# VinAIResearch/DiMSUM

Hardware: AMD Instinct MI355X
Metric: denoiser-fwd latents/sec (higher is better)
Workload: dtype f32; 1 GPU; DiM-L/2 denoiser forward, 256px (4x32x32 latents, 256 tokens), 256 latents per GPU, random-init weights (reference init, zero tensors re-drawn N(0, 0.02^2)); global_batch=256, parallelism=dp1 (replicas, independent latents), launch=eager, matmul_policy=f16s (see notes.matmul_policy)

## Files before the change

dimsum_amd/_lib.py:

```python
import ctypes as C
import os

_HERE = os.path.dirname(os.path.abspath(__file__))
LIB_PATH = os.environ.get("DIMSUM_HIP_LIB") or os.path.join(_HERE, "lib", "libdimsum_hip.so")

F32, F16, BF16 = 0, 1, 2
i32, i64, vp, f32 = C.c_int32, C.c_int64, C.c_void_p, C.c_float


u32 = C.c_uint32


class _Sized(C.Structure):

    def __init__(self, *args, **kw):
        super().__init__(*args, **kw)
        self.struct_size = C.sizeof(type(self))


class SsmExt(_Sized):
    _fields_ = [("struct_size", u32), ("kernel_variant", i32), ("ckpt_ptr", vp), ("timing_start_event", vp), ("timing_stop_event", vp),
                ("out_z_lo_offset", i64), ("dt_w_ptr", vp), ("dt_x_ptr", vp), ("dt_w_row_stride", i64), ("dt_x_row_stride", i64),
                ("dt_rank", i32), ("out_z_f16", i32), ("out_z_scale_ptr", vp), ("out_z_scale_ld", i64)]

# ... 235 lines not shown


class StateUpdateSlotsParams(_Sized):
    _fields_ = [("struct_size", u32), ("num_slots", i32), ("update", StateUpdateParams), ("slots_ptr", vp), ("slots_stride", i64)]


class DecodeLinearSlotsParams(_Sized):
    _fields_ = [("struct_size", u32), ("num_slots", i32), ("linear", DecodeLinearParams), ("slots_ptr", vp), ("slots_stride", i64)]


DECODE_NORM_NONE, DECODE_NORM_LAYER, DECODE_NORM_RMS = 0, 1, 2
DECODE_MAX_BATCH = 16


class CrossEntropyParams(_Sized):
    _fields_ = ([("struct_size", u32), ("dtype", i32)]
                + [(n, i64) for n in ("rows", "vocab", "logits_row_stride", "dlogits_row_stride", "dloss_stride", "ignore_index")]
                + [(n, f32) for n in ("label_smoothing", "logit_scale", "lse_square_scale")] + [("reserved", i32)]
                + [(n, vp) for n in ("logits_ptr", "labels_ptr", "dloss_ptr", "loss_ptr", "lse_ptr", "z_loss_ptr", "dlogits_ptr")])


CROSS_ENTROPY_WAVE_ROW_MAX = 4096


class SampleLogitsParams(_Sized):
    _fields_ = ([("struct_size", u32), ("dtype", i32)] + [(n, i64) for n in ("rows", "vocab", "logits_row_stride")]
                + [("top_k", i32), ("top_p", f32), ("temperature", f32), ("reserved", i32)]
                + [(n, vp) for n in ("logits_ptr", "u_ptr", "out_ptr", "row_index_ptr", "out_table_ptr")] + [("table_steps", i64)])


class NormParams(_Sized):
    _fields_ = ([("struct_size", u32)] + [(n, i32) for n in ("rows", "cols", "is_rms_norm", "x_dtype", "residual_dtype", "out_dtype")]
                + [("eps", f32)]
                + [(n, i64) for n in ("x_row_stride", "residual_row_stride", "y_row_stride", "residual_out_row_stride")]
                + [(n, vp) for n in ("x_ptr", "residual_ptr", "weight_ptr", "bias_ptr", "y_ptr", "residual_out_ptr",
                                     "mean_ptr", "rstd_ptr", "xbias_ptr", "mod_scale_ptr", "mod_shift_ptr")]
                + [("mod_row_stride", i64), ("rows_per_batch", i32), ("y_split3", i32), ("y_inv_scale_ptr", vp)])


class NormBwdParams(_Sized):
    _fields_ = ([("struct_size", u32)] + [(n, i32) for n in ("rows", "cols", "is_rms_norm")] + [("eps", f32), ("reserved", i32)]
                + [(n, i64) for n in ("r_row_stride", "dy_row_stride", "dres_row_stride", "dx_row_stride")]
                + [(n, vp) for n in ("r_ptr", "weight_ptr", "mean_ptr", "rstd_ptr", "dy_ptr", "dres_ptr", "dx_ptr",
                                     "dweight_ptr", "dbias_ptr")])


class TtParams(_Sized):
    _fields_ = ([("struct_size", u32)] + [(n, i32) for n in ("batch", "tokens", "channels", "grid", "kind", "y_split3")]
                + [(n, i64) for n in ("x_batch_stride", "x_token_stride", "res_batch_stride", "res_token_stride",
                                      "y_batch_stride", "y_token_stride", "mod_batch_stride", "w_batch_stride",
                                      "w_token_stride", "red_batch_stride")]
                + [(n, vp) for n in ("x_ptr", "in_index_ptr", "out_index_ptr", "gate_ptr", "scale_ptr", "shift_ptr",
                                     "residual_ptr", "y_ptr", "w_ptr", "wdot_ptr", "wsum_ptr", "tsum_ptr", "y_inv_scale_ptr")]
                + [("y_f16s_lds_offset", i32), ("reserved", i32)])


class XattnParams(_Sized):
    _fields_ = ([("struct_size", u32)] + [(n, i32) for n in ("batch", "seqlen", "heads", "head_dim")] + [("scale", f32), ("n_dirs", i32)]
                + [(n, i64) for n in ("qkv_batch_stride", "qkv_token_stride", "out_batch_stride", "out_token_stride")]
                + [(n, vp) for n in ("qkv1_ptr", "qkv2_ptr", "out_ptr", "lse_ptr", "bias1_ptr", "bias2_ptr")]
                + [("precision", i32), ("out_split3", i32)]
                + [(n, vp) for n in ("x1_inv_ptr", "x2_inv_ptr", "kv_bound_ptr", "out_inv_ptr")] + [("qkv_f16", i32), ("reserved2", i32)])


class XattnBwdParams(_Sized):
    _fields_ = ([("struct_size", u32), ("reserved", u32), ("fwd", XattnParams)] + [(n, i64) for n in ("dqkv_batch_stride", "dqkv_token_stride")]
                + [(n, vp) for n in ("dout_ptr", "dqkv1_ptr", "dqkv2_ptr", "delta_ptr")])


class GemmExt(_Sized):
    _fields_ = ([("struct_size", u32), ("rows_per_batch", i32), ("timing_start_event", vp), ("timing_stop_event", vp)]
                + [(n, i32) for n in ("tune_variant", "tune_group_m", "tune_reserved", "c_image_pieces")]
                + [(n, vp) for n in ("gate_bound_ptr", "h_inv_scale_ptr", "residual_ptr", "gate_ptr")]
                + [("residual_ld", i64), ("gate_ld", i64), ("x12_ptr", vp), ("x12_ld", i64), ("a_alias_rows", i64), ("b_alias_rows", i64),
                   ("a_alias_weight_order", i32), ("qkv_q_cols", i32), ("conv_weight_ptr", vp), ("conv_bias_ptr", vp),
                   ("conv_rows", i32), ("conv_width", i32), ("conv_seq", i32), ("conv_weight_ld", i32),
                   ("a_block_inv_ptr", vp), ("a_block_inv_ld", i64), ("tn_pair_a_cols", i64), ("tn_pair_b_cols", i64),
                   ("k_scale_ptr", vp), ("c_scale_ptr", vp), ("k_inv_a_ptr", vp), ("k_inv_b_ptr", vp)])


class GemmParams(_Sized):
    _fields_ = ([("struct_size", u32)] + [(n, i32) for n in ("m", "n", "k", "operand_dtype", "epilogue")] + [("out_scale", f32), ("reserved", i32)]
                + [(n, i64) for n in ("lda", "ldb", "ldc")]
                + [(n, vp) for n in ("a_ptr", "b_ptr", "bias_ptr", "c_ptr", "a_inv_scale_ptr", "b_inv_scale_ptr")]
                + [("ext", C.POINTER(GemmExt))])


class GeluExt(_Sized):
    _fields_ = [("struct_size", u32), ("reserved", i32), ("row_inv_ptr", vp), ("bound_ptr", vp)]


class GeluParams(_Sized):
    _fields_ = ([("struct_size", u32), ("out_image", i32), ("rows", i64), ("hidden", i64)]
                + [(n, vp) for n in ("x_ptr", "bias_ptr", "dh_ptr", "out_ptr", "inv_scale_ptr", "dbias_ptr")] + [("ext", C.POINTER(GeluExt))])


GELU_OUT_F32, GELU_OUT_SPLIT3, GELU_OUT_PAIR, GELU_OUT_F16S = 0, 1, 2, 3


class MoeExt(_Sized):
    _fields_ = [("struct_size", u32), ("reserved", i32)]


class MoeRouteParams(_Sized):
    _fields_ = ([("struct_size", u32), ("mode", i32), ("num_experts", i32), ("reserved", i32), ("tokens", i64), ("hidden", i64)]
                + [(n, vp) for n in ("x_ptr", "w_ptr", "b_ptr", "prob_ptr", "expert_ptr", "logits_ptr", "offsets_ptr", "perm_ptr", "inv_ptr",
                                     "row_expert_ptr", "work_ptr")]
                + [("work_bytes", i64)] + [(n, vp) for n in ("dprob_ptr", "dxp_ptr", "dx_ptr", "dw_ptr", "db_ptr")] + [("ext", C.POINTER(MoeExt))])


class MoeRowsParams(_Sized):
    _fields_ = ([("struct_size", u32), ("reserved", i32), ("rows", i64), ("hidden", i64)]
                + [(n, vp) for n in ("src_ptr", "perm_ptr", "prob_ptr", "y_ptr", "dst_ptr", "dprob_ptr")] + [("ext", C.POINTER(MoeExt))])


class MoeActParams(_Sized):
    _fields_ = ([("struct_size", u32), ("gated", i32), ("num_experts", i32), ("reserved", i32), ("rows", i64), ("width", i64)]
                + [(n, vp) for n in ("x_ptr", "bias_ptr", "row_expert_ptr", "dh_ptr", "out_ptr", "dbias_ptr")] + [("ext", C.POINTER(MoeExt))])


class MoeGemmParams(_Sized):
    _fields_ = ([("struct_size", u32), ("num_experts", i32), ("tokens", i64), ("k", i64), ("n", i64), ("ldc", i64), ("x_ptr", vp), ("offsets_ptr", vp),
                 ("w_ptrs", C.POINTER(vp)), ("bias_ptr", vp), ("out_ptr", vp), ("ext", C.POINTER(MoeExt))])


class MoeGemmDgradParams(_Sized):
    _fields_ = ([("struct_size", u32), ("num_experts", i32), ("tokens", i64), ("k", i64), ("n", i64), ("ldc", i64), ("dy_ptr", vp), ("offsets_ptr", vp),
                 ("w_ptrs", C.POINTER(vp)), ("dx_ptr", vp), ("ext", C.POINTER(MoeExt))])


class MoeGemmWgradParams(_Sized):
# ... 137 lines not shown
```

dimsum_amd/attention_fusion.py:

```python
import torch
import torch.nn as nn
import torch.nn.functional as F

from . import gemm, native
from .utils import note_torch_path


class _XattnCoreFn(torch.autograd.Function):

    @staticmethod
    def forward(ctx, qkv1, qkv2, bias1, bias2, heads):
        b1 = None if bias1 is None else bias1.float().contiguous()
        b2 = None if bias2 is None else bias2.float().contiguous()
        if not any(ctx.needs_input_grad[:4]):
            return native.xattn_fusion_fwd(qkv1, qkv2, heads, bias1=b1, bias2=b2)
        out, lse = native.xattn_fusion_fwd(qkv1, qkv2, heads, need_lse=True, bias1=b1, bias2=b2)
        ctx.heads = heads
        ctx.f16 = gemm.attn_bwd_f16_enabled(qkv1)
        ctx.save_for_backward(qkv1, qkv2, b1, b2, out, lse)
        return out

    @staticmethod
    def backward(ctx, dout):
        qkv1, qkv2, b1, b2, out, lse = ctx.saved_tensors
        dqkv1, dqkv2 = native.xattn_fusion_bwd(qkv1, qkv2, out, lse, dout, ctx.heads, bias1=b1, bias2=b2, f16=ctx.f16)
        W = dqkv1.shape[-1]
        db1 = dqkv1.reshape(-1, W).sum(0) if (b1 is not None and ctx.needs_input_grad[2]) else None
        db2 = dqkv2.reshape(-1, W).sum(0) if (b2 is not None and dqkv2 is not None and ctx.needs_input_grad[3]) else None
        return dqkv1, dqkv2, db1, db2, None


class CrossAttentionFusion(nn.Module):
    def __init__(self, dim, num_heads=8, qkv_bias=False, qk_norm=False, attn_drop=0.0, proj_drop=0.0,
                 norm_layer=nn.LayerNorm, swap_k=False):
        super().__init__()
        assert dim % num_heads == 0, "dim should be divisible by num_heads"
        self.num_heads = num_heads
        self.head_dim = dim // 2 // num_heads
        self.scale = self.head_dim ** -0.5
        self.swap_k = swap_k
        self.qkv1 = nn.Linear(dim // 2, dim // 2 * 3, bias=qkv_bias)
        self.q_norm1 = norm_layer(self.head_dim) if qk_norm else nn.Identity()
        self.k_norm1 = norm_layer(self.head_dim) if qk_norm else nn.Identity()
        self.qkv2 = nn.Linear(dim // 2, dim // 2 * 3, bias=qkv_bias)
        self.q_norm2 = norm_layer(self.head_dim) if qk_norm else nn.Identity()
        self.k_norm2 = norm_layer(self.head_dim) if qk_norm else nn.Identity()
        self.attn_drop = nn.Dropout(attn_drop)
        self.proj = nn.Linear(dim, dim)
        self.proj_drop = nn.Dropout(proj_drop)
        self._plain = not qk_norm and not swap_k

    def _split(self, qkv, B, N):
        return qkv.reshape(B, N, 3, self.num_heads, self.head_dim).permute(2, 0, 3, 1, 4).unbind(0)

    def forward(self, x1, x2):
        y, b = self.forward_deferred(x1, x2)
        return y if b is None else y + b

    def takes_images(self, ref):
        return self._plain and not (self.training and (self.attn_drop.p > 0.0 or self.proj_drop.p > 0.0)) and native.xattn_supported(ref, self.head_dim)

    def forward_deferred(self, x1, x2, images=False, residual=None):
        if images:
            B, N, C3 = x1.shape
            b1, b2 = self.qkv1.bias, self.qkv2.bias
            if (b1 is None) != (b2 is None):
                raise RuntimeError("CrossAttentionFusion: qkv1 / qkv2 must both have a bias or none")
            bk1 = {} if b1 is None else {"bias": b1.float().contiguous()}
            bk2 = {} if b2 is None else {"bias": b2.float().contiguous()}
            f16 = isinstance(x1, native.F16Image) and (self.num_heads * self.head_dim) % 8 == 0
            qkv1 = qkv2 = None
            if f16:
                kvb = gemm.attn_kv_bound(self.qkv1.weight, b1, self.qkv2.weight, b2)
                qkv1 = gemm.qkv_f16s(x1.reshape(B * N, C3), self.qkv1.weight, b1, N, kvb[0:2])
                qkv2 = gemm.qkv_f16s(x2.reshape(B * N, C3), self.qkv2.weight, b2, N, kvb[2:4]) if qkv1 is not None else None
            if qkv2 is None:
                qkv1 = gemm.linear_split3(x1.reshape(B * N, C3), self.qkv1.weight, **bk1)
                qkv2 = gemm.linear_split3(x2.reshape(B * N, C3), self.qkv2.weight, **bk2)
            qkv1, qkv2 = qkv1.view(B, N, -1), qkv2.view(B, N, -1)
            if f16:
                f3 = native.xattn_fusion_fwd(qkv1, qkv2, self.num_heads, split3="f16s", f16s=(x1.inv.reshape(B, N), x2.inv.reshape(B, N), kvb))
            else:
                f3 = native.xattn_fusion_fwd(qkv1, qkv2, self.num_heads, split_bf16=True, split3="pair" if isinstance(x1, native.PairImage) else True)
            if residual is not None:
                pb = None if self.proj.bias is None else self.proj.bias.float()
                y = gemm.linear_split3(f3.reshape(B * N, -1), self.proj.weight, bias=pb, residual=residual.reshape(B * N, -1))
                return y.view(residual.shape), None
            return gemm.linear_split3(f3.reshape(B * N, -1), self.proj.weight).view(B, N, -1), self.proj.bias
        B, N, C = x1.shape
        drop = self.attn_drop.p if self.training else 0.0
        if self._plain and drop == 0.0 and native.xattn_supported(x1, self.head_dim):
            b1, b2 = self.qkv1.bias, self.qkv2.bias
            if (b1 is None) != (b2 is None):
                raise RuntimeError("CrossAttentionFusion: qkv1 / qkv2 must both have a bias or none")
            fused = _XattnCoreFn.apply(gemm.linear(x1, self.qkv1.weight), gemm.linear(x2, self.qkv2.weight), b1, b2, self.num_heads)
        else:
            if self._plain and drop == 0.0:
                note_torch_path(f"CrossAttentionFusion core for head_dim {self.head_dim} / {x1.dtype}", required_opt_in=True)
            else:
                note_torch_path("CrossAttentionFusion variant (qk_norm / swap_k / attention dropout: unused by the published configs)")
            qkv1, qkv2 = self.qkv1(x1), self.qkv2(x2)
            q1, k1, v1 = self._split(qkv1, B, N)
            q2, k2, v2 = self._split(qkv2, B, N)
            q1, k1, q2, k2 = self.q_norm1(q1), self.k_norm1(k1), self.q_norm2(q2), self.k_norm2(k2)
            if not self.swap_k:
                x12 = F.scaled_dot_product_attention(q1, k2, v2, dropout_p=drop)
                x21 = F.scaled_dot_product_attention(q2, k1, v1, dropout_p=drop)
            else:
                x12 = F.scaled_dot_product_attention(q2, k1, v2, dropout_p=drop)
                x21 = F.scaled_dot_product_attention(q1, k2, v1, dropout_p=drop)
            fused = torch.cat((x12.transpose(1, 2).reshape(B, N, C), x21.transpose(1, 2).reshape(B, N, C)), dim=-1)
        if isinstance(self.proj_drop, nn.Dropout) and self.proj_drop.p > 0.0 and self.training:
            return self.proj_drop(self.proj(fused)), None
        return gemm.linear(fused, self.proj.weight), self.proj.bias
```

dimsum_amd/csrc/gemm_nt.hip:

```cpp
#include "gemm_nt_kernel.hpp"

namespace dimsum {
namespace gemm_nt {

struct gemm_flat_t : dimsum_gemm_ext_t {
    int32_t m, n, k, operand_dtype, epilogue;
    float out_scale;
    int64_t lda, ldb, ldc;
    const void *a_ptr, *b_ptr, *bias_ptr;
    void *c_ptr;
    const void *a_inv_scale_ptr, *b_inv_scale_ptr;
};
static int gemm_flat_from(const dimsum_gemm_params_t *p, gemm_flat_t &f) {
    if (!p) return DIMSUM_ERR_NULL;
    if (p->struct_size != sizeof(dimsum_gemm_params_t)) return DIMSUM_ERR_ABI;
    const int rc = ext_from<dimsum_gemm_ext_t>(p->ext, f);
    if (rc != DIMSUM_OK) return rc;
    f.m = p->m; f.n = p->n; f.k = p->k; f.operand_dtype = p->operand_dtype; f.epilogue = p->epilogue; f.out_scale = p->out_scale;
    f.lda = p->lda; f.ldb = p->ldb; f.ldc = p->ldc;
    f.a_ptr = p->a_ptr; f.b_ptr = p->b_ptr; f.bias_ptr = p->bias_ptr; f.c_ptr = p->c_ptr;
    f.a_inv_scale_ptr = p->a_inv_scale_ptr; f.b_inv_scale_ptr = p->b_inv_scale_ptr;
    return DIMSUM_OK;
}

// ... 100 lines not shown
    return a.N % (gated ? 128 : kBN) == 0 && nk >= 4 && nk % 2 == 0 && a.tiles_m * a.tiles_n > persist_grid() && a.a_alias_tiles == 0 && a.b_alias_tiles == 0;
}

}
}

#ifdef DIMSUM_GEMM_TUNE
#define DIMSUM_GEMM_TUNE_VARIANTS(X) X(1) X(2) X(4) X(8) X(12) X(16) X(3) X(40) X(44) X(72) X(104)
#define DIMSUM_GEMM_TUNE_CASE(V) case V: return launch<kOpBf16, kEpiF32, V>(a, w);
#endif

static int gemm_nt_run(const dimsum_gemm_params_t *pub, void *stream, int *probe) {
    using namespace dimsum;
    using namespace dimsum::gemm_nt;
    gemm_flat_t p;
    Args a;
    if (const int rc = gemm_prologue(pub, p, a)) return rc;
    if (p.m <= 0 || p.n <= 0 || p.k < 2 * kBK || p.m % kBM != 0 || p.k % kBK != 0 || p.n % 4 != 0) return DIMSUM_ERR_SHAPE;
    if (p.a_alias_rows != 0 && (p.a_alias_rows < 0 || p.a_alias_rows % kBK != 0 || p.k != 3 * p.a_alias_rows)) return DIMSUM_ERR_SHAPE;
    if (p.b_alias_rows != 0 && (p.b_alias_rows < 0 || p.b_alias_rows % kBK != 0 || p.k != 3 * p.b_alias_rows || (p.epilogue != DIMSUM_GEMM_EPI_F32 && p.epilogue != DIMSUM_GEMM_EPI_F32_CONV))) return DIMSUM_ERR_SHAPE;
    if (!rows_16bit_ok(p.a_ptr, p.lda, p.a_alias_rows ? 2 * p.a_alias_rows : p.k) || !rows_16bit_ok(p.b_ptr, p.ldb, p.b_alias_rows ? 2 * p.b_alias_rows : p.k)) return DIMSUM_ERR_STRIDE;
    if (!offsets_fit(p, false, false)) return DIMSUM_ERR_STRIDE;
    a.K = p.k;
    a.a_alias_tiles = (int)(p.a_alias_rows / kBK);
    a.a_alias_from = a.a_alias_tiles;
    if (p.a_alias_weight_order) {
        if (!p.a_alias_rows) return DIMSUM_ERR_SHAPE;
        a.a_alias_tiles *= 2;
        a.a_alias_from = a.a_alias_tiles;
    }
    a.b_alias_tiles = (int)(p.b_alias_rows / kBK);
    a.stagger = p.tune_reserved > 0 ? p.tune_reserved : 0;
    if ((p.a_inv_scale_ptr == nullptr) != (p.b_inv_scale_ptr == nullptr)) return DIMSUM_ERR_NULL;
    if (a.sb && !aligned_to<char>(a.sb, 16)) return DIMSUM_ERR_STRIDE;
#ifndef DIMSUM_GEMM_TUNE
    if (p.tune_variant != 0 && p.tune_variant != 512 && p.tune_variant != 513 && p.tune_variant != 514) return DIMSUM_ERR_UNSUPPORTED;
#endif
    const bool bf = p.operand_dtype == DIMSUM_BF16;
    if (p.tune_variant == 512 && bf) return DIMSUM_ERR_UNSUPPORTED;
    const bool m128 = m128_tiles(p.epilogue, bf, p.k, p.tune_variant);
    const Where w = where(p, stream, probe);
    constexpr int kShip = kVarFullLineStores | kVarNtStores;
    if (p.epilogue == DIMSUM_GEMM_EPI_F32_GATE_RESIDUAL) {
        if (!p.residual_ptr) return DIMSUM_ERR_NULL;
        if (!rows_f32_out_ok(p) || p.residual_ld % 4 != 0 || p.residual_ld < p.n || !aligned_to<char>(p.residual_ptr, 16) ||
            (p.bias_ptr && !aligned_to<char>(p.bias_ptr, 16)) || (p.gate_ptr && (p.gate_ld % 4 != 0 || !aligned_to<char>(p.gate_ptr, 16))))
            return DIMSUM_ERR_STRIDE;
        if (p.gate_ptr && (p.rows_per_batch <= 0 || p.rows_per_batch % kBM != 0 || p.m % p.rows_per_batch != 0)) return DIMSUM_ERR_SHAPE;
        fill_right(a, p, p.n, kBN);
        a.res = reinterpret_cast<const float *>(p.residual_ptr);
        a.gate = reinterpret_cast<const float *>(p.gate_ptr);
        a.ldr = p.residual_ld; a.ldg = p.gate_ld;
        a.rows_per_batch = p.gate_ptr ? p.rows_per_batch : p.m;
        if (persist_ok(a, p.epilogue, bf, p.tune_variant)) return launch_persist<kOpF16, kEpiF32GateRes, kShip>(a, w);
        return bf ? launch<kOpBf16, kEpiF32GateRes, kShip>(a, w) : launch_f16<kEpiF32GateRes, kShip>(a, w, m128);
    }
    if (p.epilogue == DIMSUM_GEMM_EPI_F16_QKV) {
        if (bf || !a.sa || !p.gate_bound_ptr) return DIMSUM_ERR_NULL;
        if (p.rows_per_batch <= 0 || p.rows_per_batch % kBM != 0 || p.m % p.rows_per_batch != 0 || p.qkv_q_cols <= 0 || p.qkv_q_cols % 16 != 0 ||
            p.qkv_q_cols > p.n || p.n % 8 != 0)
            return DIMSUM_ERR_SHAPE;
        if (p.ldc % 8 != 0 || p.ldc < p.n || !aligned_to<char>(p.c_ptr, 16) || (p.bias_ptr && !aligned_to<char>(p.bias_ptr, 16)) ||
            (int64_t)257 * p.ldc * 2 >= ((int64_t)1 << 31))
            return DIMSUM_ERR_STRIDE;
        fill_right(a, p, p.n, kBN);
        a.gate_bound = reinterpret_cast<const float *>(p.gate_bound_ptr);
        a.rows_per_batch = p.rows_per_batch;
        a.q_cols = p.qkv_q_cols;
        return launch_f16<kEpiF16Qkv>(a, w, m128);
    }
    if (p.epilogue == DIMSUM_GEMM_EPI_GELU_F16) {
        if (bf || !a.sa || !p.gate_bound_ptr || p.a_alias_rows != 0 || p.x12_ptr || p.c_image_pieces != 0) return DIMSUM_ERR_UNSUPPORTED;
        if (!p.h_inv_scale_ptr) return DIMSUM_ERR_NULL;
        if (p.n % 8 != 0) return DIMSUM_ERR_SHAPE;
        if (p.ldc % 8 != 0 || p.ldc < p.n || !aligned_to<char>(p.c_ptr, 16) || (p.bias_ptr && !aligned_to<char>(p.bias_ptr, 16)) ||
            !aligned_to<char>(p.h_inv_scale_ptr, 4) || (int64_t)257 * p.ldc * 2 >= ((int64_t)1 << 31))
            return DIMSUM_ERR_STRIDE;
        fill_right(a, p, p.n, kBN);
        a.gate_bound = reinterpret_cast<const float *>(p.gate_bound_ptr);
        a.inv_out = reinterpret_cast<float *>(p.h_inv_scale_ptr);
        return launch_f16<kEpiGeluF16>(a, w, m128);
    }
    if (p.epilogue == DIMSUM_GEMM_EPI_F32_CONV) {
        if (!p.conv_weight_ptr) return DIMSUM_ERR_NULL;
        if (p.conv_rows <= 0 || p.conv_rows % kBM != 0 || p.conv_rows > p.m || p.conv_width < 2 || p.conv_width > 4 || p.conv_seq <= 0 || 256 % p.conv_seq != 0 ||
            p.conv_seq % 4 != 0 || p.n % p.conv_seq != 0 || p.conv_weight_ld < p.conv_width)
            return DIMSUM_ERR_SHAPE;
        if (!rows_f32_out_ok(p)) return DIMSUM_ERR_STRIDE;
        fill_right(a, p, p.n, kBN);
        a.bias0 = nullptr;
        a.conv_w = reinterpret_cast<const float *>(p.conv_weight_ptr);
        a.conv_b = reinterpret_cast<const float *>(p.conv_bias_ptr);
        a.conv_rows = p.conv_rows; a.conv_width = p.conv_width; a.conv_seq = p.conv_seq; a.conv_w_ld = p.conv_weight_ld;
        return bf ? launch<kOpBf16, kEpiF32Conv, kShip>(a, w) : launch_f16<kEpiF32Conv, kShip>(a, w, m128);
    }
    if (p.epilogue == DIMSUM_GEMM_EPI_F32 || p.epilogue == DIMSUM_GEMM_EPI_F32_BIAS) {
        if (!rows_f32_out_ok(p)) return DIMSUM_ERR_STRIDE;
        const bool bias = p.epilogue == DIMSUM_GEMM_EPI_F32_BIAS;
        if (bias && (!p.bias_ptr || !aligned_to<char>(p.bias_ptr, 16))) return DIMSUM_ERR_NULL;
        fill_right(a, p, p.n, kBN);
        if (bias) return bf ? launch<kOpBf16, kEpiF32Bias, kShip>(a, w) : launch_f16<kEpiF32Bias, kShip>(a, w, m128);
#ifdef DIMSUM_GEMM_TUNE
        if (bf) switch (p.tune_variant) {
            case 0: case 512: case 513: break;
            case 100: return launch<kOpBf16, kEpiF32, 0>(a, w);
            DIMSUM_GEMM_TUNE_VARIANTS(DIMSUM_GEMM_TUNE_CASE)
// ... 123 lines not shown
```

dimsum_amd/csrc/gemm_nt_kernel.hpp:

```cpp
#pragma once
#include "common.hpp"

namespace dimsum {
namespace gemm_nt {

typedef float f4 __attribute__((ext_vector_type(4)));
typedef __bf16 bf16x8_t __attribute__((ext_vector_type(8)));
typedef _Float16 f16x8_t __attribute__((ext_vector_type(8)));
typedef unsigned u32x4 __attribute__((ext_vector_type(4)));
typedef unsigned u32x2 __attribute__((ext_vector_type(2)));
typedef __attribute__((address_space(3))) void lds_void_t;
typedef __attribute__((address_space(1))) const void glb_void_t;

constexpr int kBM = 256, kBN = 256, kBK = 64;
constexpr int kHalf = 16384;
constexpr int kParity = 4 * kHalf;
constexpr int kSlotA0 = 0, kSlotA1 = kHalf, kSlotB0 = 2 * kHalf, kSlotB1 = 3 * kHalf;

enum { kOpBf16 = 0, kOpF16 = 1 };
enum { kEpiF32 = 0, kEpiGatedSplit3 = 1, kEpiGatedF16 = 2, kEpiF32Bias = 3, kEpiF32GateRes = 4, kEpiF16Qkv = 5, kEpiF32Conv = 6, kEpiGeluF16 = 7 };

struct Args {
    const char *A, *B0, *B1;
    void *C;
    const float *bias0, *bias1;
    const float *sa, *sb;
    const float *gate_bound;
    float *inv_out;
    const float *res, *gate;
    int64_t ldr, ldg;
    int rows_per_batch;
    int64_t lda, ldb, ldc;
    int M, N, K;
    int tiles_m, tiles_n;
    float out_scale;
    int group_m;
    int stagger;
    float *x12;
    int64_t ldx;
    int splits;
    int64_t c_split_stride;
    int a_alias_tiles;
    int a_alias_from;
    int tn_pieces;
    int64_t a_pair_cols, b_pair_cols;
    int b_alias_tiles;
    const float *conv_w, *conv_b;
    int conv_rows, conv_width, conv_seq, conv_w_ld;
    const float *a_block_inv;
    int a_block_inv_ld;
    const _Float16 *k_fac;
    const float *c_scale;
    const float *k_inv_a, *k_inv_b;
    int q_cols;
    int c_pieces2;
};
enum { kVarLgkmAfterBarrier = 1, kVarNoEpilogue = 2, kVarNtStores = 4, kVarFullLineStores = 8, kVarNoSetprio = 16, kVarSc1Stores = 32, kVarSc0Stores = 64, kVarKeepX12 = 128, kVarTN = 256, kVarM128 = 512, kVarRebase = 1024, kVarPersist = 2048, kVarRowFac = 4096, kVarNN = 8192 };

__device__ __forceinline__ float dpp_row_ror8(float x) {
    const int v = __builtin_bit_cast(int, x);
    return __builtin_bit_cast(float, __builtin_amdgcn_update_dpp(v, v, 0x128, 0xf, 0xf, false));
}
template <int kAux> __device__ __forceinline__ void store_f4(__amdgpu_buffer_rsrc_t rsrc, unsigned voff, const f4 &v) {
    __builtin_amdgcn_raw_buffer_store_b128(__builtin_bit_cast(u32x4, v), rsrc, voff, 0, kAux);
}

template <int kOp> __device__ __forceinline__ f4 mma(const u32x4 &a, const u32x4 &b, f4 c) {
    if constexpr (kOp == kOpBf16) return __builtin_amdgcn_mfma_f32_16x16x32_bf16(__builtin_bit_cast(bf16x8_t, a), __builtin_bit_cast(bf16x8_t, b), c, 0, 0, 0);
    else return __builtin_amdgcn_mfma_f32_16x16x32_f16(__builtin_bit_cast(f16x8_t, a), __builtin_bit_cast(f16x8_t, b), c, 0, 0, 0);
}

__device__ __forceinline__ const char *uniform_ptr(const char *q) {
    const uint64_t v = reinterpret_cast<uint64_t>(q);
    const unsigned lo = __builtin_amdgcn_readfirstlane((unsigned)v), hi = __builtin_amdgcn_readfirstlane((unsigned)(v >> 32));
    return reinterpret_cast<const char *>(((uint64_t)hi << 32) | lo);
}

__device__ __forceinline__ unsigned pick_mask(bool c) {
    unsigned m = c ? 0xffffffffu : 0u;
    asm volatile("" : "+v"(m));
    return m;
}
// ... 501 lines not shown
        DIMSUM_WAIT_VM(8);
        DIMSUM_PHASE_SYNC();
        DIMSUM_QUADRANT(0, 1, a0, b1);
        DIMSUM_PHASE_END();
        DIMSUM_READ_A(a1, kSlotA1, par);
        read_fac(kt);
        DIMSUM_WAIT_VM(6);
        DIMSUM_PHASE_SYNC();
        rebase(a1, 1, kt);
        DIMSUM_QUADRANT(1, 1, a1, b1);
        DIMSUM_PHASE_END();
        DIMSUM_READ_A(a0, kSlotA0, par_next);
        read_fac(kt + 1);
        DIMSUM_WAIT_VM(4);
        DIMSUM_PHASE_SYNC();
        DIMSUM_QUADRANT(1, 0, a1, b0);
        rebase(a0, 0, kt + 1);
        DIMSUM_PHASE_END();
        DIMSUM_READ_B(b0, kSlotB0, par_next);
        DIMSUM_WAIT_VM(2);
        DIMSUM_PHASE_SYNC();
        DIMSUM_QUADRANT(0, 0, a0, b0);
        DIMSUM_PHASE_END();
        DIMSUM_READ_B(b1, kSlotB1, par_next);
        DIMSUM_WAIT_VM(0);
        DIMSUM_PHASE_SYNC();
        DIMSUM_QUADRANT(0, 1, a0, b1);
        DIMSUM_PHASE_END();
        DIMSUM_READ_A(a1, kSlotA1, par_next);
        read_fac(kt + 1);
        DIMSUM_PHASE_SYNC();
        rebase(a1, 1, kt + 1);
        DIMSUM_QUADRANT(1, 1, a1, b1);
        DIMSUM_PHASE_END();
        DIMSUM_QUADRANT(1, 0, a1, b0);
    }
    if (wr == 0) __builtin_amdgcn_s_barrier();
    }

    int lane_e = lane;
    if constexpr (kPersist) asm volatile("" : "+v"(lane_e));
    {
    const int lane = lane_e;
    const int ecol = wc * 32 + (lane >> 4) * 4;
    if constexpr (kVar & kVarNoEpilogue) {
#pragma unroll
        for (int mi = 0; mi < 2; ++mi)
#pragma unroll
            for (int ni = 0; ni < 2; ++ni)
#pragma unroll
                for (int i = 0; i < 4; ++i)
#pragma unroll
                    for (int j = 0; j < 2; ++j) asm volatile("" ::"v"(acc[mi][ni][i][j]));
    } else if constexpr (kEpi == kEpiF32 || kEpi == kEpiF32Bias || kEpi == kEpiF32GateRes || kEpi == kEpiF32Conv) {
        if constexpr (kEpi == kEpiF32Conv) {
            if (m0 < p.conv_rows) {
                constexpr int kNW = kM1 ? 4 : 8;
                constexpr int kHalfRows = kM1 ? 64 : 128;
                float *Ct = reinterpret_cast<float *>(p.C) + (int64_t)m0 * p.ldc + n0;
                const __amdgpu_buffer_rsrc_t crsrc = __builtin_amdgcn_make_buffer_rsrc(Ct, 0, 0x7fffffff, 0x00020000);
                const int W = p.conv_width;
                const bool has_s = p.sa != nullptr;
                const unsigned ms = pick_mask(has_s);
                const float *sap = has_s ? p.sa + m0 : reinterpret_cast<const float *>(p.A), *sbp = has_s ? p.sb : reinterpret_cast<const float *>(p.B0);
                float csa[2][4];
                f4 csb[2][2];
#pragma unroll
                for (int mi = 0; mi < 2; ++mi)
#pragma unroll
                    for (int i = 0; i < 4; ++i) {
                        csa[mi][i] = pick(ms, sap[mi * kMiRows + wr * 64 + i * 16 + (lane & 15)], 1.0f);
                    }
#pragma unroll
                for (int ni = 0; ni < 2; ++ni)
#pragma unroll
                    for (int j = 0; j < 2; ++j) {
                        const int col = n0 + ni * 128 + ecol + j * 16;
                        csb[ni][j] = pick(ms, *reinterpret_cast<const f4 *>(sbp + (col < p.N ? col : 0)), f4{1.f, 1.f, 1.f, 1.f});
                    }
                float ctap[2], cbia[2];
#pragma unroll
                for (int mi = 0; mi < 2; ++mi) {
                    const int row = m0 + mi * kMiRows + w * (kHalfRows / kNW) + (lane & 15);
                    ctap[mi] = pick(pick_mask_lanes((lane >> 4) < W), p.conv_w[(int64_t)row * p.conv_w_ld + ((lane >> 4) < W ? (lane >> 4) : 0)], 0.f);
                    cbia[mi] = pick(pick_mask(p.conv_b != nullptr), (p.conv_b ? p.conv_b : reinterpret_cast<const float *>(p.B0))[row], 0.f);
                }
#pragma unroll
                for (int mi = 0; mi < 2; ++mi) {
                    if (mi) __syncthreads();
#pragma unroll
                    for (int ni = 0; ni < 2; ++ni)
#pragma unroll
                        for (int j = 0; j < 2; ++j) {
                            const int tcol = ni * 128 + ecol + j * 16;
#pragma unroll
                            for (int i = 0; i < 4; ++i) {
                                const int rl = wr * 64 + i * 16 + (lane & 15);
                                const f4 x = acc[mi][ni][i][j] * (csb[ni][j] * csa[mi][i]);
                                *reinterpret_cast<f4 *>(lds + rl * 1024 + (((tcol >> 2) ^ (rl & 7)) << 4)) = x;
                            }
                        }
                    __syncthreads();
#pragma unroll 4
                    for (int it = 0; it < kHalfRows / kNW; ++it) {
                        const int rl = w * (kHalfRows / kNW) + it, row = m0 + mi * kMiRows + rl;
                        const f4 v = *reinterpret_cast<const f4 *>(lds + rl * 1024 + ((lane ^ (rl & 7)) << 4));
                        float w4[4];
#pragma unroll
                        for (int k = 0; k < 4; ++k)
                            w4[k] = (k >= 4 - W) ? __builtin_bit_cast(float, __builtin_amdgcn_readlane(__builtin_bit_cast(int, ctap[mi]), it + 16 * (k - (4 - W)))) : 0.f;
                        const float cbias = __builtin_bit_cast(float, __builtin_amdgcn_readlane(__builtin_bit_cast(int, cbia[mi]), it));
                        const bool start = ((4 * lane) % p.conv_seq) == 0;
                        float p1 = __shfl_up(v[3], 1, 64), p2 = __shfl_up(v[2], 1, 64), p3 = __shfl_up(v[1], 1, 64);
                        p1 = start ? 0.f : p1; p2 = start ? 0.f : p2; p3 = start ? 0.f : p3;
                        f4 y;
                        y[0] = fmaf(w4[0], p3, fmaf(w4[1], p2, fmaf(w4[2], p1, fmaf(w4[3], v[0], cbias))));
                        y[1] = fmaf(w4[0], p2, fmaf(w4[1], p1, fmaf(w4[2], v[0], fmaf(w4[3], v[1], cbias))));
                        y[2] = fmaf(w4[0], p1, fmaf(w4[1], v[0], fmaf(w4[2], v[1], fmaf(w4[3], v[2], cbias))));
                        y[3] = fmaf(w4[0], v[0], fmaf(w4[1], v[1], fmaf(w4[2], v[2], fmaf(w4[3], v[3], cbias))));
#pragma unroll
                        for (int e = 0; e < 4; ++e) y[e] = y[e] * fast_rcp(1.0f + fast_exp(-y[e]));
                        if (n0 + 4 * lane < p.N) store_f4<2>(crsrc, (unsigned)(((mi * kMiRows + rl) * p.ldc + 4 * lane) * 4), y);
                        DIMSUM_PACE_STORES();
                    }
                }
                return;
            }
        }
        constexpr int kAux = ((kVar & kVarNtStores) ? 2 : 0) | ((kVar & kVarSc1Stores) ? 16 : 0) | ((kVar & kVarSc0Stores) ? 1 : 0);
        float *Ct = reinterpret_cast<float *>(p.C) + (int64_t)m0 * p.ldc + n0 + (kBT ? (int64_t)split * p.c_split_stride : (int64_t)0);
        const __amdgpu_buffer_rsrc_t rsrc = __builtin_amdgcn_make_buffer_rsrc(Ct, 0, 0x7fffffff, 0x00020000);
        if constexpr (kVar & kVarFullLineStores) {
            const bool up = (lane & 8) != 0;
            const int frow = wr * 64 + (lane & 7);
            const int fcol = wc * 32 + (lane >> 4) * 4 + (up ? 16 : 0);
            const bool has_s = kRebase || p.sa != nullptr;
            const unsigned ms = pick_mask(has_s);
            const bool has_sb = has_s && !kRowFac;
            const unsigned msb = pick_mask(has_sb);
            const float *sap = p.sa ? p.sa + m0 : reinterpret_cast<const float *>(p.A), *sbp = has_sb ? p.sb : reinterpret_cast<const float *>(p.B0);
            float c_scale = 1.0f;
            if constexpr (kRowFac) c_scale = p.k_inv_a ? c_scale_own : *p.c_scale;
            bool live[2];
            f4 bv[2], sbv[2], gv[2];
            auto load_cols = [&](int ni) {
                const int col = ni * 128 + fcol;
                live[ni] = n0 + col < p.N;
                const int lc = live[ni] ? n0 + col : 0;
                bv[ni] = f4{0.f, 0.f, 0.f, 0.f}; sbv[ni] = gv[ni] = f4{1.f, 1.f, 1.f, 1.f};
                if constexpr (kEpi == kEpiF32Bias) bv[ni] = *reinterpret_cast<const f4 *>(p.bias0 + lc);
                if constexpr (kEpi == kEpiF32GateRes) {
                    bv[ni] = pick(pick_mask(p.bias0 != nullptr), *reinterpret_cast<const f4 *>((p.bias0 ? p.bias0 : reinterpret_cast<const float *>(p.B0)) + lc), bv[ni]);
                    gv[ni] = pick(pick_mask(p.gate != nullptr),
                                  *reinterpret_cast<const f4 *>((p.gate ? p.gate + (int64_t)(m0 / p.rows_per_batch) * p.ldg : reinterpret_cast<const float *>(p.B0)) + lc), gv[ni]);
                }
                sbv[ni] = pick(msb, *reinterpret_cast<const f4 *>(sbp + lc), sbv[ni]);
            };
            load_cols(0);
            live[1] = n0 + 128 + fcol < p.N;
            float rs[2][4][2];
            if constexpr (!kPersist || kRebase || kEpi != kEpiF32GateRes)
#pragma unroll
            for (int mi = 0; mi < 2; ++mi)
#pragma unroll
                for (int i = 0; i < 4; ++i) {
                    const int lrow = frow + mi * kMiRows + i * 16;
                    if constexpr (kRebase) rs[mi][i][0] = rs[mi][i][1] = top[mi * 2 + (i >> 1)];
                    else if constexpr (kRowFac) {
                        rs[mi][i][0] = c_scale * pick(ms, sap[lrow], 1.0f); rs[mi][i][1] = c_scale * pick(ms, sap[lrow + 8], 1.0f);
                    }
                    else {
                        rs[mi][i][0] = pick(ms, sap[lrow], 1.0f); rs[mi][i][1] = pick(ms, sap[lrow + 8], 1.0f);
                    }
                }
            constexpr int kGS = kPersist ? DIMSUM_PERSIST_GS : 4, kNG = 16 / kGS;
            f4 rr[2][kGS][2];
            float rg[2][kGS][2];
            auto load_res = [&](int g) {
                if constexpr (kEpi == kEpiF32GateRes) {
                    const int t0 = g * kGS, ni = t0 >> 3, mi = (t0 >> 2) & 1;
                    if constexpr (kPersist) {
#pragma unroll
                        for (int k = 0; k < kGS; ++k) {
                            const int lrow = frow + mi * kMiRows + ((t0 + k) & 3) * 16;
                            rg[g & 1][k][0] = pick(ms, sap[lrow], 1.0f); rg[g & 1][k][1] = pick(ms, sap[lrow + 8], 1.0f);
                        }
                    }
                    const float *rp = p.res + (int64_t)(m0 + frow + mi * kMiRows) * p.ldr + (live[ni] ? n0 + ni * 128 + fcol : 0);
#pragma unroll
                    for (int k = 0; k < kGS; ++k) {
                        const int i = (t0 + k) & 3;
                        rr[g & 1][k][0] = *reinterpret_cast<const f4 *>(rp + (int64_t)(i * 16) * p.ldr);
                        rr[g & 1][k][1] = *reinterpret_cast<const f4 *>(rp + (int64_t)(i * 16 + 8) * p.ldr);
                    }
                }
            };
            load_res(0);
#pragma unroll
            for (int g = 0; g < kNG; ++g) {
                if (g + 1 < kNG) load_res(g + 1);
                if (g * kGS == 4) load_cols(1);
#pragma unroll
                for (int k = 0; k < kGS; ++k) {
                    const int t = g * kGS + k, ni = t >> 3, mi = (t >> 2) & 1, i = t & 3;
                    const int col = ni * 128 + fcol;
                    const f4 x0 = acc[mi][ni][i][0], x1 = acc[mi][ni][i][1];
                    f4 s0, s1;
#pragma unroll
                    for (int e = 0; e < 4; ++e) {
                        const float r0 = dpp_row_ror8(x0[e]), r1 = dpp_row_ror8(x1[e]);
                        s0[e] = up ? r1 : x0[e];
                        s1[e] = up ? x1[e] : r0;
                    }
                    const int lrow = frow + mi * kMiRows + i * 16;
                    const unsigned voff = (unsigned)((lrow * p.ldc + col) * 4);
                    constexpr bool kRowsInGroup = kPersist && kEpi == kEpiF32GateRes;
                    s0 = s0 * (sbv[ni] * (kRowsInGroup ? rg[g & 1][k][0] : rs[mi][i][0]));
                    s1 = s1 * (sbv[ni] * (kRowsInGroup ? rg[g & 1][k][1] : rs[mi][i][1]));
                    if constexpr (kEpi == kEpiF32GateRes) {
                        s0 = rr[g & 1][k][0] + gv[ni] * (s0 + bv[ni]);
                        s1 = rr[g & 1][k][1] + gv[ni] * (s1 + bv[ni]);
                    } else {
                        s0 = s0 + bv[ni];
                        s1 = s1 + bv[ni];
                    }
                    if (live[ni]) {
                        store_f4<kAux>(rsrc, voff, s0);
                        store_f4<kAux>(rsrc, voff + (unsigned)(8 * p.ldc * 4), s1);
                    }
                    if constexpr (kEpi != kEpiF32GateRes) DIMSUM_PACE_STORES();
                }
            }
        } else {
            const int frow = wr * 64 + (lane & 15);
#pragma unroll
            for (int ni = 0; ni < 2; ++ni)
#pragma unroll
                for (int j = 0; j < 2; ++j) {
                    const int col = ni * 128 + ecol + j * 16;
                    if (n0 + col < p.N) {
                        f4 bv = f4{0.f, 0.f, 0.f, 0.f};
                        if constexpr (kEpi == kEpiF32Bias) bv = *reinterpret_cast<const f4 *>(p.bias0 + n0 + col);
#pragma unroll
                        for (int mi = 0; mi < 2; ++mi)
#pragma unroll
                            for (int i = 0; i < 4; ++i)
                                store_f4<kAux>(rsrc, (unsigned)(((frow + mi * kMiRows + i * 16) * p.ldc + col) * 4), acc[mi][ni][i][j] + bv);
                    }
                }
        }
    } else if constexpr (kEpi == kEpiF16Qkv || kEpi == kEpiGeluF16) {
        constexpr bool kGelu = kEpi == kEpiGeluF16;
        constexpr int kNW = kM1 ? 4 : 8;
        float *red = reinterpret_cast<float *>(lds);
        (void)red;
        const float wl1 = p.gate_bound[0], bmax = p.gate_bound[1];
        float row_sa[2][4], row_qs[2][4];
        f4 cbv[2][2], csb[2][2];
#pragma unroll
        for (int mi = 0; mi < 2; ++mi)
#pragma unroll
            for (int i = 0; i < 4; ++i) row_sa[mi][i] = p.sa[m0 + mi * kMiRows + wr * 64 + i * 16 + (lane & 15)];
        {
            const unsigned mbias = pick_mask(p.bias0 != nullptr);
            const float *b0p = p.bias0 ? p.bias0 : p.sb;
#pragma unroll
            for (int ni = 0; ni < 2; ++ni)
#pragma unroll
                for (int j = 0; j < 2; ++j) {
                    const int col = n0 + ni * 128 + ecol + j * 16, lc = col < p.N ? col : 0;
                    cbv[ni][j] = pick(mbias, *reinterpret_cast<const f4 *>(b0p + lc), f4{0.f, 0.f, 0.f, 0.f});
                    csb[ni][j] = *reinterpret_cast<const f4 *>(p.sb + lc);
                }
        }
        float kv_scale = 0.f, kv_inv;
        if constexpr (!kGelu) {
            {
                const float *sab = p.sa + (int64_t)(m0 / p.rows_per_batch) * p.rows_per_batch;
                float mloc = 0.f;
                for (int t = threadIdx.x; t < p.rows_per_batch; t += kNW * 64) mloc = fmaxf(mloc, sab[t]);
                mloc = wave_allmax(mloc);
                if (lane == 0) red[w] = mloc;
            }
// ... 278 lines not shown
```

dimsum_amd/csrc/norm.hip:

```cpp
#include "common.hpp"

namespace dimsum {

constexpr int kMaxPieces = 8;

__device__ __forceinline__ float wave_allsum(float v) {
#pragma unroll
    for (int o = 32; o > 0; o >>= 1) v += __shfl_xor(v, o, kWave);
    return v;
}

template <typename T> __device__ __forceinline__ f32x4 ld_cols(const T *row, int c, int N, bool vec) {
    if (vec) return c < N ? widen(ld4<T>(row + c)) : f32x4{{0.f, 0.f, 0.f, 0.f}};
    f32x4 r;
#pragma unroll
    for (int e = 0; e < 4; ++e) r.v[e] = (c + e < N) ? to_f32<T>(row[c + e]) : 0.f;
    return r;
}
template <typename T> __device__ __forceinline__ void st_cols(T *row, int c, int N, bool vec, const f32x4 &v) {
    if (vec) { if (c < N) st4<T>(row + c, v); return; }
#pragma unroll
    for (int e = 0; e < 4; ++e)
        if (c + e < N) row[c + e] = from_f32<T>(v.v[e]);
}
// ... 18 lines not shown
        const TR *res = p.residual_ptr ? reinterpret_cast<const TR *>(p.residual_ptr) + row * p.residual_row_stride : nullptr;
        TR *ro = p.residual_out_ptr ? reinterpret_cast<TR *>(p.residual_out_ptr) + row * p.residual_out_row_stride : nullptr;
        TY *y = reinterpret_cast<TY *>(p.y_ptr) + row * p.y_row_stride;
        f32x4 r[kPieces];
        float s = 0.f;
#pragma unroll
        for (int i = 0; i < kPieces; ++i) r[i] = ld_cols<TX>(x, (i * kWave + lane) * 4, N, vec);
        if (xb) {
            f32x4 q[kPieces];
#pragma unroll
            for (int i = 0; i < kPieces; ++i) q[i] = ld_cols<float>(xb, (i * kWave + lane) * 4, N, vec);
#pragma unroll
            for (int i = 0; i < kPieces; ++i)
#pragma unroll
                for (int e = 0; e < 4; ++e) r[i].v[e] += q[i].v[e];
        }
        if (res) {
            f32x4 q[kPieces];
#pragma unroll
            for (int i = 0; i < kPieces; ++i) q[i] = ld_cols<TR>(res, (i * kWave + lane) * 4, N, vec);
#pragma unroll
            for (int i = 0; i < kPieces; ++i)
#pragma unroll
                for (int e = 0; e < 4; ++e) r[i].v[e] += q[i].v[e];
        }
        if (ro) {
#pragma unroll
            for (int i = 0; i < kPieces; ++i) st_cols<TR>(ro, (i * kWave + lane) * 4, N, vec, r[i]);
        }
#pragma unroll
        for (int i = 0; i < kPieces; ++i)
#pragma unroll
            for (int e = 0; e < 4; ++e) s += p.is_rms_norm ? r[i].v[e] * r[i].v[e] : r[i].v[e];
        s = wave_allsum(s);
        float mean = 0.f, var;
        if (p.is_rms_norm) {
            var = s * inv_n;
        } else {
            mean = s * inv_n;
            float v2 = 0.f;
#pragma unroll
            for (int i = 0; i < kPieces; ++i) {
                const int c = (i * kWave + lane) * 4;
#pragma unroll
                for (int e = 0; e < 4; ++e) { const float dlt = (c + e < N) ? r[i].v[e] - mean : 0.f; v2 += dlt * dlt; }
            }
            var = wave_allsum(v2) * inv_n;
        }
        const float rstd = 1.0f / sqrtf(var + p.eps);
        if (lane == 0) {
            if (p.rstd_ptr) reinterpret_cast<float *>(p.rstd_ptr)[row] = rstd;
            if (p.mean_ptr && !p.is_rms_norm) reinterpret_cast<float *>(p.mean_ptr)[row] = mean;
        }
        float ymax = 0.f;
#pragma unroll
        for (int i = 0; i < kPieces; ++i) {
            const int c = (i * kWave + lane) * 4;
            if (c < N) {
                const f32x4 wv = ld_cols<float>(w, c, N, vec);
                const f32x4 bv = bb ? ld_cols<float>(bb, c, N, vec) : f32x4{{0.f, 0.f, 0.f, 0.f}};
                f32x4 o;
#pragma unroll
                for (int e = 0; e < 4; ++e) o.v[e] = (r[i].v[e] - mean) * rstd * wv.v[e] + bv.v[e];
                if (msc) {
                    const f32x4 sc = ld_cols<float>(msc, c, N, vec), sh = ld_cols<float>(msh, c, N, vec);
#pragma unroll
                    for (int e = 0; e < 4; ++e) o.v[e] = fmaf(o.v[e], 1.0f + sc.v[e], sh.v[e]);
                }
                if (p.y_split3 == 2) {
                    r[i] = o;
#pragma unroll
                    for (int e = 0; e < 4; ++e) ymax = fmaxf(ymax, fabsf(o.v[e]));
                } else if (p.y_split3) st_split_left(reinterpret_cast<unsigned short *>(p.y_ptr) + row * p.y_row_stride, c, N, o, p.y_split3 == 3);
                else st_cols<TY>(y, c, N, vec, o);
            }
        }
        if (p.y_split3 == 2) {
            float sc, inv;
            f16s_scales(wave_allmax(ymax), sc, inv);
            __half *yh = reinterpret_cast<__half *>(p.y_ptr) + row * p.y_row_stride;
#pragma unroll
            for (int i = 0; i < kPieces; ++i) {
                const int c = (i * kWave + lane) * 4;
                if (c < N) *reinterpret_cast<uint2 *>(yh + c) = f16s_pack4(r[i], sc);
            }
            if (lane == 0) reinterpret_cast<float *>(p.y_inv_scale_ptr)[row] = inv;
        }
    }
}

template <int kPieces>
__global__ __launch_bounds__(256) void norm_bwd_kernel(const dimsum_norm_bwd_params_t p, const bool vec) {
    const int lane = threadIdx.x & (kWave - 1);
    const int wave = __builtin_amdgcn_readfirstlane(threadIdx.x >> 6);
    const int N = p.cols;
    const float inv_n = 1.0f / (float)N;
    const float *w = reinterpret_cast<const float *>(p.weight_ptr);
    f32x4 wreg[kPieces], dw[kPieces], db[kPieces];
#pragma unroll
    for (int i = 0; i < kPieces; ++i) {
        const int c = (i * kWave + lane) * 4;
        wreg[i] = ld_cols<float>(w, c, N, vec);
        dw[i] = {{0.f, 0.f, 0.f, 0.f}};
        db[i] = {{0.f, 0.f, 0.f, 0.f}};
    }
    const int64_t stride = (int64_t)gridDim.x * 4;
// ... 79 lines not shown
        }
    }
}

template <typename TX, typename TR, typename TY>
static int launch_norm_fwd(const dimsum_norm_params_t &p, hipStream_t s) {
    const int N = p.cols;
    bool vec = N % 4 == 0 && aligned_to<TX>(p.x_ptr, 4 * sizeof(TX)) && aligned_to<TY>(p.y_ptr, 4 * sizeof(TY)) &&
               p.x_row_stride % 4 == 0 && p.y_row_stride % 4 == 0 && aligned_to<float>(p.weight_ptr, 16) &&
               (!p.bias_ptr || aligned_to<float>(p.bias_ptr, 16));
    if (p.residual_ptr) vec = vec && aligned_to<TR>(p.residual_ptr, 4 * sizeof(TR)) && p.residual_row_stride % 4 == 0;
    if (p.residual_out_ptr) vec = vec && aligned_to<TR>(p.residual_out_ptr, 4 * sizeof(TR)) && p.residual_out_row_stride % 4 == 0;
    if (p.xbias_ptr) vec = vec && aligned_to<float>(p.xbias_ptr, 16);
    if (p.mod_scale_ptr) vec = vec && aligned_to<float>(p.mod_scale_ptr, 16) && aligned_to<float>(p.mod_shift_ptr, 16) && p.mod_row_stride % 4 == 0;
    const int pieces = (N + 255) / 256;
    const int64_t blocks = (p.rows + 3) / 4;
    const dim3 grid((unsigned)(blocks < 256 * 16 ? blocks : 256 * 16)), block(256);
#define DIMSUM_NF(K) hipLaunchKernelGGL((norm_fwd_kernel<TX, TR, TY, K>), grid, block, 0, s, p, vec)
    if (pieces <= 1) DIMSUM_NF(1);
    else if (pieces <= 2) DIMSUM_NF(2);
    else if (pieces <= 4) DIMSUM_NF(4);
    else if (pieces <= 5) DIMSUM_NF(5);
    else if (pieces <= kMaxPieces) DIMSUM_NF(8);
    else return DIMSUM_ERR_SHAPE;
#undef DIMSUM_NF
    return launch_status();
}

template <typename TX, typename TR>
static int dispatch_out(const dimsum_norm_params_t &p, hipStream_t s) {
    switch (p.out_dtype) {
        case DIMSUM_F32: return launch_norm_fwd<TX, TR, float>(p, s);
        case DIMSUM_F16: return launch_norm_fwd<TX, TR, __half>(p, s);
        case DIMSUM_BF16: return launch_norm_fwd<TX, TR, __hip_bfloat16>(p, s);
        default: return DIMSUM_ERR_DTYPE;
    }
}
template <typename TX>
static int dispatch_res(const dimsum_norm_params_t &p, hipStream_t s) {
    switch (p.residual_dtype) {
        case DIMSUM_F32: return dispatch_out<TX, float>(p, s);
        case DIMSUM_F16: return dispatch_out<TX, __half>(p, s);
        case DIMSUM_BF16: return dispatch_out<TX, __hip_bfloat16>(p, s);
        default: return DIMSUM_ERR_DTYPE;
    }
}

}

extern "C" int dimsum_norm_fwd(const dimsum_norm_params_t *p, void *stream) {
    using namespace dimsum;
    if (!p) return DIMSUM_ERR_NULL;
    if (p->struct_size != sizeof(dimsum_norm_params_t)) return DIMSUM_ERR_ABI;
    if (!p->x_ptr || !p->weight_ptr || !p->y_ptr) return DIMSUM_ERR_NULL;
    if (p->rows < 0 || p->cols <= 0) return DIMSUM_ERR_SHAPE;
    if ((p->mod_scale_ptr == nullptr) != (p->mod_shift_ptr == nullptr)) return DIMSUM_ERR_NULL;
    if (p->mod_scale_ptr && p->rows_per_batch <= 0) return DIMSUM_ERR_SHAPE;
    if (p->y_split3 == 2) {
        if (!p->y_inv_scale_ptr) return DIMSUM_ERR_NULL;
        if (p->out_dtype != DIMSUM_F16 || p->cols % 4 != 0 || p->y_row_stride % 4 != 0 || p->y_row_stride < p->cols || !dimsum::aligned_to<char>(p->y_ptr, 8))
            return DIMSUM_ERR_STRIDE;
    } else
    if (p->y_split3 && (p->out_dtype != DIMSUM_BF16 || p->cols % 4 != 0 || p->y_row_stride % 4 != 0 || p->y_row_stride < (p->y_split3 == 3 ? 2 : 3) * (int64_t)p->cols ||
                        !dimsum::aligned_to<char>(p->y_ptr, 8)))
        return DIMSUM_ERR_STRIDE;
    if (p->rows == 0) return DIMSUM_OK;
    hipStream_t s = reinterpret_cast<hipStream_t>(stream);
    switch (p->x_dtype) {
        case DIMSUM_F32: return dispatch_res<float>(*p, s);
        case DIMSUM_F16: return dispatch_res<__half>(*p, s);
        case DIMSUM_BF16: return dispatch_res<__hip_bfloat16>(*p, s);
        default: return DIMSUM_ERR_DTYPE;
    }
}

extern "C" int dimsum_norm_bwd(const dimsum_norm_bwd_params_t *p, void *stream) {
    using namespace dimsum;
    if (!p) return DIMSUM_ERR_NULL;
    if (p->struct_size != sizeof(dimsum_norm_bwd_params_t)) return DIMSUM_ERR_ABI;
    if (!p->r_ptr || !p->weight_ptr || !p->rstd_ptr || !p->dy_ptr || !p->dx_ptr || !p->dweight_ptr) return DIMSUM_ERR_NULL;
    if (p->rows < 0 || p->cols <= 0) return DIMSUM_ERR_SHAPE;
    if (p->rows == 0) return DIMSUM_OK;
    hipStream_t s = reinterpret_cast<hipStream_t>(stream);
    const int N = p->cols;
    bool vec = N % 4 == 0 && aligned_to<float>(p->r_ptr, 16) && aligned_to<float>(p->dy_ptr, 16) && aligned_to<float>(p->dx_ptr, 16) &&
               aligned_to<float>(p->weight_ptr, 16) && p->r_row_stride % 4 == 0 && p->dy_row_stride % 4 == 0 && p->dx_row_stride % 4 == 0;
    if (p->dres_ptr) vec = vec && aligned_to<float>(p->dres_ptr, 16) && p->dres_row_stride % 4 == 0;
    const int pieces = (N + 255) / 256;
    const int64_t blocks = (p->rows + 3) / 4;
    const int64_t cap = p->rows >= 32768 ? 512 : 384;
    const dim3 grid((unsigned)(blocks < cap ? blocks : cap)), block(256);
#define DIMSUM_NB(K) hipLaunchKernelGGL((norm_bwd_kernel<K>), grid, block, 0, s, *p, vec)
    if (pieces <= 1) DIMSUM_NB(1);
    else if (pieces <= 2) DIMSUM_NB(2);
    else if (pieces <= 4) DIMSUM_NB(4);
    else if (pieces <= 5) DIMSUM_NB(5);
    else if (pieces <= kMaxPieces) DIMSUM_NB(8);
    else return DIMSUM_ERR_SHAPE;
#undef DIMSUM_NB
    return launch_status();
}
```

dimsum_amd/csrc/token_transform.hip:

```cpp
#include <stdlib.h>
#include <type_traits>

#include "common.hpp"

namespace dimsum {

constexpr int kTTThreads = 256;
__device__ __forceinline__ int haar_lds(int j) {
    const int cp = j >> 4, p = j & 15;
    return (cp >> 2) * 68 + p * 4 + (cp & 3);
}

__device__ __forceinline__ void haar2(float a, float b, float c, float d, float &ll, float &lh, float &hl, float &hh) {
    const float p = a + b, q = a - b, r = c + d, s = c - d;
    ll = (p + r) * 0.5f; lh = (p - r) * 0.5f; hl = (q + s) * 0.5f; hh = (q - s) * 0.5f;
}
__device__ __forceinline__ void ihaar2(float ll, float lh, float hl, float hh, float &a, float &b, float &c, float &d) {
    const float p = ll + lh, q = ll - lh, r = hl + hh, s = hl - hh;
    a = (p + r) * 0.5f; b = (p - r) * 0.5f; c = (q + s) * 0.5f; d = (q - s) * 0.5f;
}

__device__ __forceinline__ void haar_fwd16(const float *X, float *Y) {
    float b1[4][4];
#pragma unroll
// ... 1 lines not shown
#pragma unroll
        for (int j = 0; j < 2; ++j)
            haar2(X[(2 * i) * 4 + 2 * j], X[(2 * i) * 4 + 2 * j + 1], X[(2 * i + 1) * 4 + 2 * j], X[(2 * i + 1) * 4 + 2 * j + 1],
                  b1[0][i * 2 + j], b1[1][i * 2 + j], b1[2][i * 2 + j], b1[3][i * 2 + j]);
#pragma unroll
    for (int k1 = 0; k1 < 4; ++k1) {
        float o[4];
        haar2(b1[k1][0], b1[k1][1], b1[k1][2], b1[k1][3], o[0], o[1], o[2], o[3]);
#pragma unroll
        for (int k2 = 0; k2 < 4; ++k2) Y[k1 * 4 + k2] = o[k2] * 0.25f;
    }
}
__device__ __forceinline__ void haar_inv16(const float *Y, float *X) {
    float b1[4][4];
#pragma unroll
    for (int k1 = 0; k1 < 4; ++k1)
        ihaar2(Y[k1 * 4 + 0], Y[k1 * 4 + 1], Y[k1 * 4 + 2], Y[k1 * 4 + 3], b1[k1][0], b1[k1][1], b1[k1][2], b1[k1][3]);
#pragma unroll
    for (int i = 0; i < 2; ++i)
#pragma unroll
        for (int j = 0; j < 2; ++j)
            ihaar2(b1[0][i * 2 + j], b1[1][i * 2 + j], b1[2][i * 2 + j], b1[3][i * 2 + j], X[(2 * i) * 4 + 2 * j],
                   X[(2 * i) * 4 + 2 * j + 1], X[(2 * i + 1) * 4 + 2 * j], X[(2 * i + 1) * 4 + 2 * j + 1]);
}

__device__ __forceinline__ void dct4(const float *in, int stride, float *out, int ostride, bool inverse) {
    constexpr float kA = 0.5f;
    constexpr float kC1 = 0.6532814824381883f;
    constexpr float kC2 = 0.5f;
    constexpr float kC3 = 0.2705980500730985f;
    const float x0 = in[0], x1 = in[stride], x2 = in[2 * stride], x3 = in[3 * stride];
    if (!inverse) {
        const float s03 = x0 + x3, d03 = x0 - x3, s12 = x1 + x2, d12 = x1 - x2;
        out[0] = kA * (s03 + s12);
        out[ostride] = kC1 * d03 + kC3 * d12;
        out[2 * ostride] = kC2 * (s03 - s12);
        out[3 * ostride] = kC3 * d03 - kC1 * d12;
    } else {
        const float e = kA * x0 + kC2 * x2, f = kA * x0 - kC2 * x2, g = kC1 * x1 + kC3 * x3, h = kC3 * x1 - kC1 * x3;
        out[0] = e + g;
        out[ostride] = f + h;
        out[2 * ostride] = f - h;
        out[3 * ostride] = e - g;
    }
}
__device__ __forceinline__ void dct16(const float *X, float *Y, bool inverse) {
    float t[16];
#pragma unroll
    for (int r = 0; r < 4; ++r) dct4(X + r * 4, 1, t + r * 4, 1, inverse);
#pragma unroll
    for (int c = 0; c < 4; ++c) dct4(t + c, 4, Y + c, 4, inverse);
}

template <int KIND, int VEC, bool F16S = false, int kFix = 0>
__global__ __launch_bounds__(kTTThreads) void token_transform_kernel(const dimsum_tt_params_t p) {
    extern __shared__ __attribute__((aligned(16))) float lds[];
    const int tid = threadIdx.x;
    const int nthreads = (F16S || KIND != DIMSUM_TT_NONE) ? (int)blockDim.x : kTTThreads;
    const int b = blockIdx.y;
    const int C = p.channels, G = p.grid;
    int s_of[16];
    if (KIND == DIMSUM_TT_NONE) {
#pragma unroll
        for (int k = 0; k < 16; ++k) s_of[k] = blockIdx.x * 16 + k;
    } else {
        const int gb = G / 4, bh = blockIdx.x / gb, bw = blockIdx.x - bh * gb;
#pragma unroll
        for (int k = 0; k < 16; ++k) s_of[k] = (bh * 4 + (k >> 2)) * G + bw * 4 + (k & 3);
    }
    int grp = blockIdx.x;
    const int ngrp = KIND == DIMSUM_TT_NONE ? (p.tokens + 15) / 16 : 1;
    auto pos_of = [&](int k) { return KIND == DIMSUM_TT_NONE ? grp * 16 + k : s_of[k]; };
    int tin[KIND == DIMSUM_TT_NONE ? 1 : 16], tout[KIND == DIMSUM_TT_NONE ? 1 : 16];
    if constexpr (KIND != DIMSUM_TT_NONE) {
        if (p.in_index_ptr) {
#pragma unroll
            for (int k = 0; k < 16; ++k) tin[k] = p.in_index_ptr[s_of[k]];
        } else {
#pragma unroll
            for (int k = 0; k < 16; ++k) tin[k] = s_of[k];
        }
        if (p.out_index_ptr) {
#pragma unroll
            for (int k = 0; k < 16; ++k) tout[k] = p.out_index_ptr[s_of[k]];
        } else {
#pragma unroll
            for (int k = 0; k < 16; ++k) tout[k] = s_of[k];
        }
    }
    float stash[F16S ? 16 : 1][VEC], tmax[F16S ? 16 : 1];
    if constexpr (F16S) {
#pragma unroll
        for (int k = 0; k < 16; ++k) tmax[k] = 0.f;
    }
    const float *xb = reinterpret_cast<const float *>(p.x_ptr) + (int64_t)b * p.x_batch_stride;
    float *yb = p.y_ptr ? reinterpret_cast<float *>(p.y_ptr) + (int64_t)b * p.y_batch_stride : nullptr;
    const float *rb = p.residual_ptr ? reinterpret_cast<const float *>(p.residual_ptr) + (int64_t)b * p.res_batch_stride : nullptr;
    const float *gate = p.gate_ptr ? reinterpret_cast<const float *>(p.gate_ptr) + (int64_t)b * p.mod_batch_stride : nullptr;
    const float *scale = p.scale_ptr ? reinterpret_cast<const float *>(p.scale_ptr) + (int64_t)b * p.mod_batch_stride : nullptr;
    const float *shift = p.shift_ptr ? reinterpret_cast<const float *>(p.shift_ptr) + (int64_t)b * p.mod_batch_stride : nullptr;

    const float *wb = p.w_ptr ? reinterpret_cast<const float *>(p.w_ptr) + (int64_t)b * p.w_batch_stride : nullptr;
    const bool has_gate = kFix == 0 ? gate != nullptr : kFix == 2;
    const bool has_mod = kFix == 0 ? scale != nullptr : (kFix == 1 || kFix == 3 || kFix == 5);
    const bool has_shift = kFix == 0 ? shift != nullptr : kFix == 1;
    const bool has_res = kFix == 0 ? rb != nullptr : kFix == 2;
    const bool has_w = kFix == 0 ? wb != nullptr : kFix >= 3;
    const bool has_tsum = kFix == 0 ? p.tsum_ptr != nullptr : kFix == 5;
    const bool has_y = kFix == 0 ? yb != nullptr : kFix != 4;
    float wdot[VEC], wsum[VEC], tsum[VEC];
#pragma unroll
    for (int e = 0; e < VEC; ++e) { wdot[e] = 0.f; wsum[e] = 0.f; tsum[e] = 0.f; }
    auto flush_red = [&](int c) {
        if (wb || p.tsum_ptr) {
#pragma unroll
            for (int e = 0; e < VEC; ++e) {
                if (p.wdot_ptr) atomicAdd(reinterpret_cast<float *>(p.wdot_ptr) + (int64_t)b * p.red_batch_stride + c + e, wdot[e]);
                if (p.wsum_ptr) atomicAdd(reinterpret_cast<float *>(p.wsum_ptr) + (int64_t)b * p.red_batch_stride + c + e, wsum[e]);
                if (p.tsum_ptr) atomicAdd(reinterpret_cast<float *>(p.tsum_ptr) + (int64_t)b * p.red_batch_stride + c + e, tsum[e]);
                wdot[e] = 0.f; wsum[e] = 0.f; tsum[e] = 0.f;
            }
        }
    };

    auto load_vec = [&](const float *ptr, float *dst) {
        if constexpr (VEC == 4) { const float4 t = *reinterpret_cast<const float4 *>(ptr); dst[0] = t.x; dst[1] = t.y; dst[2] = t.z; dst[3] = t.w; }
        else dst[0] = *ptr;
    };
    auto store_out = [&](int k, int c, const float *val) {
#pragma clang fp contract(off)
        int tok;
        if constexpr (KIND == DIMSUM_TT_NONE) {
            if (pos_of(k) >= p.tokens) return;
            tok = p.out_index_ptr ? p.out_index_ptr[pos_of(k)] : pos_of(k);
        } else {
            tok = tout[k];
        }
        float o[VEC], t[VEC];
#pragma unroll
        for (int e = 0; e < VEC; ++e) o[e] = val[e];
        if (has_w) { load_vec(wb + (int64_t)tok * p.w_token_stride + c, t);
#pragma unroll
            for (int e = 0; e < VEC; ++e) { wdot[e] = fmaf(o[e], t[e], wdot[e]); wsum[e] += t[e]; } }
        if (has_tsum) {
#pragma unroll
            for (int e = 0; e < VEC; ++e) tsum[e] += o[e]; }
        if (!has_y) return;
        if (has_mod) { load_vec(scale + c, t);
#pragma unroll
            for (int e = 0; e < VEC; ++e) o[e] *= 1.0f + t[e]; }
        if (has_shift) { load_vec(shift + c, t);
#pragma unroll
            for (int e = 0; e < VEC; ++e) o[e] += t[e]; }
        if (has_res) { load_vec(rb + (int64_t)tok * p.res_token_stride + c, t);
#pragma unroll
            for (int e = 0; e < VEC; ++e) o[e] += t[e]; }
        if constexpr (F16S) {
#pragma unroll
            for (int e = 0; e < VEC; ++e) { stash[k][e] = o[e]; tmax[k] = fmaxf(tmax[k], fabsf(o[e])); }
            return;
        }
        if constexpr (VEC == 4) {
            if (p.y_split3) {
                st_split_left(reinterpret_cast<unsigned short *>(p.y_ptr) + (int64_t)b * p.y_batch_stride + (int64_t)tok * p.y_token_stride, c, C,
                              f32x4{{o[0], o[1], o[2], o[3]}}, p.y_split3 == 3);
                return;
            }
        }
        float *dst = yb + (int64_t)tok * p.y_token_stride + c;
        if constexpr (VEC == 4) *reinterpret_cast<float4 *>(dst) = make_float4(o[0], o[1], o[2], o[3]);
        else dst[0] = o[0];
    };
    auto load_in = [&](int k, int c, float *dst) {
#pragma clang fp contract(off)
        int tok;
        if constexpr (KIND == DIMSUM_TT_NONE) {
            if (pos_of(k) >= p.tokens) {
#pragma unroll
                for (int e = 0; e < VEC; ++e) dst[e] = 0.f;
                return;
            }
            tok = p.in_index_ptr ? p.in_index_ptr[pos_of(k)] : pos_of(k);
        } else {
            tok = tin[k];
        }
        load_vec(xb + (int64_t)tok * p.x_token_stride + c, dst);
        if (has_gate) { float t[VEC]; load_vec(gate + c, t);
#pragma unroll
            for (int e = 0; e < VEC; ++e) dst[e] *= t[e]; }
    };

    if constexpr (KIND == DIMSUM_TT_NONE) {
        const int cg = (C + VEC - 1) / VEC;
        const int nsub = cg <= kTTThreads / 4 ? 4 : (cg <= kTTThreads / 2 ? 2 : 1);
        if (!F16S && nsub > 1 && C % VEC == 0) {
            const int sub = tid / cg, c = (tid - sub * cg) * VEC;
            if (sub < nsub) {
                auto pass = [&](auto perc) {
                    constexpr int PER = decltype(perc)::value;
                    for (grp = blockIdx.x; grp < ngrp; grp += gridDim.x) {
                        float v[PER][VEC];
#pragma unroll
                        for (int k = 0; k < PER; ++k) load_in(sub * PER + k, c, v[k]);
#pragma unroll
                        for (int k = 0; k < PER; ++k) store_out(sub * PER + k, c, v[k]);
                    }
                    flush_red(c);
                };
                if (nsub == 2) pass(std::integral_constant<int, 8>{});
                else pass(std::integral_constant<int, 4>{});
            }
            return;
        }
    }

    if constexpr (KIND == DIMSUM_TT_HAAR_INV) {
        for (int c = tid * VEC; c < C; c += nthreads * VEC) {
#pragma unroll
            for (int k = 0; k < 16; ++k) {
                float v[VEC];
                load_in(k, c, v);
#pragma unroll
                for (int e = 0; e < VEC; ++e) lds[haar_lds((c + e) * 16 + k)] = v[e] * 4.0f;
            }
        }
        __syncthreads();
    }

    for (int c = tid * VEC; c < C; c += nthreads * VEC) {
        float X[VEC][16], Y[VEC][16];
        if constexpr (KIND == DIMSUM_TT_HAAR_INV) {
#pragma unroll
            for (int q = 0; q < 16; ++q)
#pragma unroll
                for (int e = 0; e < VEC; ++e) Y[e][q] = lds[haar_lds(q * C + c + e)];
#pragma unroll
            for (int e = 0; e < VEC; ++e) haar_inv16(Y[e], X[e]);
#pragma unroll
            for (int k = 0; k < 16; ++k) { float o[VEC];
// ... 41 lines not shown
            }
        }
    }

    if constexpr (KIND == DIMSUM_TT_HAAR_FWD) {
        __syncthreads();
        for (int c = tid * VEC; c < C; c += nthreads * VEC) {
#pragma unroll
            for (int k = 0; k < 16; ++k) {
                float o[VEC];
                if constexpr (VEC == 4) {
                    const float4 t = *reinterpret_cast<const float4 *>(&lds[(c >> 2) * 68 + k * 4]);
                    o[0] = t.x; o[1] = t.y; o[2] = t.z; o[3] = t.w;
                } else {
                    o[0] = lds[haar_lds(c * 16 + k)];
                }
                store_out(k, c, o);
            }
            flush_red(c);
        }
    }

    if constexpr (F16S && VEC == 4) {
        float *red = lds + p.y_f16s_lds_offset;
        const int wave = tid >> 6, lane = tid & 63;
#pragma unroll
        for (int k = 0; k < 16; ++k) tmax[k] = wave_allmax(tmax[k]);
        if (lane < 16) {
            float m = tmax[0];
#pragma unroll
            for (int k = 1; k < 16; ++k) m = lane == k ? tmax[k] : m;
            red[wave * 16 + lane] = m;
        }
        __syncthreads();
        const int c = tid * VEC;
        __half *yh = reinterpret_cast<__half *>(p.y_ptr) + (int64_t)b * p.y_batch_stride;
        float *inv_out = reinterpret_cast<float *>(p.y_inv_scale_ptr) + (int64_t)b * p.tokens;
#pragma unroll
        for (int k = 0; k < 16; ++k) {
            if (KIND == DIMSUM_TT_NONE && pos_of(k) >= p.tokens) continue;
            float m = red[k];
            for (int w = 1; w < (nthreads >> 6); ++w) m = fmaxf(m, red[w * 16 + k]);
            float sc, inv;
            f16s_scales(m, sc, inv);
            int tok;
            if constexpr (KIND == DIMSUM_TT_NONE) tok = p.out_index_ptr ? p.out_index_ptr[pos_of(k)] : pos_of(k);
            else tok = tout[k];
            if (c < C) *reinterpret_cast<uint2 *>(yh + (int64_t)tok * p.y_token_stride + c) = f16s_pack4(f32x4{{stash[k][0], stash[k][1], stash[k][2], stash[k][3]}}, sc);
            if (tid == k) inv_out[tok] = inv;
        }
    }
}

template <int kPieces, int kOut>
__global__ __launch_bounds__(256) void token_rows_kernel(const dimsum_tt_params_t p) {
    const int lane = threadIdx.x & 63, wave = threadIdx.x >> 6;
    const int C = p.channels, T = p.tokens;
    const int64_t rows = (int64_t)p.batch * T;
    for (int64_t row = (int64_t)blockIdx.x * 4 + wave; row < rows; row += (int64_t)gridDim.x * 4) {
        const int b = (int)(row / T), s = (int)(row - (int64_t)b * T);
        const int src = p.in_index_ptr ? p.in_index_ptr[s] : s, dst = p.out_index_ptr ? p.out_index_ptr[s] : s;
        const float *x = reinterpret_cast<const float *>(p.x_ptr) + (int64_t)b * p.x_batch_stride + (int64_t)src * p.x_token_stride;
        const float *res = p.residual_ptr ? reinterpret_cast<const float *>(p.residual_ptr) + (int64_t)b * p.res_batch_stride + (int64_t)dst * p.res_token_stride : nullptr;
        const float *gate = p.gate_ptr ? reinterpret_cast<const float *>(p.gate_ptr) + (int64_t)b * p.mod_batch_stride : nullptr;
        const float *scale = p.scale_ptr ? reinterpret_cast<const float *>(p.scale_ptr) + (int64_t)b * p.mod_batch_stride : nullptr;
        const float *shift = p.shift_ptr ? reinterpret_cast<const float *>(p.shift_ptr) + (int64_t)b * p.mod_batch_stride : nullptr;
        f32x4 v[kPieces];
        float m = 0.f;
        auto ld = [&](const float *ptr, f32x4 (&q)[kPieces]) {
#pragma unroll
            for (int i = 0; i < kPieces; ++i) {
                const int c = (i * 64 + lane) * 4;
                const float4 t = c < C ? *reinterpret_cast<const float4 *>(ptr + c) : make_float4(0.f, 0.f, 0.f, 0.f);
                q[i] = f32x4{{t.x, t.y, t.z, t.w}};
            }
        };
        f32x4 q[kPieces];
        ld(x, v);
        if (gate) { ld(gate, q);
#pragma unroll
            for (int i = 0; i < kPieces; ++i)
#pragma unroll
                for (int e = 0; e < 4; ++e) v[i].v[e] *= q[i].v[e]; }
        if (scale) { ld(scale, q);
#pragma unroll
            for (int i = 0; i < kPieces; ++i)
#pragma unroll
                for (int e = 0; e < 4; ++e) v[i].v[e] *= 1.0f + q[i].v[e]; }
        if (shift) { ld(shift, q);
#pragma unroll
            for (int i = 0; i < kPieces; ++i)
#pragma unroll
                for (int e = 0; e < 4; ++e) v[i].v[e] += q[i].v[e]; }
        if (res) { ld(res, q);
#pragma unroll
            for (int i = 0; i < kPieces; ++i)
#pragma unroll
                for (int e = 0; e < 4; ++e) v[i].v[e] += q[i].v[e]; }
#pragma unroll
        for (int i = 0; i < kPieces; ++i)
#pragma unroll
            for (int e = 0; e < 4; ++e) m = fmaxf(m, fabsf(v[i].v[e]));
        if constexpr (kOut == 2) {
            float sc, inv;
            f16s_scales(wave_allmax(m), sc, inv);
            __half *y = reinterpret_cast<__half *>(p.y_ptr) + (int64_t)b * p.y_batch_stride + (int64_t)dst * p.y_token_stride;
#pragma unroll
            for (int i = 0; i < kPieces; ++i) {
                const int c = (i * 64 + lane) * 4;
                if (c < C) *reinterpret_cast<uint2 *>(y + c) = f16s_pack4(v[i], sc);
            }
            if (lane == 0) reinterpret_cast<float *>(p.y_inv_scale_ptr)[(int64_t)b * T + dst] = inv;
        } else if constexpr (kOut == 1) {
            unsigned short *y = reinterpret_cast<unsigned short *>(p.y_ptr) + (int64_t)b * p.y_batch_stride + (int64_t)dst * p.y_token_stride;
#pragma unroll
            for (int i = 0; i < kPieces; ++i) {
                const int c = (i * 64 + lane) * 4;
                if (c < C) st_split_left(y, c, C, v[i], p.y_split3 == 3);
            }
        } else {
            float *y = reinterpret_cast<float *>(p.y_ptr) + (int64_t)b * p.y_batch_stride + (int64_t)dst * p.y_token_stride;
#pragma unroll
            for (int i = 0; i < kPieces; ++i) {
                const int c = (i * 64 + lane) * 4;
                if (c < C) *reinterpret_cast<float4 *>(y + c) = make_float4(v[i].v[0], v[i].v[1], v[i].v[2], v[i].v[3]);
            }
        }
    }
}

template <int VEC>
static int launch_tt(const dimsum_tt_params_t &p, hipStream_t s) {
    const bool blocked = p.kind != DIMSUM_TT_NONE;
    const int nblk = blocked ? (p.grid / 4) * (p.grid / 4) : (p.tokens + 15) / 16;
    const int cgs = (p.channels + VEC - 1) / VEC;
    int gx = nblk;
    if (!blocked && (p.w_ptr || p.tsum_ptr) && p.y_split3 != 2) {
        const int min_wgs = p.y_ptr ? 1024 : 512;
        while (gx % 2 == 0 && (int64_t)(gx / 2) * p.batch >= min_wgs) gx /= 2;
    }
    const dim3 grid(gx, p.batch), block(blocked ? (cgs <= 64 ? 64 : (cgs <= 128 ? 128 : kTTThreads)) : kTTThreads);
    size_t lds = (p.kind == DIMSUM_TT_HAAR_FWD || p.kind == DIMSUM_TT_HAAR_INV) ? (size_t)((p.channels + 3) / 4) * 68 * 4 : 0;
    if (lds > 160 * 1024) return DIMSUM_ERR_SHAPE;
    if (p.kind == DIMSUM_TT_NONE && p.y_ptr && !p.w_ptr && !p.tsum_ptr && p.channels <= 2048) {
        if constexpr (VEC == 4) {
            const int64_t rows = (int64_t)p.batch * p.tokens;
            int64_t blocks = (rows + 3) / 4;
            if (blocks > 256 * 16) blocks = 256 * 16;
            const dim3 g1((unsigned)blocks), b1(256);
#define DIMSUM_TTR(O)                                                                                    \
            if (p.channels <= 512) hipLaunchKernelGGL((token_rows_kernel<2, O>), g1, b1, 0, s, p);          \
            else if (p.channels <= 1024) hipLaunchKernelGGL((token_rows_kernel<4, O>), g1, b1, 0, s, p);    \
            else hipLaunchKernelGGL((token_rows_kernel<8, O>), g1, b1, 0, s, p)
            if (p.y_split3 == 2) { DIMSUM_TTR(2); }
            else if (p.y_split3) { DIMSUM_TTR(1); }
            else { DIMSUM_TTR(0); }
#undef DIMSUM_TTR
            return launch_status();
        }
        if (p.y_split3 == 2) return DIMSUM_ERR_STRIDE;
    }
    if (p.y_split3 == 2) {
        if constexpr (VEC == 4) {
            dimsum_tt_params_t q = p;
            q.y_f16s_lds_offset = (int32_t)(lds / 4);
            lds += 64 * 4;
            const int cg = (p.channels + 3) / 4;
            const dim3 blockh(cg <= 64 ? 64 : (cg <= 128 ? 128 : kTTThreads));
            static const bool fix = !(getenv("DIMSUM_TT_FIX") && atoi(getenv("DIMSUM_TT_FIX")) == 0);
            const bool pre = fix && p.scale_ptr && p.shift_ptr && !p.gate_ptr && !p.residual_ptr, post = fix && p.gate_ptr && p.residual_ptr && !p.scale_ptr && !p.shift_ptr;
#define DIMSUM_TTH(K) do { if (blocked && pre) hipLaunchKernelGGL((token_transform_kernel<K, 4, true, (K) == DIMSUM_TT_NONE ? 0 : 1>), grid, blockh, lds, s, q);          \
                           else if (blocked && post) hipLaunchKernelGGL((token_transform_kernel<K, 4, true, (K) == DIMSUM_TT_NONE ? 0 : 2>), grid, blockh, lds, s, q);    \
                           else hipLaunchKernelGGL((token_transform_kernel<K, 4, true, 0>), grid, blockh, lds, s, q); } while (0)
            switch (p.kind) {
                case DIMSUM_TT_NONE: DIMSUM_TTH(DIMSUM_TT_NONE); break;
                case DIMSUM_TT_HAAR_FWD: DIMSUM_TTH(DIMSUM_TT_HAAR_FWD); break;
                case DIMSUM_TT_HAAR_INV: DIMSUM_TTH(DIMSUM_TT_HAAR_INV); break;
                case DIMSUM_TT_DCT_FWD: DIMSUM_TTH(DIMSUM_TT_DCT_FWD); break;
                case DIMSUM_TT_DCT_INV: DIMSUM_TTH(DIMSUM_TT_DCT_INV); break;
                default: return DIMSUM_ERR_SHAPE;
            }
#undef DIMSUM_TTH
            return launch_status();
        }
        return DIMSUM_ERR_STRIDE;
    }
    if constexpr (VEC == 4) {
        static const bool fix = !(getenv("DIMSUM_TT_FIX") && atoi(getenv("DIMSUM_TT_FIX")) == 0);
        const bool sc = p.scale_ptr != nullptr, sh = p.shift_ptr != nullptr, ga = p.gate_ptr != nullptr, re = p.residual_ptr != nullptr;
        const bool w = p.w_ptr != nullptr, ts = p.tsum_ptr != nullptr, y = p.y_ptr != nullptr;
        int kf = 0;
        if (fix && !w && !ts && y) kf = (blocked && sc && sh && !ga && !re) ? 1 : (blocked && ga && re && !sc && !sh) ? 2 : 0;
        else if (fix && w && !sh && !ga && !re) kf = (sc && !ts && y) ? 3 : (!sc && !ts && !y) ? 4 : (sc && ts && y) ? 5 : 0;
        if (kf) {
#define DIMSUM_TTF(K) do { if (kf == 1) hipLaunchKernelGGL((token_transform_kernel<K, 4, false, 1>), grid, block, lds, s, p);      \
                           else if (kf == 2) hipLaunchKernelGGL((token_transform_kernel<K, 4, false, 2>), grid, block, lds, s, p); \
                           else if (kf == 3) hipLaunchKernelGGL((token_transform_kernel<K, 4, false, 3>), grid, block, lds, s, p); \
                           else if (kf == 4) hipLaunchKernelGGL((token_transform_kernel<K, 4, false, 4>), grid, block, lds, s, p); \
                           else hipLaunchKernelGGL((token_transform_kernel<K, 4, false, 5>), grid, block, lds, s, p); } while (0)
            switch (p.kind) {
                case DIMSUM_TT_NONE: DIMSUM_TTF(DIMSUM_TT_NONE); break;
                case DIMSUM_TT_HAAR_FWD: DIMSUM_TTF(DIMSUM_TT_HAAR_FWD); break;
                case DIMSUM_TT_HAAR_INV: DIMSUM_TTF(DIMSUM_TT_HAAR_INV); break;
                case DIMSUM_TT_DCT_FWD: DIMSUM_TTF(DIMSUM_TT_DCT_FWD); break;
                case DIMSUM_TT_DCT_INV: DIMSUM_TTF(DIMSUM_TT_DCT_INV); break;
                default: return DIMSUM_ERR_SHAPE;
            }
#undef DIMSUM_TTF
            return launch_status();
        }
    }
#define DIMSUM_TT(K) hipLaunchKernelGGL((token_transform_kernel<K, VEC>), grid, block, lds, s, p)
    switch (p.kind) {
        case DIMSUM_TT_NONE: DIMSUM_TT(DIMSUM_TT_NONE); break;
        case DIMSUM_TT_HAAR_FWD: DIMSUM_TT(DIMSUM_TT_HAAR_FWD); break;
        case DIMSUM_TT_HAAR_INV: DIMSUM_TT(DIMSUM_TT_HAAR_INV); break;
        case DIMSUM_TT_DCT_FWD: DIMSUM_TT(DIMSUM_TT_DCT_FWD); break;
        case DIMSUM_TT_DCT_INV: DIMSUM_TT(DIMSUM_TT_DCT_INV); break;
        default: return DIMSUM_ERR_SHAPE;
    }
#undef DIMSUM_TT
    return launch_status();
}

}

extern "C" int dimsum_token_transform(const dimsum_tt_params_t *p, void *stream) {
    using namespace dimsum;
    if (!p) return DIMSUM_ERR_NULL;
    if (p->struct_size != sizeof(dimsum_tt_params_t)) return DIMSUM_ERR_ABI;
    if (!p->x_ptr) return DIMSUM_ERR_NULL;
    if (!p->y_ptr && !p->tsum_ptr && !(p->w_ptr && (p->wdot_ptr || p->wsum_ptr))) return DIMSUM_ERR_NULL;
    if ((p->wdot_ptr || p->wsum_ptr) && !p->w_ptr) return DIMSUM_ERR_NULL;
    if (p->batch < 0 || p->tokens <= 0 || p->channels <= 0) return DIMSUM_ERR_SHAPE;
    if (p->kind != DIMSUM_TT_NONE && (p->grid % 4 != 0 || p->grid * p->grid != p->tokens)) return DIMSUM_ERR_SHAPE;
    if (p->batch == 0) return DIMSUM_OK;
    hipStream_t s = reinterpret_cast<hipStream_t>(stream);
    bool vec = p->channels % 4 == 0 && aligned_to<float>(p->x_ptr, 16) && (!p->y_ptr || aligned_to<float>(p->y_ptr, 16)) &&
               p->x_batch_stride % 4 == 0 && p->x_token_stride % 4 == 0 && p->y_batch_stride % 4 == 0 && p->y_token_stride % 4 == 0 &&
               p->mod_batch_stride % 4 == 0 && (!p->gate_ptr || aligned_to<float>(p->gate_ptr, 16)) &&
               (!p->scale_ptr || aligned_to<float>(p->scale_ptr, 16)) && (!p->shift_ptr || aligned_to<float>(p->shift_ptr, 16));
    if (p->residual_ptr) vec = vec && aligned_to<float>(p->residual_ptr, 16) && p->res_batch_stride % 4 == 0 && p->res_token_stride % 4 == 0;
    if (p->w_ptr) vec = vec && aligned_to<float>(p->w_ptr, 16) && p->w_batch_stride % 4 == 0 && p->w_token_stride % 4 == 0;
    if (p->y_split3 == 2) {
        if (!p->y_ptr || !p->y_inv_scale_ptr) return DIMSUM_ERR_NULL;
        if (!vec || p->y_token_stride < p->channels || p->channels > (p->kind == DIMSUM_TT_NONE ? 2048 : 4 * kTTThreads) || p->w_ptr || p->tsum_ptr)
            return DIMSUM_ERR_STRIDE;
    } else
    if (p->y_split3 && (!vec || !p->y_ptr || p->y_token_stride < (p->y_split3 == 3 ? 2 : 3) * (int64_t)p->channels)) return DIMSUM_ERR_STRIDE;
    return vec ? launch_tt<4>(*p, s) : launch_tt<1>(*p, s);
}
```

dimsum_amd/gemm.py:

```python
import contextlib
import os
import threading

import torch
import torch.nn.functional as F

_policy = "default"


class _Local(threading.local):
    frozen = None


_tls = _Local()


@contextlib.contextmanager
def frozen_weights():
    outer = _tls.frozen
    if outer is None:
        _tls.frozen = {}
    try:
        yield
    finally:
# ... 428 lines not shown
            cache[key("w16s_bound", w)] = (scal[sl:sl + 2], w)
        else:
            cache[key("w16s", w)] = ((images[j], lambda i=sl: scal[i:i + 1] / _K10), w)
            if partner is not None:
                j2 = j + (2 if bias is not None else 1)
                cache[key("w16s", partner.weight)] = ((images[j2], lambda i=sl + 2: scal[i:i + 1] / _K10), partner.weight)
                cache[key("kvbound", w)] = (scal[sl:sl + 4], w)
            else:
                cache[key("kvbound", w)] = (torch.cat([scal[sl:sl + 2], scal[sl:sl + 2]]), w)
    if not training and os.environ.get("DIMSUM_FORWARD_MEMO", "1") != "0":
        alogs = [a for m in model.modules() for a in (getattr(m, "A_log", None), getattr(m, "A_b_log", None)) if isinstance(a, torch.nn.Parameter) and a.is_cuda]
        if alogs:
            vals = torch._foreach_neg(torch._foreach_exp([a.detach().float() for a in alogs]))
            for a, v in zip(alogs, vals):
                cache[key("negexpA", a)] = (v, a)
    _tls.frozen = cache
    try:
        yield
    finally:
        _tls.frozen = None


def neg_exp(a_log):
    frozen = _tls.frozen
    if frozen is not None and not torch.is_grad_enabled() and not torch.cuda.is_current_stream_capturing():
        hit = frozen.get(("negexpA", a_log.data_ptr(), tuple(a_log.shape), tuple(a_log.stride()), a_log.dtype))
        if hit is not None:
            return hit[0]
    return -torch.exp(a_log.float())


def own_gemm_enabled():
    return os.environ.get("DIMSUM_GEMM_NT", "1") != "0"


def _nt(a, b, **kw):
    from . import native
    if own_gemm_enabled() and native.gemm_nt_supported(a, b):
        return native.gemm_nt(a, b, **kw)
    y = torch.mm(a, b.t(), out_dtype=torch.float32)
    return y if kw.get("bias") is None else y + kw["bias"]


def _tail(y, bias, residual, gate, rows_per_batch):
    if bias is not None:
        y = y + bias
    if residual is None:
        return y
    if gate is not None:
        y = (y.view(-1, rows_per_batch, y.shape[-1]) * gate.unsqueeze(1)).view(y.shape)
    return residual + y


def _nt_f16s(a, b, bias=None, residual=None, gate=None, rows_per_batch=None):
    from . import native
    if own_gemm_enabled() and native.gemm_nt_supported(a.data, b.data) and (gate is None or rows_per_batch % 256 == 0):
        return native.gemm_nt(a.data, b.data, bias=bias, scales=(a.inv, b.inv), residual=residual, gate=gate, rows_per_batch=rows_per_batch)
    return _tail(torch.mm(a.data, b.data.t(), out_dtype=torch.float32) * a.inv[:, None] * b.inv[None, :], bias, residual, gate, rows_per_batch)


def linear_split3(x3, weight, bias=None, residual=None, gate=None, rows_per_batch=None):
    from . import native
    if isinstance(x3, native.F16Image):
        return _nt_f16s(x3, weight_f16s(weight), bias, residual, gate, rows_per_batch)
    w3i = weight_image(weight)
    if isinstance(x3, native.PairImage) and not (own_gemm_enabled() and native.gemm_nt_supported(x3, w3i) and (gate is None or rows_per_batch % 256 == 0)):
        x3 = x3.image3()
    if residual is None and bias is None:
        return _nt(x3, w3i)
    if own_gemm_enabled() and native.gemm_nt_supported(x3, w3i) and (gate is None or rows_per_batch % 256 == 0):
        return native.gemm_nt(x3, w3i, bias=bias, residual=residual, gate=gate, rows_per_batch=rows_per_batch)
    return _tail(torch.mm(x3, w3i.t(), out_dtype=torch.float32), bias, residual, gate, rows_per_batch)


def matmul_wx_split3(weight, x3, conv=None):
    from . import native
    if conv is not None:
        cw, cb, seq = conv
        a = weight_f16s(weight) if isinstance(x3, native.F16Image) else weight_image(weight)
        ad, bd = (a.data, x3.data) if isinstance(x3, native.F16Image) else (a, x3)
        ok = (os.environ.get("DIMSUM_INPROJ_CONV", "1") != "0" and own_gemm_enabled() and native.gemm_nt_supported(ad, bd)
              and cw.dtype == torch.float32 and cw.dim() == 2 and cw.stride(1) == 1 and cw.shape[0] % 256 == 0 and 2 <= cw.shape[1] <= 4
              and seq % 4 == 0 and 256 % seq == 0 and x3.shape[0] % seq == 0)
        if ok:
            cbf = None if cb is None else cb.detach().float().contiguous()
            if isinstance(x3, native.F16Image):
                return native.gemm_nt(ad, bd, scales=(a.inv, x3.inv), conv=(cw.detach(), cbf, seq)), True
            return native.gemm_nt(a, x3, conv=(cw.detach(), cbf, seq)), True
        return matmul_wx_split3(weight, x3), False
    if isinstance(x3, native.F16Image):
        return _nt_f16s(weight_f16s(weight), x3)
    w3i = weight_image(weight)
    if isinstance(x3, native.PairImage) and not (own_gemm_enabled() and native.gemm_nt_supported(w3i, x3)):
        x3 = x3.image3()
    return _nt(w3i, x3)


def gated_mlp_hidden_split3(x3, w12, b12):
    from . import native
    if isinstance(x3, native.F16Image):
        w16 = weight_f16s(w12)
        if own_gemm_enabled() and native.gemm_nt_supported(x3.data, w16.data, gated=True):
            return native.gemm_nt(x3.data, w16.data, bias=b12, epilogue="gated_f16", scales=(x3.inv, w16.inv), gate_bound=gated_bound(w12, b12))
        x12 = _nt_f16s(x3, w16)
        return native.rows_f16s(native.gated_gelu_fwd(x12, b12))
    w3i = weight_image(w12)
    if own_gemm_enabled() and native.gemm_nt_supported(x3, w3i, gated=True):
        pair = (w12.shape[0] // 2) % 64 == 0 and os.environ.get("DIMSUM_PAIR_IMAGES", "1") != "0"
        return native.gemm_nt(x3, w3i, bias=b12, epilogue="gated_split3", pair_out=pair)
    if isinstance(x3, native.PairImage):
        x3 = x3.image3()
    return native.gated_gelu_fwd(torch.mm(x3, w3i.t(), out_dtype=torch.float32), b12, split3=True)


def mlp_hidden_split3(x3, w1, b1):
    from . import native
    F_ = w1.shape[0]
# ... 117 lines not shown
```

dimsum_amd/models_dim.py:

```python
import math
import os
from functools import partial

import numpy as np
import torch
import torch.nn as nn
import torch.nn.functional as F

from . import scanning_orders as so
from . import gemm
from .attention_fusion import CrossAttentionFusion
from .dct_layer import init_dct_kernel, init_idct_kernel
from .mlp import GatedMLP, Mlp
from .switch_mlp import SwitchMLP
from .modules.mamba_simple import CondMamba, Mamba
from .ops import token_ops
from .ops.layernorm import RMSNorm, layer_norm_fn, rms_norm_fn
from .pe.cpe import AdaInPosCNN
from .pe.my_rotary import apply_rotary, get_2d_sincos_rotary_embed
from .wavelet_layer import DWT_2D, IDWT_2D


def modulate(x, shift, scale):
    return x * (1 + scale.unsqueeze(1)) + shift.unsqueeze(1)
# ... 225 lines not shown
    if inference_params is not None:
        raise NotImplementedError("inference_params: " + _NOT_CAUSAL)


def _modulation(seq, c):
    hit = getattr(gemm._tls, "cond", None)
    if hit is not None and hit[0] is c and len(seq) == 2 and isinstance(seq[0], nn.SiLU):
        return seq[1](hit[1])
    return seq(c)


def _mlp_in_weight(mlp):
    return (mlp.w12 if isinstance(mlp, GatedMLP) else mlp.fc1).weight


def _mlp_tail(mlp, x, normed, shift, scale, gate):
    if isinstance(mlp, GatedMLP) and mlp._fused and gemm.split3_train_enabled(normed, mlp.w12.weight):
        from .mlp import mod_gated_mlp_images
        m, mb = mod_gated_mlp_images(mlp, normed, shift, scale)
        return token_ops.gate_residual(x, m, gate, mb)
    h = token_ops.pre_mixer(normed, "none", None, shift, scale)
    if hasattr(mlp, "forward_deferred"):
        m, mb = mlp.forward_deferred(h)
        return token_ops.gate_residual(x, m, gate, mb)
    return token_ops.gate_residual(x, mlp(h), gate, None)


def _fast_tail(norm_2, mlp, hidden_states):
    return (not torch.is_grad_enabled() and isinstance(norm_2, RMSNorm) and hasattr(mlp, "forward_deferred")
            and hidden_states.dtype == torch.float32)


def _norm_mlp_tail(norm_2, mlp, hidden_states, shift, scale, gate, fused=None, pb=None, in_epilogue=False):
    if _fast_tail(norm_2, mlp, hidden_states):
        from . import native
        B, L, H = hidden_states.shape
        x, res = (hidden_states, None) if fused is None else (fused, None if in_epilogue else hidden_states)
        s3 = getattr(mlp, "_fused", False) and gemm.split3_enabled(hidden_states, _mlp_in_weight(mlp), producer="norm")
        y, _, _, hnew = native.layer_norm_fwd(x.reshape(B * L, H), norm_2.weight, norm_2.bias, norm_2.eps,
                                              residual=None if res is None else res.reshape(B * L, H), is_rms_norm=True, x_bias=pb,
                                              mod_scale=scale, mod_shift=shift, rows_per_batch=L, **({"split3": s3} if s3 else {}))
        if s3 and hnew.is_contiguous():
            return mlp.forward_deferred(hidden_states, x3=y, residual=hnew.view(B, L, H), gate=gate)[0]
        m, mb = mlp.forward_deferred(hidden_states, x3=y) if s3 else mlp.forward_deferred(y.view(B, L, H))
        return token_ops.gate_residual(hnew.view(B, L, H), m, gate, mb)
    if fused is not None:
        hidden_states = token_ops.gate_residual(hidden_states, fused, None, pb)
    if isinstance(norm_2, RMSNorm) and hidden_states.is_cuda and torch.is_grad_enabled():
        normed, hidden_states = norm_2(hidden_states, prenorm=True)
        return _mlp_tail(mlp, hidden_states, normed, shift, scale, gate)
    return _mlp_tail(mlp, hidden_states, norm_2(hidden_states), shift, scale, gate)


def _mix_through_images(mixer, hidden_states, kind, table, shift, scale, c, fork=False):
    if getattr(mixer, "takes_image", lambda: False)() and gemm.split3_enabled(hidden_states, mixer.in_proj.weight, left=False):
        m = mixer(None, c, x3=token_ops.pre_mixer(hidden_states, kind, table, shift, scale,
                                                  split3=gemm.split3_enabled(hidden_states, mixer.in_proj.weight, left=False)))
        return (m, hidden_states) if fork else m
    if fork and hidden_states.is_cuda and torch.is_grad_enabled() and hidden_states.requires_grad:
        t, hidden_states = token_ops.pre_mixer_fork(hidden_states, kind, table, shift, scale)
        return mixer(t, c), hidden_states
    m = mixer(token_ops.pre_mixer(hidden_states, kind, table, shift, scale), c)
    return (m, hidden_states) if fork else m


class _BlockBase(nn.Module):

    def _prenorm(self, hidden_states, residual):
        if not self.fused_add_norm:
            residual = hidden_states if residual is None else residual + self.drop_path(hidden_states)
            hidden_states = (self.norm(residual) if isinstance(self.norm, nn.Identity)
                             else self.norm(residual.to(dtype=self.norm.weight.dtype)))
            if self.residual_in_fp32:
                residual = residual.to(torch.float32)
            return hidden_states, residual
        fn = rms_norm_fn if isinstance(self.norm, RMSNorm) else layer_norm_fn
        x = hidden_states if residual is None else self.drop_path(hidden_states)
        return fn(x, self.norm.weight, self.norm.bias, residual=residual, prenorm=True,
                  residual_in_fp32=self.residual_in_fp32, eps=self.norm.eps)

    def _table(self, L, device, build):
        cache = self.__dict__.setdefault("_tables", {})
        key = (L, str(device))
        if key not in cache:
            fwd = build(math.isqrt(L))
            mixer = getattr(self, "mixer", None)
            if mixer is not None and getattr(mixer, "_is_zigzag", lambda: False)() and getattr(mixer, "zigzag_paths", None) is not None \
                    and os.environ.get("DIMSUM_FOLD_ZIGZAG", "1") != "0":
                perm = mixer.zigzag_paths[mixer.layer_idx].detach().cpu().numpy().astype(np.int64)
                assert perm.shape[0] == L, "zigzag path length != sequence length"
                fwd = perm if fwd is None else so.compose(fwd, perm)
                mixer._zigzag_folded = True
            if fwd is None:
                cache[key] = None
            else:
                inv = so.reverse_permut_np(fwd)
                cache[key] = {"fwd": so.as_index(fwd, device), "inv": so.as_index(inv, device),
                              "inv32": torch.as_tensor(inv.astype(np.int32), device=device)}
        return cache[key]

    def allocate_inference_cache(self, *a, **k):
        raise NotImplementedError("allocate_inference_cache: " + _NOT_CAUSAL)


class DiMBlockRaw(_BlockBase):

    def __init__(self, dim, mixer_cls, norm_cls=nn.LayerNorm, fused_add_norm=False, residual_in_fp32=False, drop_path=0.0,
                 reverse=False, transpose=False, scanning_continuity=False, c_dim=None):
        super().__init__()
        self.residual_in_fp32, self.fused_add_norm = residual_in_fp32, fused_add_norm
        self.reverse, self.transpose, self.scanning_continuity = reverse, transpose, scanning_continuity
        c_dim = dim if c_dim is None else c_dim
        self.mixer = mixer_cls(dim)
        self.norm = norm_cls(dim)
        self.drop_path = DropPath(drop_path) if drop_path > 0.0 else nn.Identity()
        self.adaLN_modulation = nn.Sequential(nn.SiLU(), nn.Linear(c_dim, 3 * dim, bias=True))

    def _order(self, H):
        if not (self.reverse or self.transpose or self.scanning_continuity):
            return None
        return so.block_order_table(H, self.reverse, self.transpose, self.scanning_continuity)

    def forward(self, hidden_states, residual=None, c=None, inference_params=None, out_split3=False):
        _refuse_cache(inference_params)
        hidden_states, residual = self._prenorm(hidden_states, residual)
        table = self._table(hidden_states.shape[1], hidden_states.device, self._order)
        shift, scale, gate = _modulation(self.adaLN_modulation, c).chunk(3, dim=1)
        m, hidden_states = _mix_through_images(self.mixer, hidden_states, "none", table, shift, scale, c, fork=True)
        return token_ops.post_mixer(hidden_states, m, gate, "none", table, **({"split3": out_split3} if out_split3 else {})), residual


class DiMBlock(_BlockBase):

    def __init__(self, dim, mixer_cls, norm_cls=nn.LayerNorm, fused_add_norm=False, residual_in_fp32=False, drop_path=0.0,
                 reverse=False, transpose=False, scanning_continuity=False, skip=False, use_gated_mlp=True):
        super().__init__()
        self.residual_in_fp32, self.fused_add_norm = residual_in_fp32, fused_add_norm
        self.reverse, self.transpose, self.scanning_continuity = reverse, transpose, scanning_continuity
        self.mixer = mixer_cls(dim)
        self.norm = norm_cls(dim)
        self.norm_2 = norm_cls(dim)
        self.drop_path = DropPath(drop_path) if drop_path > 0.0 else nn.Identity()
        self.adaLN_modulation = nn.Sequential(nn.SiLU(), nn.Linear(dim, 6 * dim, bias=True))
        self.mlp = _make_mlp(dim)

    def _order(self, H):
        if not (self.reverse or self.transpose or self.scanning_continuity):
            return None
        return so.block_order_table(H, self.reverse, self.transpose, self.scanning_continuity)

    def forward(self, hidden_states, residual=None, c=None, inference_params=None):
        _refuse_cache(inference_params)
        hidden_states, residual = self._prenorm(hidden_states, residual)
        table = self._table(hidden_states.shape[1], hidden_states.device, self._order)
        shift, scale, gate, shift_mlp, scale_mlp, gate_mlp = _modulation(self.adaLN_modulation, c).chunk(6, dim=1)
        m, hidden_states = _mix_through_images(self.mixer, hidden_states, "none", table, shift, scale, c, fork=True)
        hidden_states = token_ops.post_mixer(hidden_states, m, gate, "none", table)
        return _norm_mlp_tail(self.norm_2, self.mlp, hidden_states, shift_mlp, scale_mlp, gate_mlp), residual


class DiMBlockWindow(DiMBlock):

    def __init__(self, dim, mixer_cls, norm_cls=nn.LayerNorm, fused_add_norm=False, residual_in_fp32=False, drop_path=0.0,
                 reverse=False, transpose=False, scanning_continuity=False, skip=False, shift_window=False):
        super().__init__(dim, mixer_cls, norm_cls=norm_cls, fused_add_norm=fused_add_norm, residual_in_fp32=residual_in_fp32,
                         drop_path=drop_path, reverse=reverse, transpose=transpose, scanning_continuity=scanning_continuity, skip=skip)
        self.shift_window = shift_window

    def _order(self, H):
        if H % 4:
            raise NotImplementedError("DiMBlockWindow: the reference zero-pads a token grid that 4x4 windows do not tile "
                                      "(scanning_orders.py:358-360), which lengthens the sequence -- not a token permutation")
        tab = so.local_scan_table(H, 4, column_first=bool(self.transpose))
        if self.shift_window:
            tab = so.compose(tab, np.roll(np.arange(H * H).reshape(H, H), (-1, -1), axis=(0, 1)).reshape(-1))
        return tab[::-1].copy() if self.reverse else tab


class _FreqBlock(_BlockBase):
    kind = "none"

    def _init_common(self, dim, mixer_cls, norm_cls, fused_add_norm, residual_in_fp32, drop_path, reverse, transpose,
                     scanning_continuity, no_ffn, c_dim):
        self.residual_in_fp32, self.fused_add_norm = residual_in_fp32, fused_add_norm
        self.reverse, self.transpose, self.scanning_continuity, self.no_ffn = reverse, transpose, scanning_continuity, no_ffn
        self._c_dim = dim if c_dim is None else c_dim

    def _finish_common(self, dim, norm_cls, drop_path):
        self.drop_path = DropPath(drop_path) if drop_path > 0.0 else nn.Identity()
        self.adaLN_modulation = nn.Sequential(nn.SiLU(), nn.Linear(self._c_dim, 6 * dim if not self.no_ffn else 3 * dim, bias=True))
        if not self.no_ffn:
            self.norm_2 = norm_cls(dim)
            self.mlp = _make_mlp(dim)

    def forward(self, hidden_states, residual=None, c=None, inference_params=None, out_split3=False):
        _refuse_cache(inference_params)
        hidden_states, residual = self._prenorm(hidden_states, residual)
        table = self._table(hidden_states.shape[1], hidden_states.device, self._order)
        mods = _modulation(self.adaLN_modulation, c).chunk(3 if self.no_ffn else 6, dim=1)
        shift, scale, gate = mods[:3]
        if self.no_ffn:
            m, hidden_states = _mix_through_images(self.mixer, hidden_states, self.kind, table, shift, scale, c, fork=True)
            return token_ops.post_mixer(hidden_states, m, gate, self.kind, table, **({"split3": out_split3} if out_split3 else {})), residual
        assert not out_split3
        t = token_ops.pre_mixer(hidden_states, self.kind, table, torch.zeros_like(shift), torch.zeros_like(scale))
        t = t + gate.unsqueeze(1) * self.mixer(modulate(t, shift, scale), c)
        t = t + mods[5].unsqueeze(1) * self.mlp(modulate(self.norm_2(t), mods[3], mods[4]))
        zero = torch.zeros_like(hidden_states)
        return token_ops.post_mixer(zero, t, torch.ones_like(gate), self.kind, table), residual


class WaveDiMBlock(_FreqBlock):
    kind = "haar"

    def __init__(self, dim, mixer_cls, norm_cls=nn.LayerNorm, fused_add_norm=False, residual_in_fp32=False, drop_path=0.0,
                 reverse=False, transpose=False, scanning_continuity=False, skip=False, no_ffn=False, c_dim=None,
                 window_scan=True, num_wavelet_lv=2):
        super().__init__()
        assert num_wavelet_lv == 2, "only the two-level transform of the published configs is implemented"
        self._init_common(dim, mixer_cls, norm_cls, fused_add_norm, residual_in_fp32, drop_path, reverse, transpose,
                          scanning_continuity, no_ffn, c_dim)
        self.window_scan, self.num_wavelet_lv = window_scan, num_wavelet_lv
        self.mixer = mixer_cls(dim)
        self.norm = norm_cls(dim)
        self.dwt, self.idwt = DWT_2D(wave="haar"), IDWT_2D(wave="haar")
        self._finish_common(dim, norm_cls, drop_path)

    def _order(self, H):
        if self.window_scan:
            tab = so.local_scan_table(H, H // 4, column_first=bool(self.transpose))
        else:
            tab = so.block_order_table(H, False, self.transpose, False)
        return so.compose(tab, so.block_order_table(H, self.reverse, False, self.scanning_continuity))


class DCTBlock(_FreqBlock):
    kind = "dct"

    def __init__(self, dim, mixer_cls, fused_add_norm=False, residual_in_fp32=False, drop_path=0.0, norm_cls=nn.LayerNorm,
                 dct_size=2, reverse=False, transpose=False, scanning_continuity=False, no_ffn=False, c_dim=None):
        super().__init__()
        assert dct_size == 4, "only the 4x4 DCT of DiMBlockCombinedFourier is implemented"
        self._init_common(dim, mixer_cls, norm_cls, fused_add_norm, residual_in_fp32, drop_path, reverse, transpose,
                          scanning_continuity, no_ffn, c_dim)
        self.dim, self.dct_size, self.reserve_kernel = dim, dct_size, dct_size
        self.norm = norm_cls(dim)
        self.mixer = mixer_cls(dim)
        self._finish_common(dim, norm_cls, drop_path)
        self.dct_conv = init_dct_kernel(dim, dct_size, dct_size)
        self.idct_conv = nn.Sequential(init_idct_kernel(dim, dct_size, dct_size), nn.PixelShuffle(dct_size))

    def _order(self, H):
        if not (self.reverse or self.transpose or self.scanning_continuity):
            return None
        return so.block_order_table(H, self.reverse, self.transpose, self.scanning_continuity)


class _ForkHalves(torch.autograd.Function):

    @staticmethod
    def forward(ctx, h):
        C = h.shape[-1] // 2
        return h[..., :C], h[..., C:], h.view_as(h)

    @staticmethod
    def backward(ctx, d1, d2, dres):
        if dres is None:
            return torch.cat((d1, d2), dim=-1)
        C = dres.shape[-1] // 2
        out = torch.empty(dres.shape, device=dres.device, dtype=dres.dtype)
        for d, sl in ((d1, slice(0, C)), (d2, slice(C, 2 * C))):
            if d is None:
                out[..., sl] = dres[..., sl]
            else:
                torch.add(d, dres[..., sl], out=out[..., sl])
        return out


class _CombinedBase(_BlockBase):
    _branch_images = True

    def _freq(self, x2, c, inference_params, kw):
        return self.freq_mamba(x2, None, c, inference_params, **kw)[0]

    def _init_tail(self, dim, norm_cls, drop_path, use_gated_mlp, swap_k_kw):
        self.proj = CrossAttentionFusion(dim, num_heads=8, qkv_bias=True, **swap_k_kw)
        self.drop_path = DropPath(drop_path) if drop_path > 0.0 else nn.Identity()
        self.norm_2 = norm_cls(dim)
        self.adaLN_modulation = nn.Sequential(nn.SiLU(), nn.Linear(dim, 3 * dim, bias=True))
        self.mlp = _make_mlp(dim, use_gated_mlp)

    def forward(self, hidden_states, residual=None, c=None, inference_params=None):
        _refuse_cache(inference_params)
        hidden_states, residual = self._prenorm(hidden_states, residual)
        if hidden_states.is_cuda and torch.is_grad_enabled() and hidden_states.requires_grad:
            x1, x2, hidden_states = _ForkHalves.apply(hidden_states)
        else:
            x1, x2 = hidden_states.chunk(2, dim=2)
        img = self._branch_images and self.proj.takes_images(hidden_states) and gemm.split3_enabled(x1, self.proj.qkv1.weight)
        kw = {"out_split3": img} if img else {}
        if ((not torch.is_grad_enabled()) and hidden_states.is_cuda and branch_streams_enabled()
                and not torch.cuda.is_current_stream_capturing()):
            cur = torch.cuda.current_stream(hidden_states.device)
            side = self.__dict__.get("_side_stream")
            if side is None or side.device != hidden_states.device:
                side = self.__dict__["_side_stream"] = torch.cuda.Stream(device=hidden_states.device)
            side.wait_stream(cur)
            with torch.cuda.stream(side):
                x2 = self._freq(x2, c, inference_params, kw)
            x1, _ = self.spatial_mamba(x1, None, c, inference_params, **kw)
            cur.wait_stream(side)
            x2.record_stream(cur)
        else:
            x1, _ = self.spatial_mamba(x1, None, c, inference_params, **kw)
            x2 = self._freq(x2, c, inference_params, kw)
        fast_tail = _fast_tail(self.norm_2, self.mlp, hidden_states)
        in_epilogue = bool(img) and fast_tail and hidden_states.is_contiguous()
        fused, pb = self.proj.forward_deferred(x1, x2, **({"images": True} if img else {}), **({"residual": hidden_states} if in_epilogue else {}))
        shift, scale, gate = _modulation(self.adaLN_modulation, c).chunk(3, dim=1)
        return _norm_mlp_tail(self.norm_2, self.mlp, hidden_states, shift, scale, gate, fused, pb, in_epilogue), residual


class DiMBlockCombined(_CombinedBase):

    def __init__(self, dim, mixer_cls, norm_cls=nn.LayerNorm, fused_add_norm=False, residual_in_fp32=False, drop_path=0.0,
                 reverse=False, transpose=False, scanning_continuity=False, use_gated_mlp=True):
        super().__init__()
        self.residual_in_fp32, self.fused_add_norm = residual_in_fp32, fused_add_norm
        self.reverse, self.transpose, self.scanning_continuity = reverse, transpose, scanning_continuity
        self.norm = norm_cls(dim)
        kw = dict(norm_cls=nn.Identity, drop_path=0.0, fused_add_norm=False, residual_in_fp32=residual_in_fp32,
                  scanning_continuity=scanning_continuity, c_dim=dim)
        self.spatial_mamba = DiMBlockRaw(dim // 2, mixer_cls, reverse=reverse, transpose=transpose, **kw)
        self.freq_mamba = WaveDiMBlock(dim // 2, mixer_cls, reverse=False, transpose=reverse, no_ffn=True, num_wavelet_lv=2, **kw)
        self._init_tail(dim, norm_cls, drop_path, use_gated_mlp, dict(swap_k=False))


class DiMBlockCombinedFourier(_CombinedBase):

    def __init__(self, dim, mixer_cls, mixer_cls_2, norm_cls=nn.LayerNorm, fused_add_norm=False, residual_in_fp32=False,
                 drop_path=0.0, reverse=False, transpose=False, scanning_continuity=False, use_gated_mlp=True):
        super().__init__()
        self.residual_in_fp32, self.fused_add_norm = residual_in_fp32, fused_add_norm
        self.reverse, self.transpose, self.scanning_continuity = reverse, transpose, scanning_continuity
        self.norm = norm_cls(dim)
        kw = dict(norm_cls=nn.Identity, drop_path=0.0, fused_add_norm=False, residual_in_fp32=residual_in_fp32,
                  scanning_continuity=scanning_continuity, c_dim=dim)
        self.spatial_mamba = DiMBlockRaw(dim // 2, mixer_cls, reverse=reverse, transpose=transpose, **kw)
        self.freq_mamba = DCTBlock(dim // 2, mixer_cls_2, reverse=False, transpose=False, no_ffn=True, dct_size=4, **kw)
        self._init_tail(dim, norm_cls, drop_path, use_gated_mlp, {})


class EinFFT(nn.Module):

    def __init__(self, dim):
        super().__init__()
        from . import native
        if dim % native.EINFFT_CHANNEL_GRANULE or not 0 < dim <= native.EINFFT_MAX_CHANNELS:
            raise NotImplementedError(f"block_type='combined_einfft': the spectral branch's width must be a multiple of "
                                      f"{native.EINFFT_CHANNEL_GRANULE}, at most {native.EINFFT_MAX_CHANNELS} (got {dim}: hidden size {2 * dim})")
        self.hidden_size, self.num_blocks, self.block_size = dim, 4, dim // 4
        self.sparsity_threshold, self.scale = 0.01, 0.02
        shape = (2, self.num_blocks, self.block_size)
        self.complex_weight_1 = nn.Parameter(torch.randn(*shape, self.block_size, dtype=torch.float32) * self.scale)
        self.complex_weight_2 = nn.Parameter(torch.randn(*shape, self.block_size, dtype=torch.float32) * self.scale)
        self.complex_bias_1 = nn.Parameter(torch.randn(*shape, dtype=torch.float32) * self.scale)
        self.complex_bias_2 = nn.Parameter(torch.randn(*shape, dtype=torch.float32) * self.scale)

    def forward(self, x):
        from .ops.einfft import einfft
        return einfft(x, self.complex_weight_1, self.complex_bias_1, self.complex_weight_2, self.complex_bias_2, self.sparsity_threshold)
# ... 323 lines not shown
```

dimsum_amd/native.py:

```python
import contextlib

import os

import torch

from . import _lib

_DT = {torch.float32: _lib.F32, torch.float16: _lib.F16, torch.bfloat16: _lib.BF16}


class _ZeroArena:
    CHUNK = 1 << 22

    def __init__(self):
        import threading
        self._lock, self._cur = threading.Lock(), {}

    def take(self, n, device):
        n = int(n)
        if n <= 0 or n > self.CHUNK // 4 or torch.cuda.is_current_stream_capturing() or os.environ.get("DIMSUM_ZERO_ARENA", "1") == "0":
            return torch.zeros(max(n, 0), device=device, dtype=torch.float32)
        pad = (n + 63) // 64 * 64
        key = (str(device), torch.cuda.current_stream(device).cuda_stream)
        with self._lock:
# ... 634 lines not shown
    M, V = logits.shape
    _check(tuple(dloss.shape) == (M,) and dloss.dtype == torch.float32 and dloss.stride(0) >= 0, "cross_entropy_bwd: dloss must be (rows,) float32")
    _check(tuple(lse.shape) == (M,) and lse.dtype == torch.float64, "cross_entropy_bwd: lse must be (rows,) float64, as cross_entropy_fwd returns it")
    _gpu(dloss, logits, lse, labels)
    labels, lse = labels.contiguous(), lse.contiguous()
    dlogits = logits if inplace else torch.empty((M, V), device=logits.device, dtype=logits.dtype)
    P.dlogits_row_stride, P.dloss_stride = max(dlogits.stride(0), V), dloss.stride(0)
    P.logits_ptr, P.labels_ptr, P.lse_ptr, P.dloss_ptr, P.dlogits_ptr = _ptr(logits), _ptr(labels), _ptr(lse), _ptr(dloss), _ptr(dlogits)
    with torch.cuda.device(logits.device):
        _lib.check(_lib.load().dimsum_cross_entropy_bwd(P, _stream(logits)), "cross_entropy_bwd")
    return dlogits


def sample_logits(logits, u, top_k=1, top_p=0.0, temperature=1.0, out=None, row_index=None, out_table=None):
    _check(logits.dim() == 2 and logits.dtype in _DT and logits.shape[0] >= 1 and logits.shape[1] >= 1,
           "sample_logits: logits must be (rows >= 1, vocab >= 1) in float32, float16 or bfloat16")
    M, V = logits.shape
    _check(logits.stride(1) == 1 and (M == 1 or logits.stride(0) >= V),
           "sample_logits: logits must have unit column stride and a row stride >= vocab (a [..., :vocab] view of a padded buffer is fine)")
    temperature = float(temperature)
    _check(temperature > 0.0 and temperature != float("inf"), "sample_logits: temperature must be finite and > 0")
    top_k = int(top_k)
    _check(-2 ** 31 <= top_k < 2 ** 31, "sample_logits: top_k must fit 32 bits")
    steps = 0
    if row_index is not None:
        _check(row_index.dtype == torch.int64 and row_index.numel() == 1, "sample_logits: row_index must be one int64 on the device")
        _check(u is not None and u.dim() == 2, "sample_logits: with row_index, u must be (steps, rows)")
        steps = u.shape[0]
    else:
        _check(out_table is None, "sample_logits: out_table needs row_index")
    if u is not None:
        _check(u.dtype == torch.float32 and u.is_contiguous() and tuple(u.shape) == ((steps, M) if row_index is not None else (M,)),
               "sample_logits: u must be contiguous float32, (rows,) or with row_index (steps, rows)")
    else:
        _check(top_k == 1, "sample_logits: only top_k == 1 draws nothing: u is required")
    if out_table is not None:
        _check(out_table.dtype == torch.int64 and out_table.is_contiguous() and tuple(out_table.shape) == (steps, M),
               "sample_logits: out_table must be contiguous int64 (steps, rows), as u")
    if out is None:
        out = torch.empty(M, device=logits.device, dtype=torch.int64)
    else:
        _check(out.dtype == torch.int64 and out.numel() == M and out.is_contiguous(), "sample_logits: out must be contiguous int64 with one element per row")
    _gpu(logits, u, out, row_index, out_table)
    P = _lib.SampleLogitsParams()
    P.dtype, P.rows, P.vocab, P.logits_row_stride = _DT[logits.dtype], M, V, max(logits.stride(0), V)
    P.top_k, P.top_p, P.temperature, P.table_steps = top_k, float(top_p), temperature, steps
    P.logits_ptr, P.u_ptr, P.out_ptr, P.row_index_ptr, P.out_table_ptr = _ptr(logits), _ptr(u), _ptr(out), _ptr(row_index), _ptr(out_table)
    with torch.cuda.device(logits.device):
        _lib.check(_lib.load().dimsum_sample_logits(P, _stream(logits)), "sample_logits")
    return out


def layer_norm_fwd(x, weight, bias, eps, residual=None, out_dtype=None, residual_dtype=None, is_rms_norm=False,
                   x_bias=None, mod_scale=None, mod_shift=None, rows_per_batch=0, split3=False):
    _gpu(x, weight, bias, residual)
    _check(x.dim() == 2 and x.stride(-1) == 1, "layer_norm_fwd: x must be (M, N) with contiguous rows")
    M, N = x.shape
    _check(tuple(weight.shape) == (N,), "layer_norm_fwd: weight must be (N,)")
    if residual is not None:
        _check(residual.shape == x.shape and residual.stride(-1) == 1, "layer_norm_fwd: bad residual")
        residual_dtype = residual.dtype
    y_inv = None
    if split3 == "f16s":
        _check(N % 4 == 0, "layer_norm_fwd: the f16s image needs N % 4 == 0")
        y = torch.empty((M, N), device=x.device, dtype=torch.float16)
        y_inv = torch.empty((M,), device=x.device, dtype=torch.float32)
    elif split3:
        _check(N % 4 == 0 and out_dtype in (None, torch.bfloat16), "layer_norm_fwd: split3 needs N % 4 == 0 (bfloat16 output)")
        y = torch.empty((M, (2 if split3 == "pair" else 3) * N), device=x.device, dtype=torch.bfloat16)
    else:
        y = torch.empty((M, N), device=x.device, dtype=x.dtype if out_dtype is None else out_dtype)
    need_res_out = residual is not None or x_bias is not None or (residual_dtype is not None and residual_dtype != x.dtype)
    if residual_dtype is None:
        residual_dtype = x.dtype
    residual_out = torch.empty((M, N), device=x.device, dtype=residual_dtype) if need_res_out else None
    mean = torch.empty((M,), device=x.device, dtype=torch.float32) if not is_rms_norm else None
    rstd = torch.empty((M,), device=x.device, dtype=torch.float32)
    if M > 0:
        P = _lib.NormParams()
        P.rows, P.cols, P.is_rms_norm, P.eps = M, N, int(is_rms_norm), float(eps)
        P.x_dtype, P.out_dtype, P.y_split3 = _DT[x.dtype], _DT[y.dtype], _SPLIT_MODE.get(split3, int(bool(split3)))
        P.y_inv_scale_ptr = _ptr(y_inv)
        P.residual_dtype = _DT[residual_out.dtype] if residual_out is not None else _DT[x.dtype]
        P.x_row_stride, P.y_row_stride = x.stride(0), y.stride(0)
        if residual is not None:
            P.residual_row_stride = residual.stride(0)
        if residual_out is not None:
            P.residual_out_row_stride = residual_out.stride(0)
        w32 = weight.float().contiguous()
        b32 = bias.float().contiguous() if bias is not None else None
        P.x_ptr, P.residual_ptr, P.weight_ptr, P.bias_ptr = _ptr(x), _ptr(residual), _ptr(w32), _ptr(b32)
        P.y_ptr, P.residual_out_ptr, P.mean_ptr, P.rstd_ptr = _ptr(y), _ptr(residual_out), _ptr(mean), _ptr(rstd)
        if x_bias is not None:
            xb32 = x_bias.float().contiguous()
            _check(tuple(xb32.shape) == (N,), "layer_norm_fwd: x_bias must be (N,)")
            P.xbias_ptr = _ptr(xb32)
        if mod_scale is not None:
            _gpu(mod_scale, mod_shift)
            _check(mod_shift is not None and rows_per_batch > 0 and M % rows_per_batch == 0, "layer_norm_fwd: bad modulation arguments")
            nb = M // rows_per_batch
            _check(tuple(mod_scale.shape) == (nb, N) and tuple(mod_shift.shape) == (nb, N) and mod_scale.dtype == torch.float32
                   and mod_shift.dtype == torch.float32 and mod_scale.stride(1) == 1 and mod_shift.stride(1) == 1
                   and mod_scale.stride(0) == mod_shift.stride(0), "layer_norm_fwd: mod_scale / mod_shift must be (M / rows_per_batch, N) float32 sharing a row stride")
            P.mod_scale_ptr, P.mod_shift_ptr, P.mod_row_stride, P.rows_per_batch = _ptr(mod_scale), _ptr(mod_shift), mod_scale.stride(0), rows_per_batch
        with torch.cuda.device(x.device):
            _lib.check(_lib.load().dimsum_norm_fwd(P, _stream(x)), "layer_norm_fwd")
    if y_inv is not None:
        y = F16Image(y, y_inv)
    elif split3 == "pair":
        y = PairImage(y)
    return y, mean, rstd, residual_out if residual_out is not None else x


def layer_norm_bwd(dy, x, weight, bias, eps, mean, rstd, dresidual=None, has_residual=False, is_rms_norm=False, x_dtype=None):
    _gpu(dy, x, weight, rstd, dresidual)
    M, N = x.shape
    xf = x if x.dtype == torch.float32 else x.float()
    dyf = dy if dy.dtype == torch.float32 else dy.float()
    drf = None if dresidual is None else (dresidual if dresidual.dtype == torch.float32 else dresidual.float())
    dx32 = torch.empty((M, N), device=x.device, dtype=torch.float32)
    acc = _zeros(2 * N if bias is not None else N, x.device)
    dw = acc[:N]
    db = acc[N:] if bias is not None else None
    if M > 0:
        P = _lib.NormBwdParams()
        P.rows, P.cols, P.is_rms_norm, P.eps = M, N, int(is_rms_norm), float(eps)
        P.r_row_stride, P.dy_row_stride, P.dx_row_stride = xf.stride(0), dyf.stride(0), dx32.stride(0)
        if drf is not None:
            P.dres_row_stride = drf.stride(0)
        w32 = weight.float().contiguous()
        P.r_ptr, P.weight_ptr, P.mean_ptr, P.rstd_ptr = _ptr(xf), _ptr(w32), _ptr(mean), _ptr(rstd)
        P.dy_ptr, P.dres_ptr, P.dx_ptr, P.dweight_ptr, P.dbias_ptr = _ptr(dyf), _ptr(drf), _ptr(dx32), _ptr(dw), _ptr(db)
        with torch.cuda.device(x.device):
            _lib.check(_lib.load().dimsum_norm_bwd(P, _stream(x)), "layer_norm_bwd")
    x_dtype = x_dtype or x.dtype
    dx = dx32 if x_dtype == torch.float32 else dx32.to(x_dtype)
    dresidual_in = None
# ... 364 lines not shown
    _check_ssm(u, delta, A, B, C, D, z, delta_bias)
    _check_bidir(A, A_b, z)
    batch, dim, seqlen = u.shape
    dstate = A.shape[1]
    _check(dstate in (4, 8, 16, 32), "selective_scan_bidir: dstate must be 4, 8, 16 or 32")
    out = torch.empty_like(delta) if need_out else None
    out_b = torch.empty_like(delta) if need_out else None
    out_z = torch.empty_like(z)
    ckpt = torch.empty(scan_ckpt_shape(batch, dim, seqlen, dstate), device=u.device, dtype=torch.float32) if need_ckpt else None
    ckpt_b = torch.empty_like(ckpt) if need_ckpt else None
    if u.numel() > 0:
        P = _lib.SsmBidirParams()
        _fill_ssm(P.fwd, u, delta, A, B, C, D, z, delta_bias, delta_softplus, out, None, out_z, ckpt)
        _fill_ssm_reversed(P, A_b, out_b, ckpt_b)
        with torch.cuda.device(u.device):
            _lib.check(_lib.load().dimsum_ssm_scan_bidir_fwd(P, _stream(u)), "selective_scan_bidir_fwd")
    res = [out, out_b, out_z]
    if need_ckpt:
        res += [ckpt, ckpt_b]
    return res


def selective_scan_bidir_bwd(u, delta, A, A_b, B, C, D, z, delta_bias, dout, out, out_b, ckpt, ckpt_b, delta_softplus, recompute_out_z,
                             dz=None, dB=None, dC=None):
    _check_ssm(u, delta, A, B, C, D, z, delta_bias)
    _check_bidir(A, A_b, z)
    _gpu(dout, out, out_b, ckpt, ckpt_b, dz)
    batch, dim, seqlen = u.shape
    also = [(t is not None and t.shape == u.shape and t.dtype == u.dtype and t.stride(-1) == 1,
             "selective_scan_bidir_bwd: `out` and `out_b` of the forward are required") for t in (out, out_b)]
    also += [(t is not None and tuple(t.shape) == scan_ckpt_shape(batch, dim, seqlen, A.shape[1]) and t.dtype == torch.float32 and t.is_contiguous(),
              "selective_scan_bidir_bwd: both directions' saved states (need_ckpt=True) are required") for t in (ckpt, ckpt_b)]
    du, ddelta, (dA, dA_b), dB, dC, dD, ddelta_bias, dz = _prep_ssm_bwd("selective_scan_bidir_bwd", u, delta, A, B, C, D, z, delta_bias, dout, dz, dB, dC, 2, also)
    out_z = torch.empty_like(out) if recompute_out_z else None
    if u.numel() > 0:
        P = _lib.SsmBidirBwdParams()
        _fill_ssm(P.bwd.fwd, u, delta, A, B, C, D, z, delta_bias, delta_softplus, out, None, out_z, ckpt)
        ws = _fill_ssm_bwd(P.bwd, dout, du, ddelta, dA, dB, dC, dD, ddelta_bias, dz, ckpt)
        _fill_ssm_reversed(P, A_b, out_b, ckpt_b)
        P.dA_b_ptr, P.dA_b_d_stride, P.dA_b_dstate_stride = _ptr(dA_b), dA_b.stride(0), dA_b.stride(1)
        with torch.cuda.device(u.device):
            _lib.check(_lib.load().dimsum_ssm_scan_bidir_bwd(P, _stream(u)), "selective_scan_bidir_bwd")
        del ws
    res = [du, ddelta, dA, dA_b, dB.to(B.dtype), dC.to(C.dtype), dD, ddelta_bias, dz]
    if out_z is not None:
        res.append(out_z)
    return res


_TT_KIND = {("none", True): 0, ("none", False): 0, ("haar", True): 1, ("haar", False): 2, ("dct", True): 3, ("dct", False): 4}


def token_transform(x, kind, forward, in_index=None, out_index=None, gate=None, scale=None, shift=None, residual=None,
                    w=None, want_y=True, want_wsum=False, want_tsum=False, split3=False):
    _gpu(x, in_index, out_index, gate, scale, shift, residual, w)
    _check(x.dim() == 3 and x.dtype == torch.float32 and x.stride(2) == 1, "token_transform: x must be (B, L, C) float32, channel-contiguous")
    B, L, C = x.shape
    grid = int(round(L ** 0.5))
    if kind != "none":
        _check(grid * grid == L and grid % 4 == 0, "token_transform: the token grid must be square with side % 4 == 0")
    _check(want_y or w is not None or want_tsum, "token_transform: nothing to compute")
    y_inv = None
    if split3 == "f16s":
        _check(want_y and C % 4 == 0 and C <= (2048 if kind == "none" else 1024) and w is None and not want_tsum,
               "token_transform: the f16s image needs channels % 4 == 0, <= 1024 (2048 without a transform), no reductions")
        y = torch.empty((B, L, C), device=x.device, dtype=torch.float16)
        y_inv = torch.empty((B, L), device=x.device, dtype=torch.float32)
    elif split3:
        _check(want_y and C % 4 == 0, "token_transform: split3 needs an output and channels % 4 == 0")
        y = torch.empty((B, L, (2 if split3 == "pair" else 3) * C), device=x.device, dtype=torch.bfloat16)
    else:
        y = torch.empty((B, L, C), device=x.device, dtype=torch.float32) if want_y else None
    mods = [m for m in (gate, scale, shift) if m is not None]
    mstride = 0
    for m in mods:
        _check(m.dtype == torch.float32 and tuple(m.shape) == (B, C) and m.stride(1) == 1, "token_transform: gate/scale/shift must be (B, C) float32")
        _check(mstride in (0, m.stride(0)), "token_transform: gate/scale/shift must share one row stride")
        mstride = m.stride(0)
    for t in (in_index, out_index):
        if t is not None:
            _check(t.dtype == torch.int32 and t.numel() == L and t.is_contiguous(), "token_transform: index tables must be int32 (L,)")
    if residual is not None:
        _check(residual.shape == x.shape and residual.dtype == torch.float32 and residual.stride(2) == 1, "token_transform: bad residual")
    wdot = wsum = tsum = None
    if w is not None:
        _check(w.shape == x.shape and w.dtype == torch.float32 and w.stride(2) == 1, "token_transform: bad w")
    if w is not None or want_tsum:
        red = _zeros(3 * B * C, x.device).view(3, B, C)
        wdot, wsum = (red[0] if w is not None else None), (red[1] if (w is not None and want_wsum) else None)
        tsum = red[2] if want_tsum else None
    if B > 0:
        P = _lib.TtParams()
        P.batch, P.tokens, P.channels, P.grid, P.kind = B, L, C, grid, _TT_KIND[(kind, bool(forward))]
        P.y_split3 = _SPLIT_MODE.get(split3, int(bool(split3)))
        P.y_inv_scale_ptr = _ptr(y_inv)
        P.x_batch_stride, P.x_token_stride = x.stride(0), x.stride(1)
        if y is not None:
            P.y_batch_stride, P.y_token_stride = y.stride(0), y.stride(1)
        if residual is not None:
            P.res_batch_stride, P.res_token_stride = residual.stride(0), residual.stride(1)
        P.red_batch_stride = C
        if w is not None:
            P.w_batch_stride, P.w_token_stride = w.stride(0), w.stride(1)
        P.mod_batch_stride = mstride
        P.x_ptr, P.in_index_ptr, P.out_index_ptr = _ptr(x), _ptr(in_index), _ptr(out_index)
        P.gate_ptr, P.scale_ptr, P.shift_ptr, P.residual_ptr, P.y_ptr = _ptr(gate), _ptr(scale), _ptr(shift), _ptr(residual), _ptr(y)
        P.w_ptr, P.wdot_ptr, P.wsum_ptr, P.tsum_ptr = _ptr(w), _ptr(wdot), _ptr(wsum), _ptr(tsum)
        with torch.cuda.device(x.device):
            _lib.check(_lib.load().dimsum_token_transform(P, _stream(x)), "token_transform")
    if y_inv is not None:
        return F16Image(y, y_inv)
    if split3 == "pair":
        y = PairImage(y)
    if want_tsum:
        return (y, wdot, wsum, tsum)
    return y if w is None else (y, wdot, wsum)


def _act_out(lead, H, split3, device, n_dbias=0):
    inv = None
    if split3 == "f16s":
        out = torch.empty(lead + (H,), device=device, dtype=torch.float16)
        inv = torch.empty(lead, device=device, dtype=torch.float32)
    elif split3:
        out = torch.empty(lead + ((2 if split3 == "pair" else 3) * H,), device=device, dtype=torch.bfloat16)
    else:
        out = torch.empty(lead + (H,), device=device, dtype=torch.float32)
    return out, inv, (_zeros(n_dbias, device) if n_dbias else None)


def _act_image(out, inv, split3):
    return F16Image(out, inv) if split3 == "f16s" else PairImage(out) if split3 == "pair" else out


def gated_gelu_fwd(x12, bias=None, split3=False):
    _gpu(x12, bias)
    _check(x12.dtype == torch.float32 and x12.is_contiguous() and x12.shape[-1] % 8 == 0, "gated_gelu: x12 must be contiguous float32 with 2H % 8 == 0")
    H = x12.shape[-1] // 2
    if bias is not None:
        _check(bias.dtype == torch.float32 and tuple(bias.shape) == (2 * H,) and bias.is_contiguous(), "gated_gelu: bias must be (2H,) float32")
    h = _act_out(x12.shape[:-1], H, bool(split3), x12.device)[0]
    rows = x12.numel() // (2 * H)
    fn = _lib.load().dimsum_gated_gelu_fwd_split3 if split3 else _lib.load().dimsum_gated_gelu_fwd
    with torch.cuda.device(x12.device):
        _lib.check(fn(_ptr(x12), _ptr(bias), _ptr(h), rows, H, _stream(x12)), "gated_gelu_fwd")
    return h


def gated_gelu_bwd(x12, bias, dh, need_dbias=True, split3=False):
    _gpu(x12, bias, dh)
    dh = dh.contiguous()
    H = x12.shape[-1] // 2
    split3 = split3 if split3 in ("pair", "f16s") else bool(split3)
    f16s = split3 == "f16s"
    _check(not f16s or (x12.is_contiguous() and x12.dtype == torch.float32 and dh.dtype == torch.float32 and H % 4 == 0 and H <= 5120), "gated_gelu_bwd: the f16s image needs contiguous float32 rows, H % 4 == 0, H <= 5120")
    dx12, inv, dbias = _act_out(x12.shape[:-1], 2 * H, split3, x12.device, 2 * H if (bias is not None and need_dbias) else 0)
    lib = _lib.load()
    fn = {False: lib.dimsum_gated_gelu_bwd, True: lib.dimsum_gated_gelu_bwd_split3, "pair": lib.dimsum_gated_gelu_bwd_pair, "f16s": lib.dimsum_gated_gelu_bwd_f16s}[split3]
    with torch.cuda.device(x12.device):
        _lib.check(fn(_ptr(x12), _ptr(bias), _ptr(dh), _ptr(dx12), *((_ptr(inv),) if f16s else ()), _ptr(dbias), x12.numel() // (2 * H), H, _stream(x12)), "gated_gelu_bwd")
# ... 503 lines not shown
    if row_scales is not None:
        ext.update(k_scale_ptr=_ptr(row_scales[0]), c_scale_ptr=_ptr(row_scales[1]))
    if row_invs is not None:
        ext.update(k_inv_a_ptr=_ptr(row_invs[0]), k_inv_b_ptr=_ptr(row_invs[1]))
    G = _lib.GemmParams()
    _fill_gemm(G, a, b, out, P, Q, R, scales=scales or (None, None), events=events, **ext)
    with torch.cuda.device(a.device):
        _lib.check(_lib.load().dimsum_gemm_tn(G, splits, P * Q, _stream(a)), "gemm_tn")
    return out[0] if splits == 1 else out.sum(0)


_gemm_kernel_log = None


@contextlib.contextmanager
def gemm_kernel_log():
    global _gemm_kernel_log
    old, _gemm_kernel_log = _gemm_kernel_log, []
    try:
        yield _gemm_kernel_log
    finally:
        _gemm_kernel_log = old


def gemm_nn_supported(a, b):
    if not (_gemm_operands_ok(a, b) and a.dtype == torch.float16):
        return False
    P, R = a.shape
    Q = b.shape[1]
    return (b.shape[0] == R and R % 64 == 0 and R >= 128 and P % 256 == 0 and Q % 256 == 0
            and 256 * a.stride(0) * 2 < 2 ** 31 and 64 * b.stride(0) * 2 + 512 < 2 ** 31)


def gemm_nn(a, a_inv, b, b_inv, splits=None):
    _gpu(a, a_inv, b, b_inv)
    _check(gemm_nn_supported(a, b) and a_inv.dtype == torch.float32 and a_inv.numel() == a.shape[0] and a_inv.is_contiguous()
           and b_inv.dtype == torch.float32 and b_inv.numel() == b.shape[0], "gemm_nn: unsupported operands")
    P, R = a.shape
    Q = b.shape[1]
    if splits is None:
        splits = _rowfac_splits(R, P, Q)
    _check(splits >= 1 and R % (splits * 64) == 0 and 128 <= R // splits <= 16384, "gemm_nn: splits must cut R into ranges of 2 .. 256 whole 64-row tiles")
    in_kernel = os.environ.get("DIMSUM_ROW_FACTORS_KERNEL", "0") != "1" and b_inv.is_contiguous()
    fac, top = (None, None) if in_kernel else row_factors(b_inv)
    out = torch.empty((splits, P, Q), device=a.device, dtype=torch.float32)
    G = _lib.GemmParams()
    _fill_gemm(G, a, b, out, P, Q, R, scales=(a_inv, None), **(dict(k_inv_a_ptr=_ptr(b_inv)) if in_kernel else dict(k_scale_ptr=_ptr(fac), c_scale_ptr=_ptr(top))))
    with torch.cuda.device(a.device):
        _lib.check(_lib.load().dimsum_gemm_nn(G, splits, P * Q, _stream(a)), "gemm_nn")
    return out[0] if splits == 1 else out.sum(0)


def gemm_nt(a, b, bias=None, epilogue="f32", out=None, out_scale=1.0, events=None, tune=None, scales=None, gate_bound=None, residual=None,
            gate=None, rows_per_batch=None, keep_x12=False, pair_out=False, weight_order=False, q_cols=None, conv=None):
    pair_in = isinstance(a, PairImage)
    pair_b = isinstance(b, PairImage)
    if pair_in:
        a = a.data
    if pair_b:
        b = b.data
    _gpu(a, b, bias)
    gated = epilogue in ("gated_split3", "gated_f16")
    _check(not (pair_in and pair_b) and not (pair_b and (gated or residual is not None or bias is not None)), "gemm_nt: a right-hand pair goes with the plain fp32 epilogue")
    _check(gemm_nt_supported(a, b, gated, pair=pair_in, pair_b=pair_b), "gemm_nt: unsupported operands (M % 256, K % 64, K >= 128, 16-bit K-contiguous rows, 16-byte aligned)")
    M, K = a.shape[0], (a.shape[1] if pair_b else b.shape[1])
    N = b.shape[0]
    ext = {}
    if pair_in:
        ext.update(a_alias_rows=K // 3, a_alias_weight_order=int(bool(weight_order)))
    if pair_b:
        ext.update(b_alias_rows=K // 3)
    if bias is not None:
        _check(bias.dtype == torch.float32 and bias.is_contiguous() and bias.numel() == N, "gemm_nt: bias must be (N,) float32")
    if epilogue == "f32":
        epi = _lib.GEMM_EPI_F32 if bias is None else _lib.GEMM_EPI_F32_BIAS
        if out is None:
            out = torch.empty((M, N), device=a.device, dtype=torch.float32)
        _check(out.dtype == torch.float32 and out.shape == (M, N) and out.stride(1) == 1, "gemm_nt: out must be (M, N) float32 rows")
        if conv is not None:
            cw, cb, seq = conv
            _gpu(cw, cb)
            _check(bias is None and residual is None and cw.dtype == torch.float32 and cw.dim() == 2 and cw.stride(1) == 1 and cw.shape[0] % 256 == 0
                   and cw.shape[0] <= M and 2 <= cw.shape[1] <= 4 and 256 % seq == 0 and seq % 4 == 0 and N % seq == 0
                   and (cb is None or (cb.dtype == torch.float32 and cb.is_contiguous() and cb.numel() == cw.shape[0])),
                   "gemm_nt: conv = (weight (rows % 256 == 0, width 2..4) f32, bias or None, seq with 256 % seq == 0)")
            epi = _lib.GEMM_EPI_F32_CONV
            ext.update(conv_weight_ptr=_ptr(cw), conv_bias_ptr=_ptr(cb), conv_rows=cw.shape[0], conv_width=cw.shape[1], conv_seq=seq, conv_weight_ld=cw.stride(0))
        if residual is not None:
            _gpu(residual, gate)
            _check(residual.dtype == torch.float32 and residual.shape == (M, N) and residual.stride(1) == 1, "gemm_nt: residual must be (M, N) float32 rows")
            epi = _lib.GEMM_EPI_F32_GATE_RESIDUAL
            ext.update(residual_ptr=_ptr(residual), residual_ld=residual.stride(0))
            if gate is not None:
                _check(rows_per_batch and rows_per_batch % 256 == 0 and M % rows_per_batch == 0 and gate.dtype == torch.float32
                       and gate.shape == (M // rows_per_batch, N) and gate.stride(1) == 1, "gemm_nt: gate must be (M / rows_per_batch, N) float32, rows_per_batch % 256 == 0")
                ext.update(gate_ptr=_ptr(gate), gate_ld=gate.stride(0), rows_per_batch=rows_per_batch)
    elif epilogue == "gated_split3":
        epi = _lib.GEMM_EPI_GATED_GELU_SPLIT3
        pieces = 2 if pair_out else 3
        ext.update(c_image_pieces=pieces)
        if out is None:
            out = torch.empty((M, pieces * (N // 2)), device=a.device, dtype=torch.bfloat16)
        _check(out.dtype == torch.bfloat16 and out.shape == (M, pieces * (N // 2)) and out.stride(1) == 1, "gemm_nt: out must be (M, 3F) / (M, 2F) bfloat16 rows")
    elif epilogue == "f16_qkv":
        epi = _lib.GEMM_EPI_F16_QKV
        _check(scales is not None and gate_bound is not None and rows_per_batch and rows_per_batch % 256 == 0 and M % rows_per_batch == 0
               and q_cols and q_cols % 16 == 0 and N % 8 == 0, "gemm_nt: f16_qkv needs scales, gate_bound = {wl1, bmax}, rows_per_batch % 256 == 0, q_cols % 16 == 0")
        ext.update(rows_per_batch=rows_per_batch, qkv_q_cols=q_cols)
        if out is None:
            out = torch.empty((M, N), device=a.device, dtype=torch.float16)
        _check(out.dtype == torch.float16 and out.shape == (M, N) and out.stride(1) == 1, "gemm_nt: out must be (M, N) float16 rows")
    elif epilogue == "gelu_f16":
        epi = _lib.GEMM_EPI_GELU_F16
        _check(scales is not None and gate_bound is not None and N % 8 == 0, "gemm_nt: gelu_f16 needs scales, gate_bound = {wl1, bmax} and N % 8 == 0")
        if out is None:
            out = torch.empty((M, N), device=a.device, dtype=torch.float16)
        _check(out.dtype == torch.float16 and out.shape == (M, N) and out.stride(1) == 1, "gemm_nt: out must be (M, N) float16 rows")
    elif epilogue == "gated_f16":
        epi = _lib.GEMM_EPI_GATED_GELU_F16
        if out is None:
            out = torch.empty((M, N // 2), device=a.device, dtype=torch.float16)
        _check(out.dtype == torch.float16 and out.shape == (M, N // 2) and out.stride(1) == 1, "gemm_nt: out must be (M, F) float16 rows")
    else:
        raise ValueError(f"gemm_nt: unknown epilogue {epilogue!r}")
    h_inv = None
    if scales is not None:
        sa, sb = scales
        _gpu(sa, sb)
        _check(sa.dtype == torch.float32 and sb.dtype == torch.float32 and sa.is_contiguous() and sb.is_contiguous() and sa.numel() == M
               and sb.numel() == N, "gemm_nt: scales must be contiguous float32 (M,) and (N,)")
        if gate_bound is not None:
            _gpu(gate_bound)
            _check(epilogue in ("gated_f16", "f16_qkv", "gelu_f16") and gate_bound.dtype == torch.float32 and gate_bound.numel() == 2 and gate_bound.is_contiguous(),
                   "gemm_nt: gate_bound is a 2-element float32 tensor for the gated_f16 / f16_qkv / gelu_f16 epilogues")
            ext.update(gate_bound_ptr=_ptr(gate_bound))
            if epilogue in ("gated_f16", "gelu_f16"):
                h_inv = torch.empty((M,), device=a.device, dtype=torch.float32)
                ext.update(h_inv_scale_ptr=_ptr(h_inv))
    x12 = None
    if keep_x12:
        _check((epilogue == "gated_split3" and a.dtype == torch.bfloat16 and scales is None) or (epilogue == "gated_f16" and a.dtype == torch.float16 and h_inv is not None),
               "gemm_nt: keep_x12 goes with the gated_split3 epilogue over bf16 images or the gated_f16 epilogue over scaled-fp16 operands with gate_bound")
        x12 = torch.empty((M, N), device=a.device, dtype=torch.float32)
        ext.update(x12_ptr=_ptr(x12), x12_ld=N)
    if tune is not None:
# ... 526 lines not shown
```

dimsum_amd/ops/token_ops.py:

```python
import math

import torch

_S = [q % 4 * 4 + q // 4 for q in range(16)]


def reorder(x, table):
    return x if table is None else x.index_select(1, table)


def modulate(x, shift, scale):
    return x * (1 + scale.unsqueeze(1)) + shift.unsqueeze(1)


def _dwt_level(img):
    a, b = img[:, :, 0::2, 0::2], img[:, :, 0::2, 1::2]
    c, d = img[:, :, 1::2, 0::2], img[:, :, 1::2, 1::2]
    p, q, r, s = a + b, a - b, c + d, c - d
    return torch.cat([(p + r) * 0.5, (p - r) * 0.5, (q + s) * 0.5, (q - s) * 0.5], dim=1)


def _idwt_level(sub):
    B, C4, H, W = sub.shape
    C = C4 // 4
# ... 136 lines not shown
    @staticmethod
    def backward(ctx, dy):
        from .. import native
        m, gate = ctx.saved_tensors
        dy = _cc(dy)
        k = 1.0 / _ADJ[ctx.kind]
        dm, dot, _ = native.token_transform(dy, ctx.kind, True, out_index=ctx.inv32, scale=gate * k - 1.0, w=m)
        return dy, dm, dot * k, None, None


class _GateResidual(torch.autograd.Function):

    @staticmethod
    def forward(ctx, res, m, gate, bias):
        from .. import native
        res, m = _cc(res), _cc(m)
        B, _, C = m.shape
        shift, g = None, gate
        if bias is not None and gate is None:
            shift = bias.float().expand(B, C)
        elif bias is not None:
            gs = torch.cat((gate, gate * bias.float()), dim=1)
            g, shift = gs[:, :C], gs[:, C:]
        ctx.save_for_backward(m, gate, bias)
        return native.token_transform(m, "none", False, gate=g, shift=shift, residual=res)

    @staticmethod
    def backward(ctx, dy):
        from .. import native
        m, gate, bias = ctx.saved_tensors
        dy = _cc(dy)
        need_m, need_gate, need_bias = ctx.needs_input_grad[1], gate is not None and ctx.needs_input_grad[2], bias is not None and ctx.needs_input_grad[3]
        dm = dgate = dbias = None
        if gate is None:
            dm = dy if need_m else None
            if need_bias:
                dbias = native.token_transform(dy, "none", True, want_y=False, want_tsum=True)[3].sum(0)
        else:
            dm, dot, _, tsum = native.token_transform(dy, "none", True, scale=gate - 1.0, w=m, want_y=need_m, want_tsum=True)
            if need_gate:
                dgate = dot if bias is None else dot + tsum * bias.float()
            if need_bias:
                dbias = (gate * tsum).sum(0)
        if dbias is not None:
            dbias = dbias.to(bias.dtype)
        return dy, dm, dgate, dbias


def gate_residual(res, m, gate=None, bias=None):
    _require_gpu(res)
    return _GateResidual.apply(res, m, gate, bias)


def pre_mixer(x, kind, table, shift, scale, split3=False):
    _require_gpu(x)
    if split3:
        from .. import native
        return native.token_transform(_cc(x), kind, True, out_index=None if table is None else table["inv32"], scale=scale, shift=shift, split3=split3)
    return _PreMixer.apply(x, shift, scale, kind, None if table is None else table["inv32"])


def pre_mixer_fork(x, kind, table, shift, scale):
    _require_gpu(x)
    return _PreMixerFork.apply(x, shift, scale, kind, None if table is None else table["inv32"])


def post_mixer(x, m, gate, kind, table, split3=False):
    _require_gpu(x)
    if split3:
        from .. import native
        return native.token_transform(_cc(m), kind, False, in_index=None if table is None else table["inv32"], gate=gate, residual=_cc(x), split3=split3)
    return _PostMixer.apply(x, m, gate, kind, None if table is None else table["inv32"])
```

include/dimsum_hip.h:

```cpp
#ifndef DIMSUM_HIP_H
#define DIMSUM_HIP_H

#include <stdint.h>

#ifdef __cplusplus
extern "C" {
#endif

#define DIMSUM_ABI_VERSION 18

typedef enum {
    DIMSUM_OK = 0,
    DIMSUM_ERR_NULL = 1,
    DIMSUM_ERR_DTYPE = 2,
    DIMSUM_ERR_SHAPE = 3,
    DIMSUM_ERR_STRIDE = 4,
    DIMSUM_ERR_UNSUPPORTED = 5,
    DIMSUM_ERR_LAUNCH = 6,
    DIMSUM_ERR_ABI = 7,
    DIMSUM_ERR_ALIAS = 8
} dimsum_status_t;

typedef enum { DIMSUM_F32 = 0, DIMSUM_F16 = 1, DIMSUM_BF16 = 2 } dimsum_dtype_t;

// ... 600 lines not shown
    const void *dres_ptr;
    void *dx_ptr;
    void *dweight_ptr, *dbias_ptr;
} dimsum_norm_bwd_params_t;

int dimsum_norm_fwd(const dimsum_norm_params_t *p, void *stream);
int dimsum_norm_bwd(const dimsum_norm_bwd_params_t *p, void *stream);

int dimsum_split3(const void *src, int64_t rows, int64_t cols, int64_t src_row_stride, void *dst, int32_t left, void *stream);
int dimsum_split3_t(const void *src, int64_t rows, int64_t cols, int64_t src_row_stride, void *dst, void *stream);

int dimsum_rows_f16s(const void *src, int64_t rows, int64_t cols, int64_t src_row_stride, void *dst, int64_t dst_row_stride,
                     void *inv_scale, void *l1max, void *stream);

int dimsum_rows_block_f16s(const void *src, int64_t rows, int64_t cols, int64_t src_row_stride, void *dst, int64_t dst_row_stride, void *table,
                           int64_t table_ld, void *stream);

typedef struct {
    const void *src;
    void *dst;
    void *inv_scale_ptr;
    void *l1max_ptr;
    void *absmax_ptr;
    int64_t rows, cols, src_row_stride, dst_row_stride;
    float l1_factor;
    int32_t reserved;
} dimsum_f16s_job_t;
int dimsum_rows_f16s_multi(const dimsum_f16s_job_t *jobs, int32_t n_jobs, void *stream);

typedef enum {
    DIMSUM_TT_NONE = 0, DIMSUM_TT_HAAR_FWD = 1, DIMSUM_TT_HAAR_INV = 2, DIMSUM_TT_DCT_FWD = 3, DIMSUM_TT_DCT_INV = 4
} dimsum_tt_kind_t;

typedef struct {
    uint32_t struct_size;
    int32_t batch, tokens, channels, grid;
    int32_t kind;
    int32_t y_split3;
    int64_t x_batch_stride, x_token_stride;
    int64_t res_batch_stride, res_token_stride;
    int64_t y_batch_stride, y_token_stride;
    int64_t mod_batch_stride;
    int64_t w_batch_stride, w_token_stride;
    int64_t red_batch_stride;
    const void *x_ptr;
    const int32_t *in_index_ptr, *out_index_ptr;
    const void *gate_ptr, *scale_ptr, *shift_ptr, *residual_ptr;
    void *y_ptr;
    const void *w_ptr;
    void *wdot_ptr, *wsum_ptr;
    void *tsum_ptr;
    void *y_inv_scale_ptr;
    int32_t y_f16s_lds_offset;
    int32_t reserved;
} dimsum_tt_params_t;

int dimsum_token_transform(const dimsum_tt_params_t *p, void *stream);

typedef struct {
    uint32_t struct_size;
    int32_t batch, seqlen, heads, head_dim;
    float scale;
    int32_t n_dirs;
    int64_t qkv_batch_stride, qkv_token_stride;
    int64_t out_batch_stride, out_token_stride;
    const void *qkv1_ptr, *qkv2_ptr;
    void *out_ptr, *lse_ptr;
    const void *bias1_ptr, *bias2_ptr;
    int32_t precision;
    int32_t out_split3;
    const void *x1_inv_ptr, *x2_inv_ptr, *kv_bound_ptr;
    void *out_inv_ptr;
    int32_t qkv_f16;
    int32_t reserved2;
} dimsum_xattn_params_t;

int dimsum_xattn_fusion_fwd(const dimsum_xattn_params_t *p, void *stream);

typedef struct {
    uint32_t struct_size;
    uint32_t reserved;
    dimsum_xattn_params_t fwd;
    int64_t dqkv_batch_stride, dqkv_token_stride;
    const void *dout_ptr;
    void *dqkv1_ptr, *dqkv2_ptr, *delta_ptr;
} dimsum_xattn_bwd_params_t;

int dimsum_xattn_fusion_bwd(const dimsum_xattn_bwd_params_t *p, void *stream);

int dimsum_gated_gelu_fwd(const void *x12, const void *bias, void *h, int64_t rows, int64_t hidden, void *stream);
int dimsum_gated_gelu_fwd_split3(const void *x12, const void *bias, void *h3, int64_t rows, int64_t hidden, void *stream);
int dimsum_gated_gelu_bwd(const void *x12, const void *bias, const void *dh, void *dx12, void *dbias, int64_t rows,
                          int64_t hidden, void *stream);
int dimsum_gated_gelu_bwd_split3(const void *x12, const void *bias, const void *dh, void *dx12_image, void *dbias, int64_t rows,
                                 int64_t hidden, void *stream);
int dimsum_gated_gelu_bwd_pair(const void *x12, const void *bias, const void *dh, void *dx12_pair, void *dbias, int64_t rows, int64_t hidden, void *stream);
int dimsum_gated_gelu_bwd_f16s(const void *x12, const void *bias, const void *dh, void *dx12_image, void *inv_scale, void *dbias, int64_t rows,
                               int64_t hidden, void *stream);

typedef enum { DIMSUM_GELU_OUT_F32 = 0, DIMSUM_GELU_OUT_SPLIT3 = 1, DIMSUM_GELU_OUT_PAIR = 2, DIMSUM_GELU_OUT_F16S = 3 } dimsum_gelu_out_t;

typedef struct {
    uint32_t struct_size;
    int32_t reserved;
    const void *row_inv_ptr, *bound_ptr;
} dimsum_gelu_ext_t;

// ... 123 lines not shown
    int64_t rows, hidden;
    const void *src_ptr, *perm_ptr;
    void *dst_ptr, *inv_scale_ptr;
    const dimsum_moe_ext_t *ext;
} dimsum_moe_permute_f16s_params_t;

typedef struct {
    uint32_t struct_size;
    int32_t gated;
    int32_t num_experts;
    int32_t reserved;
    int64_t rows, width;
    const void *x_ptr, *bias_ptr, *row_expert_ptr;
    void *out_ptr, *inv_scale_ptr;
    const dimsum_moe_ext_t *ext;
} dimsum_moe_act_f16s_params_t;

int dimsum_moe_gemm_f16s(const dimsum_moe_gemm_f16s_params_t *p, void *stream);
int dimsum_moe_permute_f16s(const dimsum_moe_permute_f16s_params_t *p, void *stream);
int dimsum_moe_act_fwd_f16s(const dimsum_moe_act_f16s_params_t *p, void *stream);

typedef enum {
    DIMSUM_GEMM_EPI_F32 = 0, DIMSUM_GEMM_EPI_GATED_GELU_SPLIT3 = 1, DIMSUM_GEMM_EPI_GATED_GELU_F16 = 2, DIMSUM_GEMM_EPI_F32_BIAS = 3,
    DIMSUM_GEMM_EPI_F32_GATE_RESIDUAL = 4,
    DIMSUM_GEMM_EPI_F32_CONV = 6,
    DIMSUM_GEMM_EPI_F16_QKV = 5,
    DIMSUM_GEMM_EPI_GELU_F16 = 7
} dimsum_gemm_epilogue_t;

typedef struct {
    uint32_t struct_size;
    int32_t rows_per_batch;
    void *timing_start_event, *timing_stop_event;
    int32_t tune_variant, tune_group_m, tune_reserved;
    int32_t c_image_pieces;
    const void *gate_bound_ptr;
    void *h_inv_scale_ptr;
    const void *residual_ptr, *gate_ptr;
    int64_t residual_ld, gate_ld;
    void *x12_ptr;
    int64_t x12_ld;
    int64_t a_alias_rows;
    int64_t b_alias_rows;
    int32_t a_alias_weight_order, qkv_q_cols;
    const void *conv_weight_ptr, *conv_bias_ptr;
    int32_t conv_rows, conv_width, conv_seq, conv_weight_ld;
    const void *a_block_inv_ptr;
    int64_t a_block_inv_ld;
    int64_t tn_pair_a_cols, tn_pair_b_cols;
    const void *k_scale_ptr;
    const void *c_scale_ptr;
    const void *k_inv_a_ptr;
    const void *k_inv_b_ptr;
} dimsum_gemm_ext_t;

typedef struct {
    uint32_t struct_size;
    int32_t m, n, k;
    int32_t operand_dtype;
    int32_t epilogue;
    float out_scale;
    int32_t reserved;
    int64_t lda, ldb, ldc;
    const void *a_ptr, *b_ptr, *bias_ptr;
    void *c_ptr;
    const void *a_inv_scale_ptr;
    const void *b_inv_scale_ptr;
    const dimsum_gemm_ext_t *ext;
} dimsum_gemm_params_t;

int dimsum_gemm_nt(const dimsum_gemm_params_t *p, void *stream);
int dimsum_gemm_nt_kernel_for(const dimsum_gemm_params_t *p);

int dimsum_gemm_tn(const dimsum_gemm_params_t *p, int32_t splits, int64_t c_split_stride, void *stream);

int dimsum_gemm_nn(const dimsum_gemm_params_t *p, int32_t splits, int64_t c_split_stride, void *stream);
int dimsum_row_factors(const void *a_inv, const void *b_inv, int64_t n, void *k_scale, void *c_scale, void *stream);

#ifdef __cplusplus
}
#endif
#endif
```

Baseline: 3495 latents/s.

## Fold RMSNorm scaling into token-transform and GEMM residual epilogue

The prenorm RMSNorm pass now computes only per-row rstd instead of writing a normalized tensor. The rstd and weight multiply is applied where the normalized values are consumed: the pre- and post-mixer token transforms and the proj GEMM residual epilogue. This removes a full-tensor write and re-read per block. In exchange the epilogues do extra loads, the GEMM residual epilogue uses a smaller residual group size, and the folded GEMM path skips the persistent kernel variant.

New measurement: 3530 latents/s (median of 6 runs). +1.0%, better.

```diff
diff --git a/dimsum_amd/_lib.py b/dimsum_amd/_lib.py
--- a/dimsum_amd/_lib.py
+++ b/dimsum_amd/_lib.py
@@ -311,7 +311,7 @@
                                       "w_token_stride", "red_batch_stride")]
                 + [(n, vp) for n in ("x_ptr", "in_index_ptr", "out_index_ptr", "gate_ptr", "scale_ptr", "shift_ptr",
                                      "residual_ptr", "y_ptr", "w_ptr", "wdot_ptr", "wsum_ptr", "tsum_ptr", "y_inv_scale_ptr")]
-                + [("y_f16s_lds_offset", i32), ("reserved", i32)])
+                + [("y_f16s_lds_offset", i32), ("norm_fold", i32), ("norm_rstd_ptr", vp), ("norm_weight_ptr", vp)])
 
 
 class XattnParams(_Sized):
@@ -335,7 +335,8 @@
                    ("a_alias_weight_order", i32), ("qkv_q_cols", i32), ("conv_weight_ptr", vp), ("conv_bias_ptr", vp),
                    ("conv_rows", i32), ("conv_width", i32), ("conv_seq", i32), ("conv_weight_ld", i32),
                    ("a_block_inv_ptr", vp), ("a_block_inv_ld", i64), ("tn_pair_a_cols", i64), ("tn_pair_b_cols", i64),
-                   ("k_scale_ptr", vp), ("c_scale_ptr", vp), ("k_inv_a_ptr", vp), ("k_inv_b_ptr", vp)])
+                   ("k_scale_ptr", vp), ("c_scale_ptr", vp), ("k_inv_a_ptr", vp), ("k_inv_b_ptr", vp),
+                   ("res_rstd_ptr", vp), ("res_weight_ptr", vp)])
 
 
 class GemmParams(_Sized):
diff --git a/dimsum_amd/attention_fusion.py b/dimsum_amd/attention_fusion.py
--- a/dimsum_amd/attention_fusion.py
+++ b/dimsum_amd/attention_fusion.py
@@ -60,7 +60,7 @@
     def takes_images(self, ref):
         return self._plain and not (self.training and (self.attn_drop.p > 0.0 or self.proj_drop.p > 0.0)) and native.xattn_supported(ref, self.head_dim)
 
-    def forward_deferred(self, x1, x2, images=False, residual=None):
+    def forward_deferred(self, x1, x2, images=False, residual=None, residual_norm=None):
         if images:
             B, N, C3 = x1.shape
             b1, b2 = self.qkv1.bias, self.qkv2.bias
@@ -84,7 +84,7 @@
                 f3 = native.xattn_fusion_fwd(qkv1, qkv2, self.num_heads, split_bf16=True, split3="pair" if isinstance(x1, native.PairImage) else True)
             if residual is not None:
                 pb = None if self.proj.bias is None else self.proj.bias.float()
-                y = gemm.linear_split3(f3.reshape(B * N, -1), self.proj.weight, bias=pb, residual=residual.reshape(B * N, -1))
+                y = gemm.linear_split3(f3.reshape(B * N, -1), self.proj.weight, bias=pb, residual=residual.reshape(B * N, -1), residual_norm=residual_norm)
                 return y.view(residual.shape), None
             return gemm.linear_split3(f3.reshape(B * N, -1), self.proj.weight).view(B, N, -1), self.proj.bias
         B, N, C = x1.shape
diff --git a/dimsum_amd/csrc/gemm_nt.hip b/dimsum_amd/csrc/gemm_nt.hip
--- a/dimsum_amd/csrc/gemm_nt.hip
+++ b/dimsum_amd/csrc/gemm_nt.hip
@@ -176,6 +176,14 @@
         a.gate = reinterpret_cast<const float *>(p.gate_ptr);
         a.ldr = p.residual_ld; a.ldg = p.gate_ld;
         a.rows_per_batch = p.gate_ptr ? p.rows_per_batch : p.m;
+        if (p.res_rstd_ptr || p.res_weight_ptr) {
+            if (!p.res_rstd_ptr || !p.res_weight_ptr) return DIMSUM_ERR_NULL;
+            if (!aligned_to<char>(p.res_weight_ptr, 16) || !aligned_to<char>(p.res_rstd_ptr, 4)) return DIMSUM_ERR_STRIDE;
+            if (bf || m128 || p.tune_variant == 514) return DIMSUM_ERR_UNSUPPORTED;
+            a.res_rstd = reinterpret_cast<const float *>(p.res_rstd_ptr);
+            a.res_w = reinterpret_cast<const float *>(p.res_weight_ptr);
+            return launch<kOpF16, kEpiF32GateResNorm, kShip>(a, w);
+        }
         if (persist_ok(a, p.epilogue, bf, p.tune_variant)) return launch_persist<kOpF16, kEpiF32GateRes, kShip>(a, w);
         return bf ? launch<kOpBf16, kEpiF32GateRes, kShip>(a, w) : launch_f16<kEpiF32GateRes, kShip>(a, w, m128);
     }
diff --git a/dimsum_amd/csrc/gemm_nt_kernel.hpp b/dimsum_amd/csrc/gemm_nt_kernel.hpp
--- a/dimsum_amd/csrc/gemm_nt_kernel.hpp
+++ b/dimsum_amd/csrc/gemm_nt_kernel.hpp
@@ -18,7 +18,7 @@
 constexpr int kSlotA0 = 0, kSlotA1 = kHalf, kSlotB0 = 2 * kHalf, kSlotB1 = 3 * kHalf;
 
 enum { kOpBf16 = 0, kOpF16 = 1 };
-enum { kEpiF32 = 0, kEpiGatedSplit3 = 1, kEpiGatedF16 = 2, kEpiF32Bias = 3, kEpiF32GateRes = 4, kEpiF16Qkv = 5, kEpiF32Conv = 6, kEpiGeluF16 = 7 };
+enum { kEpiF32 = 0, kEpiGatedSplit3 = 1, kEpiGatedF16 = 2, kEpiF32Bias = 3, kEpiF32GateRes = 4, kEpiF16Qkv = 5, kEpiF32Conv = 6, kEpiGeluF16 = 7, kEpiF32GateResNorm = 8 };
 
 struct Args {
     const char *A, *B0, *B1;
@@ -28,6 +28,7 @@
     const float *gate_bound;
     float *inv_out;
     const float *res, *gate;
+    const float *res_rstd, *res_w;
     int64_t ldr, ldg;
     int rows_per_batch;
     int64_t lda, ldb, ldc;
@@ -635,7 +636,10 @@
                 for (int i = 0; i < 4; ++i)
 #pragma unroll
                     for (int j = 0; j < 2; ++j) asm volatile("" ::"v"(acc[mi][ni][i][j]));
-    } else if constexpr (kEpi == kEpiF32 || kEpi == kEpiF32Bias || kEpi == kEpiF32GateRes || kEpi == kEpiF32Conv) {
+    } else if constexpr (kEpi == kEpiF32 || kEpi == kEpiF32Bias || kEpi == kEpiF32GateRes || kEpi == kEpiF32GateResNorm || kEpi == kEpiF32Conv) {
+        constexpr bool kResNorm = kEpi == kEpiF32GateResNorm;
+        constexpr bool kGateRes = kEpi == kEpiF32GateRes || kResNorm;
+        static_assert(!kResNorm || (!kPersist && !kM1 && (kVar & kVarFullLineStores)), "the folded norm is built on the 256-row per-tile kernel");
         if constexpr (kEpi == kEpiF32Conv) {
             if (m0 < p.conv_rows) {
                 constexpr int kNW = kM1 ? 4 : 8;
@@ -725,14 +729,15 @@
             float c_scale = 1.0f;
             if constexpr (kRowFac) c_scale = p.k_inv_a ? c_scale_own : *p.c_scale;
             bool live[2];
-            f4 bv[2], sbv[2], gv[2];
+            f4 bv[2], sbv[2], gv[2], nwv[2];
             auto load_cols = [&](int ni) {
                 const int col = ni * 128 + fcol;
                 live[ni] = n0 + col < p.N;
                 const int lc = live[ni] ? n0 + col : 0;
                 bv[ni] = f4{0.f, 0.f, 0.f, 0.f}; sbv[ni] = gv[ni] = f4{1.f, 1.f, 1.f, 1.f};
                 if constexpr (kEpi == kEpiF32Bias) bv[ni] = *reinterpret_cast<const f4 *>(p.bias0 + lc);
-                if constexpr (kEpi == kEpiF32GateRes) {
+                if constexpr (kResNorm) nwv[ni] = *reinterpret_cast<const f4 *>(p.res_w + lc);
+                if constexpr (kGateRes) {
                     bv[ni] = pick(pick_mask(p.bias0 != nullptr), *reinterpret_cast<const f4 *>((p.bias0 ? p.bias0 : reinterpret_cast<const float *>(p.B0)) + lc), bv[ni]);
                     gv[ni] = pick(pick_mask(p.gate != nullptr),
                                   *reinterpret_cast<const f4 *>((p.gate ? p.gate + (int64_t)(m0 / p.rows_per_batch) * p.ldg : reinterpret_cast<const float *>(p.B0)) + lc), gv[ni]);
@@ -742,7 +747,7 @@
             load_cols(0);
             live[1] = n0 + 128 + fcol < p.N;
             float rs[2][4][2];
-            if constexpr (!kPersist || kRebase || kEpi != kEpiF32GateRes)
+            if constexpr (!kPersist || kRebase || !kGateRes)
 #pragma unroll
             for (int mi = 0; mi < 2; ++mi)
 #pragma unroll
@@ -756,11 +761,11 @@
                         rs[mi][i][0] = pick(ms, sap[lrow], 1.0f); rs[mi][i][1] = pick(ms, sap[lrow + 8], 1.0f);
                     }
                 }
-            constexpr int kGS = kPersist ? DIMSUM_PERSIST_GS : 4, kNG = 16 / kGS;
+            constexpr int kGS = kPersist ? DIMSUM_PERSIST_GS : (kResNorm ? 2 : 4), kNG = 16 / kGS;
             f4 rr[2][kGS][2];
-            float rg[2][kGS][2];
+            float rg[2][kGS][2], rn[2][kGS][2];
             auto load_res = [&](int g) {
-                if constexpr (kEpi == kEpiF32GateRes) {
+                if constexpr (kGateRes) {
                     const int t0 = g * kGS, ni = t0 >> 3, mi = (t0 >> 2) & 1;
                     if constexpr (kPersist) {
 #pragma unroll
@@ -770,6 +775,13 @@
                         }
                     }
                     const float *rp = p.res + (int64_t)(m0 + frow + mi * kMiRows) * p.ldr + (live[ni] ? n0 + ni * 128 + fcol : 0);
+                    if constexpr (kResNorm) {
+#pragma unroll
+                        for (int k = 0; k < kGS; ++k) {
+                            const int lrow = m0 + frow + mi * kMiRows + ((t0 + k) & 3) * 16;
+                            rn[g & 1][k][0] = p.res_rstd[lrow]; rn[g & 1][k][1] = p.res_rstd[lrow + 8];
+                        }
+                    }
 #pragma unroll
                     for (int k = 0; k < kGS; ++k) {
                         const int i = (t0 + k) & 3;
@@ -797,12 +809,17 @@
                     }
                     const int lrow = frow + mi * kMiRows + i * 16;
                     const unsigned voff = (unsigned)((lrow * p.ldc + col) * 4);
-                    constexpr bool kRowsInGroup = kPersist && kEpi == kEpiF32GateRes;
+                    constexpr bool kRowsInGroup = kPersist && kGateRes;
                     s0 = s0 * (sbv[ni] * (kRowsInGroup ? rg[g & 1][k][0] : rs[mi][i][0]));
                     s1 = s1 * (sbv[ni] * (kRowsInGroup ? rg[g & 1][k][1] : rs[mi][i][1]));
-                    if constexpr (kEpi == kEpiF32GateRes) {
-                        s0 = rr[g & 1][k][0] + gv[ni] * (s0 + bv[ni]);
-                        s1 = rr[g & 1][k][1] + gv[ni] * (s1 + bv[ni]);
+                    if constexpr (kGateRes) {
+                        f4 r0 = rr[g & 1][k][0], r1 = rr[g & 1][k][1];
+                        if constexpr (kResNorm) {
+                            r0 = r0 * rn[g & 1][k][0]; r0 = r0 * nwv[ni]; r0 = r0 + f4{0.f, 0.f, 0.f, 0.f};
+                            r1 = r1 * rn[g & 1][k][1]; r1 = r1 * nwv[ni]; r1 = r1 + f4{0.f, 0.f, 0.f, 0.f};
+                        }
+                        s0 = r0 + gv[ni] * (s0 + bv[ni]);
+                        s1 = r1 + gv[ni] * (s1 + bv[ni]);
                     } else {
                         s0 = s0 + bv[ni];
                         s1 = s1 + bv[ni];
@@ -811,7 +828,7 @@
                         store_f4<kAux>(rsrc, voff, s0);
                         store_f4<kAux>(rsrc, voff + (unsigned)(8 * p.ldc * 4), s1);
                     }
-                    if constexpr (kEpi != kEpiF32GateRes) DIMSUM_PACE_STORES();
+                    if constexpr (!kGateRes) DIMSUM_PACE_STORES();
                 }
             }
         } else {
diff --git a/dimsum_amd/csrc/norm.hip b/dimsum_amd/csrc/norm.hip
--- a/dimsum_amd/csrc/norm.hip
+++ b/dimsum_amd/csrc/norm.hip
@@ -94,6 +94,7 @@
             if (p.rstd_ptr) reinterpret_cast<float *>(p.rstd_ptr)[row] = rstd;
             if (p.mean_ptr && !p.is_rms_norm) reinterpret_cast<float *>(p.mean_ptr)[row] = mean;
         }
+        if (!p.y_ptr) continue;
         float ymax = 0.f;
 #pragma unroll
         for (int i = 0; i < kPieces; ++i) {
@@ -279,7 +280,8 @@
     using namespace dimsum;
     if (!p) return DIMSUM_ERR_NULL;
     if (p->struct_size != sizeof(dimsum_norm_params_t)) return DIMSUM_ERR_ABI;
-    if (!p->x_ptr || !p->weight_ptr || !p->y_ptr) return DIMSUM_ERR_NULL;
+    if (!p->x_ptr || !p->weight_ptr) return DIMSUM_ERR_NULL;
+    if (!p->y_ptr && (!p->rstd_ptr || !p->residual_out_ptr || !p->is_rms_norm || p->y_split3 || p->mod_scale_ptr || p->bias_ptr)) return DIMSUM_ERR_NULL;
     if (p->rows < 0 || p->cols <= 0) return DIMSUM_ERR_SHAPE;
     if ((p->mod_scale_ptr == nullptr) != (p->mod_shift_ptr == nullptr)) return DIMSUM_ERR_NULL;
     if (p->mod_scale_ptr && p->rows_per_batch <= 0) return DIMSUM_ERR_SHAPE;
diff --git a/dimsum_amd/csrc/token_transform.hip b/dimsum_amd/csrc/token_transform.hip
--- a/dimsum_amd/csrc/token_transform.hip
+++ b/dimsum_amd/csrc/token_transform.hip
@@ -77,7 +77,7 @@
     for (int c = 0; c < 4; ++c) dct4(t + c, 4, Y + c, 4, inverse);
 }
 
-template <int KIND, int VEC, bool F16S = false, int kFix = 0>
+template <int KIND, int VEC, bool F16S = false, int kFix = 0, bool kFold = false>
 __global__ __launch_bounds__(kTTThreads) void token_transform_kernel(const dimsum_tt_params_t p) {
     extern __shared__ __attribute__((aligned(16))) float lds[];
     const int tid = threadIdx.x;
@@ -126,6 +126,23 @@
     const float *shift = p.shift_ptr ? reinterpret_cast<const float *>(p.shift_ptr) + (int64_t)b * p.mod_batch_stride : nullptr;
 
     const float *wb = p.w_ptr ? reinterpret_cast<const float *>(p.w_ptr) + (int64_t)b * p.w_batch_stride : nullptr;
+    static_assert(!kFold || ((kFix == 1 || kFix == 2) && VEC == 4 && KIND != DIMSUM_TT_NONE), "norm_fold: the two inference passes around a mixer");
+    const float *nrs = kFold ? reinterpret_cast<const float *>(p.norm_rstd_ptr) + (int64_t)b * p.tokens : nullptr, *nwt = reinterpret_cast<const float *>(p.norm_weight_ptr);
+    float rsv = 0.f;
+    if constexpr (kFold) {
+        const int *idx = kFix == 1 ? p.in_index_ptr : p.out_index_ptr;
+        const int k = tid & 15, gb = G / 4, bh = blockIdx.x / gb, bw = blockIdx.x - bh * gb, sk = (bh * 4 + (k >> 2)) * G + bw * 4 + (k & 3);
+        rsv = nrs[idx ? idx[sk] : sk];
+    }
+    auto fold_norm = [&](float *v, int k, int c) {
+#pragma clang fp contract(off)
+        const float rs = __builtin_bit_cast(float, __builtin_amdgcn_readlane(__builtin_bit_cast(int, rsv), k));
+        float t[VEC];
+        if constexpr (VEC == 4) { const float4 q = *reinterpret_cast<const float4 *>(nwt + c); t[0] = q.x; t[1] = q.y; t[2] = q.z; t[3] = q.w; }
+        else t[0] = nwt[c];
+#pragma unroll
+        for (int e = 0; e < VEC; ++e) { v[e] = v[e] * rs; v[e] = v[e] * t[e]; v[e] = v[e] + 0.0f; }
+    };
     const bool has_gate = kFix == 0 ? gate != nullptr : kFix == 2;
     const bool has_mod = kFix == 0 ? scale != nullptr : (kFix == 1 || kFix == 3 || kFix == 5);
     const bool has_shift = kFix == 0 ? shift != nullptr : kFix == 1;
@@ -178,6 +195,7 @@
 #pragma unroll
             for (int e = 0; e < VEC; ++e) o[e] += t[e]; }
         if (has_res) { load_vec(rb + (int64_t)tok * p.res_token_stride + c, t);
+            if constexpr (kFold && kFix == 2) fold_norm(t, k, c);
 #pragma unroll
             for (int e = 0; e < VEC; ++e) o[e] += t[e]; }
         if constexpr (F16S) {
@@ -210,6 +228,7 @@
             tok = tin[k];
         }
         load_vec(xb + (int64_t)tok * p.x_token_stride + c, dst);
+        if constexpr (kFold && kFix == 1) fold_norm(dst, k, c);
         if (has_gate) { float t[VEC]; load_vec(gate + c, t);
 #pragma unroll
             for (int e = 0; e < VEC; ++e) dst[e] *= t[e]; }
@@ -357,7 +376,7 @@
     }
 }
 
-template <int kPieces, int kOut>
+template <int kPieces, int kOut, int kFold = 0>
 __global__ __launch_bounds__(256) void token_rows_kernel(const dimsum_tt_params_t p) {
     const int lane = threadIdx.x & 63, wave = threadIdx.x >> 6;
     const int C = p.channels, T = p.tokens;
@@ -381,7 +400,18 @@
             }
         };
         f32x4 q[kPieces];
+        auto fold_norm = [&](f32x4 (&r)[kPieces], int tok) {
+#pragma clang fp contract(off)
+            const float rs = reinterpret_cast<const float *>(p.norm_rstd_ptr)[(int64_t)b * T + tok];
+            f32x4 wv[kPieces];
+            ld(reinterpret_cast<const float *>(p.norm_weight_ptr), wv);
+#pragma unroll
+            for (int i = 0; i < kPieces; ++i)
+#pragma unroll
+                for (int e = 0; e < 4; ++e) { r[i].v[e] = r[i].v[e] * rs; r[i].v[e] = r[i].v[e] * wv[i].v[e]; r[i].v[e] = r[i].v[e] + 0.0f; }
+        };
         ld(x, v);
+        if constexpr (kFold == 1) fold_norm(v, src);
         if (gate) { ld(gate, q);
 #pragma unroll
             for (int i = 0; i < kPieces; ++i)
@@ -398,6 +428,7 @@
 #pragma unroll
                 for (int e = 0; e < 4; ++e) v[i].v[e] += q[i].v[e]; }
         if (res) { ld(res, q);
+            if constexpr (kFold == 2) fold_norm(q, dst);
 #pragma unroll
             for (int i = 0; i < kPieces; ++i)
 #pragma unroll
@@ -453,18 +484,24 @@
             int64_t blocks = (rows + 3) / 4;
             if (blocks > 256 * 16) blocks = 256 * 16;
             const dim3 g1((unsigned)blocks), b1(256);
-#define DIMSUM_TTR(O)                                                                                    \
-            if (p.channels <= 512) hipLaunchKernelGGL((token_rows_kernel<2, O>), g1, b1, 0, s, p);          \
-            else if (p.channels <= 1024) hipLaunchKernelGGL((token_rows_kernel<4, O>), g1, b1, 0, s, p);    \
-            else hipLaunchKernelGGL((token_rows_kernel<8, O>), g1, b1, 0, s, p)
-            if (p.y_split3 == 2) { DIMSUM_TTR(2); }
-            else if (p.y_split3) { DIMSUM_TTR(1); }
-            else { DIMSUM_TTR(0); }
+#define DIMSUM_TTR(O, F)                                                                                    \
+            if (p.channels <= 512) hipLaunchKernelGGL((token_rows_kernel<2, O, F>), g1, b1, 0, s, p);          \
+            else if (p.channels <= 1024) hipLaunchKernelGGL((token_rows_kernel<4, O, F>), g1, b1, 0, s, p);    \
+            else hipLaunchKernelGGL((token_rows_kernel<8, O, F>), g1, b1, 0, s, p)
+            if (p.norm_fold) {
+                if (p.y_split3 != 2) return DIMSUM_ERR_UNSUPPORTED;
+                if (p.norm_fold == 1) { DIMSUM_TTR(2, 1); }
+                else { DIMSUM_TTR(2, 2); }
+            }
+            else if (p.y_split3 == 2) { DIMSUM_TTR(2, 0); }
+            else if (p.y_split3) { DIMSUM_TTR(1, 0); }
+            else { DIMSUM_TTR(0, 0); }
 #undef DIMSUM_TTR
             return launch_status();
         }
         if (p.y_split3 == 2) return DIMSUM_ERR_STRIDE;
     }
+    if (p.norm_fold && !(blocked && p.y_split3 == 2 && VEC == 4)) return DIMSUM_ERR_UNSUPPORTED;
     if (p.y_split3 == 2) {
         if constexpr (VEC == 4) {
             dimsum_tt_params_t q = p;
@@ -474,7 +511,10 @@
             const dim3 blockh(cg <= 64 ? 64 : (cg <= 128 ? 128 : kTTThreads));
             static const bool fix = !(getenv("DIMSUM_TT_FIX") && atoi(getenv("DIMSUM_TT_FIX")) == 0);
             const bool pre = fix && p.scale_ptr && p.shift_ptr && !p.gate_ptr && !p.residual_ptr, post = fix && p.gate_ptr && p.residual_ptr && !p.scale_ptr && !p.shift_ptr;
-#define DIMSUM_TTH(K) do { if (blocked && pre) hipLaunchKernelGGL((token_transform_kernel<K, 4, true, (K) == DIMSUM_TT_NONE ? 0 : 1>), grid, blockh, lds, s, q);          \
+            if (p.norm_fold && !(p.norm_fold == 1 ? pre : post)) return DIMSUM_ERR_UNSUPPORTED;
+#define DIMSUM_TTH(K) do { if (blocked && pre && p.norm_fold) hipLaunchKernelGGL((token_transform_kernel<K, 4, true, (K) == DIMSUM_TT_NONE ? 0 : 1, (K) != DIMSUM_TT_NONE>), grid, blockh, lds, s, q);   \
+                           else if (blocked && post && p.norm_fold) hipLaunchKernelGGL((token_transform_kernel<K, 4, true, (K) == DIMSUM_TT_NONE ? 0 : 2, (K) != DIMSUM_TT_NONE>), grid, blockh, lds, s, q); \
+                           else if (blocked && pre) hipLaunchKernelGGL((token_transform_kernel<K, 4, true, (K) == DIMSUM_TT_NONE ? 0 : 1>), grid, blockh, lds, s, q);          \
                            else if (blocked && post) hipLaunchKernelGGL((token_transform_kernel<K, 4, true, (K) == DIMSUM_TT_NONE ? 0 : 2>), grid, blockh, lds, s, q);    \
                            else hipLaunchKernelGGL((token_transform_kernel<K, 4, true, 0>), grid, blockh, lds, s, q); } while (0)
             switch (p.kind) {
@@ -547,6 +587,12 @@
                (!p->scale_ptr || aligned_to<float>(p->scale_ptr, 16)) && (!p->shift_ptr || aligned_to<float>(p->shift_ptr, 16));
     if (p->residual_ptr) vec = vec && aligned_to<float>(p->residual_ptr, 16) && p->res_batch_stride % 4 == 0 && p->res_token_stride % 4 == 0;
     if (p->w_ptr) vec = vec && aligned_to<float>(p->w_ptr, 16) && p->w_batch_stride % 4 == 0 && p->w_token_stride % 4 == 0;
+    if (p->norm_fold) {
+        if (p->norm_fold != 1 && p->norm_fold != 2) return DIMSUM_ERR_UNSUPPORTED;
+        if (!p->norm_rstd_ptr || !p->norm_weight_ptr || (p->norm_fold == 2 && !p->residual_ptr)) return DIMSUM_ERR_NULL;
+        if (!vec || !aligned_to<float>(p->norm_weight_ptr, 16) || !aligned_to<float>(p->norm_rstd_ptr, 4)) return DIMSUM_ERR_STRIDE;
+        if (p->w_ptr || p->tsum_ptr || !p->y_ptr) return DIMSUM_ERR_UNSUPPORTED;
+    }
     if (p->y_split3 == 2) {
         if (!p->y_ptr || !p->y_inv_scale_ptr) return DIMSUM_ERR_NULL;
         if (!vec || p->y_token_stride < p->channels || p->channels > (p->kind == DIMSUM_TT_NONE ? 2048 : 4 * kTTThreads) || p->w_ptr || p->tsum_ptr)
diff --git a/dimsum_amd/gemm.py b/dimsum_amd/gemm.py
--- a/dimsum_amd/gemm.py
+++ b/dimsum_amd/gemm.py
@@ -504,17 +504,22 @@
     return residual + y
 
 
-def _nt_f16s(a, b, bias=None, residual=None, gate=None, rows_per_batch=None):
+def _nt_f16s(a, b, bias=None, residual=None, gate=None, rows_per_batch=None, residual_norm=None):
     from . import native
     if own_gemm_enabled() and native.gemm_nt_supported(a.data, b.data) and (gate is None or rows_per_batch % 256 == 0):
-        return native.gemm_nt(a.data, b.data, bias=bias, scales=(a.inv, b.inv), residual=residual, gate=gate, rows_per_batch=rows_per_batch)
+        return native.gemm_nt(a.data, b.data, bias=bias, scales=(a.inv, b.inv), residual=residual, gate=gate, rows_per_batch=rows_per_batch,
+                              residual_norm=residual_norm)
+    if residual_norm is not None:
+        residual = residual * residual_norm[0][:, None] * residual_norm[1][None, :] + 0.0
     return _tail(torch.mm(a.data, b.data.t(), out_dtype=torch.float32) * a.inv[:, None] * b.inv[None, :], bias, residual, gate, rows_per_batch)
 
 
-def linear_split3(x3, weight, bias=None, residual=None, gate=None, rows_per_batch=None):
+def linear_split3(x3, weight, bias=None, residual=None, gate=None, rows_per_batch=None, residual_norm=None):
     from . import native
     if isinstance(x3, native.F16Image):
-        return _nt_f16s(x3, weight_f16s(weight), bias, residual, gate, rows_per_batch)
+        return _nt_f16s(x3, weight_f16s(weight), bias, residual, gate, rows_per_batch, residual_norm)
+    if residual_norm is not None:
+        raise NotImplementedError("linear_split3: residual_norm goes with a scaled-fp16 operand image (policy f16s)")
     w3i = weight_image(weight)
     if isinstance(x3, native.PairImage) and not (own_gemm_enabled() and native.gemm_nt_supported(x3, w3i) and (gate is None or rows_per_batch % 256 == 0)):
         x3 = x3.image3()
diff --git a/dimsum_amd/models_dim.py b/dimsum_amd/models_dim.py
--- a/dimsum_amd/models_dim.py
+++ b/dimsum_amd/models_dim.py
@@ -301,11 +301,14 @@
     return _mlp_tail(mlp, hidden_states, norm_2(hidden_states), shift, scale, gate)
 
 
-def _mix_through_images(mixer, hidden_states, kind, table, shift, scale, c, fork=False):
+def _mix_through_images(mixer, hidden_states, kind, table, shift, scale, c, fork=False, norm_fold=None):
     if getattr(mixer, "takes_image", lambda: False)() and gemm.split3_enabled(hidden_states, mixer.in_proj.weight, left=False):
         m = mixer(None, c, x3=token_ops.pre_mixer(hidden_states, kind, table, shift, scale,
-                                                  split3=gemm.split3_enabled(hidden_states, mixer.in_proj.weight, left=False)))
+                                                  split3=gemm.split3_enabled(hidden_states, mixer.in_proj.weight, left=False),
+                                                  **({} if norm_fold is None else {"norm_fold": norm_fold})))
         return (m, hidden_states) if fork else m
+    if norm_fold is not None:
+        raise RuntimeError("norm_fold: the mixer does not take its input as an operand image (see _CombinedBase._fold_prenorm)")
     if fork and hidden_states.is_cuda and torch.is_grad_enabled() and hidden_states.requires_grad:
         t, hidden_states = token_ops.pre_mixer_fork(hidden_states, kind, table, shift, scale)
         return mixer(t, c), hidden_states
@@ -370,13 +373,14 @@
             return None
         return so.block_order_table(H, self.reverse, self.transpose, self.scanning_continuity)
 
-    def forward(self, hidden_states, residual=None, c=None, inference_params=None, out_split3=False):
+    def forward(self, hidden_states, residual=None, c=None, inference_params=None, out_split3=False, norm_fold=None):
         _refuse_cache(inference_params)
         hidden_states, residual = self._prenorm(hidden_states, residual)
         table = self._table(hidden_states.shape[1], hidden_states.device, self._order)
         shift, scale, gate = _modulation(self.adaLN_modulation, c).chunk(3, dim=1)
-        m, hidden_states = _mix_through_images(self.mixer, hidden_states, "none", table, shift, scale, c, fork=True)
-        return token_ops.post_mixer(hidden_states, m, gate, "none", table, **({"split3": out_split3} if out_split3 else {})), residual
+        nf = {} if norm_fold is None else {"norm_fold": norm_fold}
+        m, hidden_states = _mix_through_images(self.mixer, hidden_states, "none", table, shift, scale, c, fork=True, **nf)
+        return token_ops.post_mixer(hidden_states, m, gate, "none", table, **({"split3": out_split3} if out_split3 else {}), **nf), residual
 
 
 class DiMBlock(_BlockBase):
@@ -442,16 +446,17 @@
             self.norm_2 = norm_cls(dim)
             self.mlp = _make_mlp(dim)
 
-    def forward(self, hidden_states, residual=None, c=None, inference_params=None, out_split3=False):
+    def forward(self, hidden_states, residual=None, c=None, inference_params=None, out_split3=False, norm_fold=None):
         _refuse_cache(inference_params)
         hidden_states, residual = self._prenorm(hidden_states, residual)
         table = self._table(hidden_states.shape[1], hidden_states.device, self._order)
         mods = _modulation(self.adaLN_modulation, c).chunk(3 if self.no_ffn else 6, dim=1)
         shift, scale, gate = mods[:3]
         if self.no_ffn:
-            m, hidden_states = _mix_through_images(self.mixer, hidden_states, self.kind, table, shift, scale, c, fork=True)
-            return token_ops.post_mixer(hidden_states, m, gate, self.kind, table, **({"split3": out_split3} if out_split3 else {})), residual
-        assert not out_split3
+            nf = {} if norm_fold is None else {"norm_fold": norm_fold}
+            m, hidden_states = _mix_through_images(self.mixer, hidden_states, self.kind, table, shift, scale, c, fork=True, **nf)
+            return token_ops.post_mixer(hidden_states, m, gate, self.kind, table, **({"split3": out_split3} if out_split3 else {}), **nf), residual
+        assert not out_split3 and norm_fold is None
         t = token_ops.pre_mixer(hidden_states, self.kind, table, torch.zeros_like(shift), torch.zeros_like(scale))
         t = t + gate.unsqueeze(1) * self.mixer(modulate(t, shift, scale), c)
         t = t + mods[5].unsqueeze(1) * self.mlp(modulate(self.norm_2(t), mods[3], mods[4]))
@@ -539,15 +544,47 @@
         self.adaLN_modulation = nn.Sequential(nn.SiLU(), nn.Linear(dim, 3 * dim, bias=True))
         self.mlp = _make_mlp(dim, use_gated_mlp)
 
+    def _fold_prenorm(self, hidden_states, residual):
+        if os.environ.get("DIMSUM_FOLD_PRENORM", "1") == "0" or residual is None or torch.is_grad_enabled():
+            return False
+        x, C = hidden_states, hidden_states.shape[-1]
+        if not (self.fused_add_norm and self.residual_in_fp32 and isinstance(self.norm, RMSNorm) and self.norm.bias is None
+                and self.norm.weight.dtype == torch.float32 and isinstance(self.drop_path, nn.Identity) and x.is_cuda and x.dim() == 3
+                and x.dtype == torch.float32 and residual.dtype == torch.float32 and x.is_contiguous() and residual.is_contiguous()
+                and C % 8 == 0 and x.shape[1] % 256 == 0 and gemm.own_gemm_enabled()):
+            return False
+        if not (type(self)._freq is _CombinedBase._freq and isinstance(self.spatial_mamba, DiMBlockRaw) and isinstance(self.freq_mamba, _FreqBlock)
+                and self.freq_mamba.no_ffn and self.freq_mamba.kind != "none" and _fast_tail(self.norm_2, self.mlp, x)):
+            return False
+        half = x[..., :C // 2]
+        if not (self._branch_images and self.proj.takes_images(x) and gemm.split3_enabled(half, self.proj.qkv1.weight) == "f16s"):
+            return False
+        return all(getattr(b.mixer, "takes_image", lambda: False)() and gemm.split3_enabled(half, b.mixer.in_proj.weight, left=False) == "f16s"
+                   for b in (self.spatial_mamba, self.freq_mamba))
+
     def forward(self, hidden_states, residual=None, c=None, inference_params=None):
         _refuse_cache(inference_params)
-        hidden_states, residual = self._prenorm(hidden_states, residual)
+        fold = None
+        if self._fold_prenorm(hidden_states, residual):
+            from . import native
+            B, L, C = hidden_states.shape
+            w = self.norm.weight.detach().contiguous()
+            _, _, rstd, stream = native.layer_norm_fwd(hidden_states.view(B * L, C), w, None, self.norm.eps, residual=residual.view(B * L, C),
+                                                       is_rms_norm=True, stats_only=True)
+            hidden_states = residual = stream.view(B, L, C)
+            fold = (rstd, w)
+        else:
+            hidden_states, residual = self._prenorm(hidden_states, residual)
         if hidden_states.is_cuda and torch.is_grad_enabled() and hidden_states.requires_grad:
             x1, x2, hidden_states = _ForkHalves.apply(hidden_states)
         else:
             x1, x2 = hidden_states.chunk(2, dim=2)
         img = self._branch_images and self.proj.takes_images(hidden_states) and gemm.split3_enabled(x1, self.proj.qkv1.weight)
         kw = {"out_split3": img} if img else {}
+        kw1, kw = kw, dict(kw)
+        if fold is not None:
+            h = hidden_states.shape[-1] // 2
+            kw1, kw = dict(kw, norm_fold=(fold[0], fold[1][:h])), dict(kw, norm_fold=(fold[0], fold[1][h:]))
         if ((not torch.is_grad_enabled()) and hidden_states.is_cuda and branch_streams_enabled()
                 and not torch.cuda.is_current_stream_capturing()):
             cur = torch.cuda.current_stream(hidden_states.device)
@@ -557,15 +594,17 @@
             side.wait_stream(cur)
             with torch.cuda.stream(side):
                 x2 = self._freq(x2, c, inference_params, kw)
-            x1, _ = self.spatial_mamba(x1, None, c, inference_params, **kw)
+            x1, _ = self.spatial_mamba(x1, None, c, inference_params, **kw1)
             cur.wait_stream(side)
             x2.record_stream(cur)
         else:
-            x1, _ = self.spatial_mamba(x1, None, c, inference_params, **kw)
+            x1, _ = self.spatial_mamba(x1, None, c, inference_params, **kw1)
             x2 = self._freq(x2, c, inference_params, kw)
         fast_tail = _fast_tail(self.norm_2, self.mlp, hidden_states)
         in_epilogue = bool(img) and fast_tail and hidden_states.is_contiguous()
-        fused, pb = self.proj.forward_deferred(x1, x2, **({"images": True} if img else {}), **({"residual": hidden_states} if in_epilogue else {}))
+        assert fold is None or in_epilogue
+        fused, pb = self.proj.forward_deferred(x1, x2, **({"images": True} if img else {}), **({"residual": hidden_states} if in_epilogue else {}),
+                                               **({} if fold is None else {"residual_norm": fold}))
         shift, scale, gate = _modulation(self.adaLN_modulation, c).chunk(3, dim=1)
         return _norm_mlp_tail(self.norm_2, self.mlp, hidden_states, shift, scale, gate, fused, pb, in_epilogue), residual
 
diff --git a/dimsum_amd/native.py b/dimsum_amd/native.py
--- a/dimsum_amd/native.py
+++ b/dimsum_amd/native.py
@@ -710,7 +710,7 @@
 
 
 def layer_norm_fwd(x, weight, bias, eps, residual=None, out_dtype=None, residual_dtype=None, is_rms_norm=False,
-                   x_bias=None, mod_scale=None, mod_shift=None, rows_per_batch=0, split3=False):
+                   x_bias=None, mod_scale=None, mod_shift=None, rows_per_batch=0, split3=False, stats_only=False):
     _gpu(x, weight, bias, residual)
     _check(x.dim() == 2 and x.stride(-1) == 1, "layer_norm_fwd: x must be (M, N) with contiguous rows")
     M, N = x.shape
@@ -719,7 +719,10 @@
         _check(residual.shape == x.shape and residual.stride(-1) == 1, "layer_norm_fwd: bad residual")
         residual_dtype = residual.dtype
     y_inv = None
-    if split3 == "f16s":
+    if stats_only:
+        _check(is_rms_norm and residual is not None and bias is None and mod_scale is None and not split3, "layer_norm_fwd: stats_only is the plain RMSNorm prenorm pass")
+        y = None
+    elif split3 == "f16s":
         _check(N % 4 == 0, "layer_norm_fwd: the f16s image needs N % 4 == 0")
         y = torch.empty((M, N), device=x.device, dtype=torch.float16)
         y_inv = torch.empty((M,), device=x.device, dtype=torch.float32)
@@ -737,10 +740,10 @@
     if M > 0:
         P = _lib.NormParams()
         P.rows, P.cols, P.is_rms_norm, P.eps = M, N, int(is_rms_norm), float(eps)
-        P.x_dtype, P.out_dtype, P.y_split3 = _DT[x.dtype], _DT[y.dtype], _SPLIT_MODE.get(split3, int(bool(split3)))
+        P.x_dtype, P.out_dtype, P.y_split3 = _DT[x.dtype], _DT[x.dtype if y is None else y.dtype], _SPLIT_MODE.get(split3, int(bool(split3)))
         P.y_inv_scale_ptr = _ptr(y_inv)
         P.residual_dtype = _DT[residual_out.dtype] if residual_out is not None else _DT[x.dtype]
-        P.x_row_stride, P.y_row_stride = x.stride(0), y.stride(0)
+        P.x_row_stride, P.y_row_stride = x.stride(0), (0 if y is None else y.stride(0))
         if residual is not None:
             P.residual_row_stride = residual.stride(0)
         if residual_out is not None:
@@ -1211,7 +1214,7 @@
 
 
 def token_transform(x, kind, forward, in_index=None, out_index=None, gate=None, scale=None, shift=None, residual=None,
-                    w=None, want_y=True, want_wsum=False, want_tsum=False, split3=False):
+                    w=None, want_y=True, want_wsum=False, want_tsum=False, split3=False, norm_fold=None):
     _gpu(x, in_index, out_index, gate, scale, shift, residual, w)
     _check(x.dim() == 3 and x.dtype == torch.float32 and x.stride(2) == 1, "token_transform: x must be (B, L, C) float32, channel-contiguous")
     B, L, C = x.shape
@@ -1265,6 +1268,12 @@
         P.x_ptr, P.in_index_ptr, P.out_index_ptr = _ptr(x), _ptr(in_index), _ptr(out_index)
         P.gate_ptr, P.scale_ptr, P.shift_ptr, P.residual_ptr, P.y_ptr = _ptr(gate), _ptr(scale), _ptr(shift), _ptr(residual), _ptr(y)
         P.w_ptr, P.wdot_ptr, P.wsum_ptr, P.tsum_ptr = _ptr(w), _ptr(wdot), _ptr(wsum), _ptr(tsum)
+        if norm_fold is not None:
+            which, nr, nw = norm_fold
+            _gpu(nr, nw)
+            _check(which in ("x", "residual") and split3 == "f16s" and nr.dtype == torch.float32 and nw.dtype == torch.float32 and nr.is_contiguous()
+                   and nw.is_contiguous() and nr.numel() == B * L and nw.numel() == C, "token_transform: norm_fold = ('x' | 'residual', rstd (B * L,), weight (C,)) float32, with the f16s image")
+            P.norm_fold, P.norm_rstd_ptr, P.norm_weight_ptr = (1 if which == "x" else 2), _ptr(nr), _ptr(nw)
         with torch.cuda.device(x.device):
             _lib.check(_lib.load().dimsum_token_transform(P, _stream(x)), "token_transform")
     if y_inv is not None:
@@ -1874,7 +1883,7 @@
 
 
 def gemm_nt(a, b, bias=None, epilogue="f32", out=None, out_scale=1.0, events=None, tune=None, scales=None, gate_bound=None, residual=None,
-            gate=None, rows_per_batch=None, keep_x12=False, pair_out=False, weight_order=False, q_cols=None, conv=None):
+            gate=None, rows_per_batch=None, keep_x12=False, pair_out=False, weight_order=False, q_cols=None, conv=None, residual_norm=None):
     pair_in = isinstance(a, PairImage)
     pair_b = isinstance(b, PairImage)
     if pair_in:
@@ -1913,6 +1922,12 @@
             _check(residual.dtype == torch.float32 and residual.shape == (M, N) and residual.stride(1) == 1, "gemm_nt: residual must be (M, N) float32 rows")
             epi = _lib.GEMM_EPI_F32_GATE_RESIDUAL
             ext.update(residual_ptr=_ptr(residual), residual_ld=residual.stride(0))
+            if residual_norm is not None:
+                nr, nw = residual_norm
+                _gpu(nr, nw)
+                _check(a.dtype == torch.float16 and nr.dtype == torch.float32 and nw.dtype == torch.float32 and nr.is_contiguous() and nw.is_contiguous()
+                       and nr.numel() == M and nw.numel() == N, "gemm_nt: residual_norm = (rstd (M,), weight (N,)) float32 with float16 operands")
+                ext.update(res_rstd_ptr=_ptr(nr), res_weight_ptr=_ptr(nw))
             if gate is not None:
                 _check(rows_per_batch and rows_per_batch % 256 == 0 and M % rows_per_batch == 0 and gate.dtype == torch.float32
                        and gate.shape == (M // rows_per_batch, N) and gate.stride(1) == 1, "gemm_nt: gate must be (M / rows_per_batch, N) float32, rows_per_batch % 256 == 0")
diff --git a/dimsum_amd/ops/token_ops.py b/dimsum_amd/ops/token_ops.py
--- a/dimsum_amd/ops/token_ops.py
+++ b/dimsum_amd/ops/token_ops.py
@@ -212,11 +212,14 @@
     return _GateResidual.apply(res, m, gate, bias)
 
 
-def pre_mixer(x, kind, table, shift, scale, split3=False):
+def pre_mixer(x, kind, table, shift, scale, split3=False, norm_fold=None):
     _require_gpu(x)
+    if norm_fold is not None and split3 != "f16s":
+        raise NotImplementedError("pre_mixer: norm_fold goes with the scaled-fp16 image output")
     if split3:
         from .. import native
-        return native.token_transform(_cc(x), kind, True, out_index=None if table is None else table["inv32"], scale=scale, shift=shift, split3=split3)
+        return native.token_transform(_cc(x), kind, True, out_index=None if table is None else table["inv32"], scale=scale, shift=shift, split3=split3,
+                                      **({} if norm_fold is None else {"norm_fold": ("x",) + tuple(norm_fold)}))
     return _PreMixer.apply(x, shift, scale, kind, None if table is None else table["inv32"])
 
 
@@ -225,9 +228,12 @@
     return _PreMixerFork.apply(x, shift, scale, kind, None if table is None else table["inv32"])
 
 
-def post_mixer(x, m, gate, kind, table, split3=False):
+def post_mixer(x, m, gate, kind, table, split3=False, norm_fold=None):
     _require_gpu(x)
+    if norm_fold is not None and split3 != "f16s":
+        raise NotImplementedError("post_mixer: norm_fold goes with the scaled-fp16 image output")
     if split3:
         from .. import native
-        return native.token_transform(_cc(m), kind, False, in_index=None if table is None else table["inv32"], gate=gate, residual=_cc(x), split3=split3)
+        return native.token_transform(_cc(m), kind, False, in_index=None if table is None else table["inv32"], gate=gate, residual=_cc(x), split3=split3,
+                                      **({} if norm_fold is None else {"norm_fold": ("residual",) + tuple(norm_fold)}))
     return _PostMixer.apply(x, m, gate, kind, None if table is None else table["inv32"])
diff --git a/include/dimsum_hip.h b/include/dimsum_hip.h
--- a/include/dimsum_hip.h
+++ b/include/dimsum_hip.h
@@ -676,7 +676,9 @@
     void *tsum_ptr;
     void *y_inv_scale_ptr;
     int32_t y_f16s_lds_offset;
-    int32_t reserved;
+    int32_t norm_fold;
+    const void *norm_rstd_ptr;
+    const void *norm_weight_ptr;
 } dimsum_tt_params_t;
 
 int dimsum_token_transform(const dimsum_tt_params_t *p, void *stream);
@@ -906,6 +908,8 @@
     const void *c_scale_ptr;
     const void *k_inv_a_ptr;
     const void *k_inv_b_ptr;
+    const void *res_rstd_ptr;
+    const void *res_weight_ptr;
 } dimsum_gemm_ext_t;
 
 typedef struct {
```
